# jurgisp/pydreamer

Hardware: AMD Instinct MI355X
Metric: grad-steps/sec (world-model+AC) at B=50,T=50,H=15, 64×64 obs, 1/2/4/8 GPU (higher is better)
Workload: dtype f32; 1 GPU; atari-literal: defaults+atari, batch_size 50, batch_length 50, imag_horizon 15, deter_dim 600, stoch 32x32, hidden 1000, cnn_depth 48, action_dim 18, fp32; fwd + 4 bwd + clip + 4 AdamW per step; replay resident in HBM; global_batch=50, batch_length=50, imag_horizon=15, parallelism=dp1 (batch-sharded [50])

## Files before the change

### include/dreamer_hip.h

```cpp
#ifndef DREAMER_HIP_H
#define DREAMER_HIP_H

#include <stddef.h>
#include <stdint.h>

#ifdef __cplusplus
extern "C" {
#endif

#define DM_OK 0
#define DM_E_SHAPE (-1)
#define DM_E_WORKSPACE (-2)
#define DM_E_HIP (-3)
#define DM_E_DEVICE (-4)
#define DM_E_NULL (-5)

#define DM_MAX_MLP_LAYERS 8

typedef struct dm_shape {
  int32_t T, B, I;
  int32_t H;
  int32_t D, Hd;
  int32_t S, C;
  int32_t E;
  int32_t A;
  int32_t mlp_hidden;
  int32_t mlp_layers;
  int32_t cnn_depth;
  int32_t img, img_ch;
  int32_t flags;
} dm_shape;
#define DM_FLAG_IMAGE_U8 16
#define DM_FLAG_GRU_SHIFT 5
#define DM_FLAG_BF16 128
#define DM_FLAG_GRU_LAYERS_SHIFT 8
#define DM_FLAG_GRU_LAYERS_MASK (3 << DM_FLAG_GRU_LAYERS_SHIFT)
#define DM_FLAG_GRU_MASK (3 << DM_FLAG_GRU_SHIFT)

int dm_version(void);
const char* dm_last_error(void);
int dm_device_check(void);
size_t dm_workspace_bytes(const dm_shape* shp);
int dm_stream_create_cu_mask(const uint32_t* mask, int words, void** stream);
int dm_stream_destroy(void* stream);
int dm_wgrad_side_arm(int on);
int dm_wgrad_side_touch(void);
int dm_wgrad_side_join(void* stream);

#define DM_GEMM_ACCUM 1
#define DM_GEMM_ELU 2
#define DM_GEMM_BF16 256
int dm_gemm_f32(int a_layout, int b_layout, int M, int N, int K,
                const float* A, int lda, const float* B, int ldb, float* C, int ldc,
                const float* bias, const float* add, int ldadd, int flags,
                void* ws, size_t ws_bytes, void* stream);
int dm_gemm_bf16h(int a_layout, int b_layout, int M, int N, int K, const uint16_t* A, int lda, const uint16_t* B, int ldb,
                  float* C, int ldc, uint16_t* C_h, const float* bias, int flags, void* ws, size_t ws_bytes, void* stream);
int dm_bf16_twins_enable(int on);
int dm_gemm_dma_enable(int on);
int dm_dec_l4_bwd_direct_enable(int on);
int dm_rssm_lds_enable(int on);
int dm_bptt_fold_enable(int on);
int dm_rssm_lds_status(void);
int dm_rssm_lds_status_ack(void);
int dm_rssm_lds_gave_up(void);
int dm_rssm_lds_prof(unsigned long long* out16, int reset);

int dm_ln_elu_fwd(int rows, int n, const float* x, int ldx, const float* gamma, const float* beta, float eps,
                  float* y, int ldy, float* stats, void* stream);
int dm_ln_elu_bwd(int rows, int n, const float* x, int ldx, const float* y, int ldy, const float* stats,
                  const float* gamma, const float* dy, int lddy, float* dx, int lddx,
                  float* dgamma, float* dbeta, void* ws, size_t ws_bytes, void* stream);
int dm_colsum(int rows, int n, const float* x, int ld, float* out, void* ws, size_t ws_bytes, void* stream);

int dm_gru_gates_fwd(int rows, int D, const float* gi, const float* gh, const float* h_in, int ldh,
                     float* h_out, int ldo, void* stream);
int dm_gru_gates_bwd(int rows, int D, const float* gi, const float* gh, const float* h_in, int ldh,
                     const float* dh_out, int lddh, float* dgi, float* dgh, float* dh_in, int lddi, void* stream);

int dm_sample_onehot(int rows, int groups, int C, const float* logits, int ldl, const float* u,
                     const int32_t* forced_idx, float* onehot, int ldo, int32_t* idx, void* stream);

int dm_kl_balance_fwd(int rows, int S, int C, const float* post, const float* prior,
                      float* kl, float* ent_post, float* ent_prior, void* stream);
int dm_kl_balance_bwd(int rows, int S, int C, const float* post, const float* prior,
                      float scale_post, float scale_prior, float* dpost, float* dprior, void* stream);
int dm_st_softmax_bwd(int rows, int groups, int C, const float* logits, int ldl, const float* dz, int lddz,
                      float* dlogits, int lddl, int accum, void* stream);

int dm_kl_sampled_fwd(int rows, int S, int C, const float* post, const float* prior, const int32_t* idx, float* out, void* stream);
int dm_kl_sampled_bwd(int rows, int S, int C, const float* post, const float* prior, const int32_t* idx, float scale,
                      const float* row_w, float* dpost, float* dprior, void* stream);
int dm_kl_sampled_gauss_fwd(int rows, int S, const float* post, const float* prior, const float* z, int ldz, float* out,
                            void* stream);
int dm_kl_sampled_gauss_bwd(int rows, int S, const float* post, const float* prior, const float* z, int ldz, float scale,
                            const float* row_w, float* dpost, float* dprior, float* dz, int lddz, void* stream);
int dm_reduce_i(int TB, int I, int W, const float* x, int mode, float* out, float* w_out, void* stream);
int dm_combine_rows(int count, int64_t n, const float* const* x, const float* w, float* out, void* stream);
int dm_scale_rows(int64_t rows, int n, float* x, int ldx, const float* w, float scale, void* stream);

int dm_mask_rows(int rows, int n, const float* x, int ldx, const uint8_t* reset, float* y, int ldy, void* stream);

int dm_im2col_s2(int n, int hb, int wb, int c, int k, const float* big, int big_nchw, float* col, void* stream);
#define DM_C2I_ELU 1
int dm_col2im_s2(int n, int hb, int wb, int c, int k, const float* col, const float* bias, int flags,
                 const float* elu_ref, float* big, void* stream);

typedef struct dm_mlp_params {
  const float* w[DM_MAX_MLP_LAYERS + 1];
  const float* b[DM_MAX_MLP_LAYERS + 1];
  const float* ln_g[DM_MAX_MLP_LAYERS];
  const float* ln_b[DM_MAX_MLP_LAYERS];
  int32_t precision;
  int32_t reserved_;
} dm_mlp_params;
typedef struct dm_mlp_grads {
  float* w[DM_MAX_MLP_LAYERS + 1];
  float* b[DM_MAX_MLP_LAYERS + 1];
  float* ln_g[DM_MAX_MLP_LAYERS];
  float* ln_b[DM_MAX_MLP_LAYERS];
} dm_mlp_grads;
size_t dm_mlp_acts_floats(int rows, int hidden, int layers);
size_t dm_mlp_ws_floats(int rows, int hidden, int layers);
int dm_mlp_head_fwd(int rows, int in_dim, int hidden, int layers, int out_dim,
                    const float* x, int ldx, const dm_mlp_params* p, float* acts, float* out,
                    void* ws, size_t ws_bytes, void* stream);
int dm_mlp_head_fwd_sparse(int rows, int in_dim, int sparse_cols, int hidden, int layers, int out_dim,
                           const float* x, int ldx, const dm_mlp_params* p, float* acts, float* out,
                           void* ws, size_t ws_bytes, void* stream);
int dm_mlp_head_fwd_rows(int rows_total, int row0, int rows, int in_dim, int sparse_cols, int hidden, int layers, int out_dim,
                         const float* x, int ldx, const dm_mlp_params* p, float* acts, float* out,
                         void* ws, size_t ws_bytes, void* stream);

int dm_mlp_head_bwd(int rows, int in_dim, int hidden, int layers, int out_dim,
                    const float* x, int ldx, const dm_mlp_params* p, const float* acts, const float* dout,
                    const dm_mlp_grads* g, float* dx, int lddx, int dx_accum,
                    void* ws, size_t ws_bytes, void* stream);

int dm_head_loss(int kind, int rows, const float* out, const float* target, float scale, float loss_const,
                 float* loss, float* dout, float* mean_out, void* stream);

int dm_head_loss_normal_nd(int rows, int V, const float* out, const float* target, float scale, float loss_const,
                           float* loss, float* dout, float* mean_out, void* stream);

int dm_cat_target_index(int rows, int C, int cells, const float* onehot, int32_t* idx, void* stream);
int dm_cat_image_loss(int rows, int I, int C, int cells, const float* logits, int ld, const int32_t* target, float* loss,
                      float* dlogits, void* stream);
int dm_cat_image_pred(int groups, int I, int C, int cells, const float* logits, int ld, const int32_t* target,
                      const int32_t* seen, float* logp, float* acc, float* acc_seen, void* stream);
int dm_cat_concat_rows(int rows, int I, int F, int E, const float* x, int ldx, const float* extra, float* out, void* stream);

int dm_dense_image_rows(int rows, int C, int cells, const float* image_f32, const int32_t* class_i32, const float* reward,
                        const float* terminal, float* out, int ldo, void* stream);
int dm_elu_rows_fwd(int rows, int n, const float* x, int ldx, float* y, int ldy, void* stream);
int dm_elu_rows_bwd(int rows, int n, const float* y, int ldy, const float* dy, int lddy, float* dx, int lddx, void* stream);
int dm_cat_image_loss_mix(int rows, int I, int C, int cells, const float* logits, int ld, const int32_t* target, float min_prob,
                          float* loss, float* dlogits, void* stream);

size_t dm_goals_stats_ws_floats(int rows, int G);
int dm_goals_stats(int rows, int G, const float* goals, const float* pred, const float* visage, float* out, void* ws,
                   size_t ws_bytes, void* stream);

int dm_preprocess_image_u8(int64_t n, int hw, int c, const uint8_t* src, float* dst, void* stream);

typedef struct dm_conv_params { const float* w[5]; const float* b[5]; } dm_conv_params;
typedef struct dm_conv_grads { float* w[5]; float* b[5]; } dm_conv_grads;
size_t dm_conv_encoder_acts_floats(const dm_shape* shp);
int dm_conv_encoder_fwd(const dm_shape* shp, const float* image , const dm_conv_params* p,
                        float* acts, float* embed , void* ws, size_t ws_bytes, void* stream);
int dm_conv_encoder_bwd(const dm_shape* shp, const float* image, const dm_conv_params* p, const float* acts,
                        const float* dembed, const dm_conv_grads* g, void* ws, size_t ws_bytes, void* stream);
int dm_conv_encoder_fwd_planes(const dm_shape* shp, const float* image, const dm_conv_params* p, const float* reward,
                               const float* terminal, float* acts, float* embed, int ld_embed, void* ws, size_t ws_bytes,
                               void* stream);
int dm_conv_encoder_bwd_planes(const dm_shape* shp, const float* image, const dm_conv_params* p, const float* reward,
                               const float* terminal, const float* acts, const float* dembed, int ld_dembed,
                               const dm_conv_grads* g, void* ws, size_t ws_bytes, void* stream);

size_t dm_conv_decoder_acts_floats(const dm_shape* shp);
size_t dm_conv_decoder_pred_offset(const dm_shape* shp);
int dm_conv_decoder_mse_fwd(const dm_shape* shp, const float* feat, int ldf, const float* target,
                            const dm_conv_params* p, float* acts, float* loss_image, float* image_rec ,
                            void* ws, size_t ws_bytes, void* stream);
int dm_conv_decoder_mse_bwd_rows(const dm_shape* shp, const float* feat, int ldf, const float* target,
                                 const dm_conv_params* p, const float* acts, float scale, const float* row_scale,
                                 const dm_conv_grads* g, float* dfeat, int lddf, void* ws, size_t ws_bytes, void* stream);
int dm_conv_decoder_mse_bwd(const dm_shape* shp, const float* feat, int ldf, const float* target,
                            const dm_conv_params* p, const float* acts, float scale,
                            const dm_conv_grads* g, float* dfeat, int lddf, void* ws, size_t ws_bytes, void* stream);

enum {
  DM_RSSM_Z_W = 0, DM_RSSM_Z_B, DM_RSSM_A_W, DM_RSSM_IN_G, DM_RSSM_IN_B,
  DM_RSSM_GRU_WIH, DM_RSSM_GRU_WHH, DM_RSSM_GRU_BIH, DM_RSSM_GRU_BHH,
  DM_RSSM_PRIOR_H_W, DM_RSSM_PRIOR_H_B, DM_RSSM_PRIOR_G, DM_RSSM_PRIOR_B, DM_RSSM_PRIOR_W, DM_RSSM_PRIOR_OB,
  DM_RSSM_POST_H_W, DM_RSSM_POST_H_B, DM_RSSM_POST_E_W, DM_RSSM_POST_G, DM_RSSM_POST_B, DM_RSSM_POST_W, DM_RSSM_POST_OB,
  DM_RSSM_GRU_LN_G0, DM_RSSM_GRU_LN_B0, DM_RSSM_GRU_LN_G1, DM_RSSM_GRU_LN_B1, DM_RSSM_GRU_LN_G2, DM_RSSM_GRU_LN_B2,
  DM_RSSM_GRU_L1_WIH, DM_RSSM_GRU_L1_WHH, DM_RSSM_GRU_L1_BIH, DM_RSSM_GRU_L1_BHH,
  DM_RSSM_GRU_L2_WIH, DM_RSSM_GRU_L2_WHH, DM_RSSM_GRU_L2_BIH, DM_RSSM_GRU_L2_BHH,
  DM_RSSM_GRU_L3_WIH, DM_RSSM_GRU_L3_WHH, DM_RSSM_GRU_L3_BIH, DM_RSSM_GRU_L3_BHH,
  DM_RSSM_GRU_L1_LN_G0, DM_RSSM_GRU_L1_LN_B0, DM_RSSM_GRU_L1_LN_G1, DM_RSSM_GRU_L1_LN_B1, DM_RSSM_GRU_L1_LN_G2, DM_RSSM_GRU_L1_LN_B2,
  DM_RSSM_GRU_L2_LN_G0, DM_RSSM_GRU_L2_LN_B0, DM_RSSM_GRU_L2_LN_G1, DM_RSSM_GRU_L2_LN_B1, DM_RSSM_GRU_L2_LN_G2, DM_RSSM_GRU_L2_LN_B2,
  DM_RSSM_GRU_L3_LN_G0, DM_RSSM_GRU_L3_LN_B0, DM_RSSM_GRU_L3_LN_G1, DM_RSSM_GRU_L3_LN_B1, DM_RSSM_GRU_L3_LN_G2, DM_RSSM_GRU_L3_LN_B2,
  DM_RSSM_NPARAMS
};
typedef struct dm_rssm_params { const float* p[DM_RSSM_NPARAMS]; } dm_rssm_params;
typedef struct dm_rssm_grads { float* p[DM_RSSM_NPARAMS]; } dm_rssm_grads;
size_t dm_rssm_acts_floats(const dm_shape* shp);
int dm_rssm_sequence_fwd(const dm_shape* shp, const float* embed, const float* action, const uint8_t* reset,
                         const float* h0, const float* z0, const float* u, const int32_t* forced_idx,
                         const dm_rssm_params* p, float* acts, float* feat, float* post, float* prior, int32_t* idx,
                         void* ws, size_t ws_bytes, void* stream);
int dm_rssm_sequence_bwd(const dm_shape* shp, const float* embed, const float* action, const uint8_t* reset,
                         const dm_rssm_params* p, const float* acts, const float* feat, const float* post,
                         float* dfeat, float* dpost, float* dprior,
                         const dm_rssm_grads* g, float* dembed, void* ws, size_t ws_bytes, void* stream);

#define DM_SCHED_FWD_FUSE_LN 1
#define DM_SCHED_FWD_FUSE_SAMPLE 2
#define DM_SCHED_FWD_FRAG 4
#define DM_SCHED_FWD_WZT 8
#define DM_SCHED_FWD_PSYNC 16
#define DM_SCHED_BWD_FUSE_B 1
#define DM_SCHED_BWD_FOLD 2
#define DM_SCHED_BWD_FOLD_SM 4
#define DM_SCHED_BWD_FRAG 8
#define DM_SCHED_BWD_NCHUNK_SHIFT 8
#define DM_SCHED_BWD_NCHUNK_MASK (15 << DM_SCHED_BWD_NCHUNK_SHIFT)
#define DM_SCHED_ROLL_WZT 1
#define DM_SCHED_ROLL_WAT 2
#define DM_SCHED_ROLL_ACTOR_WPACK 4
#define DM_SCHED_ROLL_ACTOR_ADD0 8
#define DM_SCHED_ROLL_FUSE_ACT 16
#define DM_SCHED_ROLL_TW_ON 32
int dm_rssm_last_schedule(int which);

typedef struct dm_gru_params { const float* w_ih; const float* w_hh; const float* b_ih; const float* b_hh; } dm_gru_params;
typedef struct dm_gru_grads { float* w_ih; float* w_hh; float* b_ih; float* b_hh; } dm_gru_grads;
size_t dm_gru_sequence_acts_floats(int T, int B, int In, int D);
size_t dm_gru_sequence_ws_bytes(int T, int B, int In, int D);
// ... 60 lines not shown
```

### pydreamer_amd/csrc/common.h

```cpp
#pragma once
#include <hip/hip_runtime.h>
#include <stdint.h>
#include <stddef.h>
#include "dreamer_hip.h"

int dm_fail(int code, const char* fmt, ...);

#define DM_MAX_DEVICES 16

#define DM_LAUNCH_CHECK()                                                                      \
  do {                                                                                         \
    hipError_t e__ = hipGetLastError();                                                        \
    if (e__ != hipSuccess) return dm_fail(DM_E_HIP, "%s:%d: %s", __FILE__, __LINE__, hipGetErrorString(e__)); \
  } while (0)

#define DM_TRY(expr)                 \
  do {                               \
    int rc__ = (expr);               \
    if (rc__ != DM_OK) return rc__;  \
  } while (0)

#define DM_REQUIRE(cond, code, ...)                     \
  do {                                                  \
    if (!(cond)) return dm_fail(code, __VA_ARGS__);     \
  } while (0)

static inline int dm_cdiv(int64_t a, int64_t b) { return (int)((a + b - 1) / b); }
static inline size_t dm_align_up(size_t x, size_t a) { return (x + a - 1) / a * a; }

struct DmArena {
  float* base;
  size_t cap;
  size_t off;
  bool ok;
  DmArena(void* p, size_t bytes) : base((float*)p), cap(bytes / sizeof(float)), off(0), ok(true) {}
  float* take(size_t nfloats) {
    size_t n = dm_align_up(nfloats, 64);
    if (base == nullptr || off + n > cap) { ok = false; off += n; return nullptr; }
    float* r = base + off;
    off += n;
    return r;
  }
};

hipStream_t dm_wgrad_side_stream(hipStream_t st);
int dm_wgrad_side_fork(hipStream_t st, hipStream_t sw);
int dm_wgrad_side_mark(hipStream_t sw, hipStream_t st);

int dm_cur_precision();
struct DmPrecisionScope {
  int prev;
  explicit DmPrecisionScope(int p);
  ~DmPrecisionScope();
};

struct DmTwinScope {
  bool active, opened;
  explicit DmTwinScope(bool bf16_mode);
  ~DmTwinScope();
};
bool dm_twins_on();
void dm_twin_add(const float* base, size_t n, unsigned short* twin, bool valid);
void dm_twin_mark(const float* p);
unsigned short* dm_twin_of(const float* p, bool need_valid);
void dm_twin_arena_note(const void* acts, bool written);
bool dm_twin_arena_valid(const void* acts);
struct DmCvtSeg { const float* src; unsigned short* dst; size_t n; };
int dm_to_bf16_multi_launch(const DmCvtSeg* segs, int count, hipStream_t st);
static inline size_t dm_half_floats(size_t elems) { return (elems + 1) / 2; }
constexpr int DM_HSTORE_MIN_K = 1024;
constexpr int DM_HSTORE_MIN_K_DENSE = 400;

struct DmGatesBwd;
struct DmGemm {
  int bf16 = dm_cur_precision();
  int a_layout = 0, b_layout = 0;
  int M = 0, N = 0, K = 0;
  const float* A = nullptr; int lda = 0;
  const float* B = nullptr; int ldb = 0;
  float* C = nullptr; int ldc = 0;
  const float* bias = nullptr;
  const float* add = nullptr; int ldadd = 0;
  const float* mulref = nullptr; int ldmul = 0;
  const uint8_t* row_zero = nullptr;
  const int* a_maj = nullptr; const int* a_min = nullptr; int a_tab_vec = 0;
  const int* b_maj = nullptr; const int* b_min = nullptr; int b_tab_vec = 0;
  int a_tab_vec8 = 0, b_tab_vec8 = 0;
  int flags = 0;
  const int2* c_tab = nullptr; int sc_cout = 0, sc_wpitch = 0;
  int bias_mod = 0;
  const float* ln_g = nullptr; const float* ln_b = nullptr; float ln_eps = 1e-3f;
  const float* lnb_x = nullptr; int lnb_ldx = 0; const float* lnb_stats = nullptr;
  const float* eg_x = nullptr; int eg_ldx = 0; const float* eg_stats = nullptr; const float* eg_gamma = nullptr; const float* eg_beta = nullptr;
  float* eg_G = nullptr; int eg_ldg = 0; float* eg_Gf = nullptr; float* eg_ps = nullptr;
  const float* lnf_ps = nullptr; int lnf_nps = 0; const float* lnf_stats = nullptr;
  const float* lnf_xw = nullptr; int lnf_ldxw = 0; const float* lnf_cs = nullptr;
  const float* sm_logits = nullptr; int sm_ld = 0; float* sm_dlogits = nullptr; int sm_ldd = 0;
  const struct DmGatesBwd* gates = nullptr;
  const float* A_frag = nullptr;
  float* C_frag = nullptr;
  const unsigned short* A_h = nullptr;
  const unsigned short* B_h = nullptr;
  unsigned short* C_h = nullptr;
  bool no_twin = false;
};
__host__ __device__ __forceinline__ size_t dm_frag_off(int row, int k) {
  return ((((size_t)(k >> 4) * 4 + (row >> 4)) * 4 + ((k >> 2) & 3)) * 16 + (row & 15)) * 4 + (k & 3);
}
static inline size_t dm_frag_floats(int K) { return (size_t)dm_cdiv(K, 16) * 1024; }
int dm_frag_pack_launch(int rows, int K, const float* X, int ldx, float* Xf, hipStream_t st);
struct DmRssmLds {
  int B, D, Hd, S, C, F, t_begin, t_end;
  const float *wzt, *zb, *wih, *bih, *whh, *bhh, *wph, *bph, *wpo, *bpo, *in_g, *in_b, *post_g, *post_b, *ea, *ee;
  const uint8_t* reset; const float* u; const int32_t* forced;
  float *x1, *gi, *gh, *hin, *zin, *feat, *x2, *post; int32_t* idx;
  float* ws; size_t ws_floats;
};
bool dm_rssm_lds_ok(int B, int D, int Hd, int S, int C);
size_t dm_rssm_lds_ws_floats(int B, int D, int Hd, int S, int C, int steps);
int dm_rssm_lds_launch(const DmRssmLds& q, hipStream_t st);
extern "C" int dm_rssm_lds_enable(int on);
bool dm_z_embed_ok(int n);
int dm_sparse_rows_launch(int rows, int n, int Zc, const float* z, int ldz, const float* Wt, float* x, int ldx,
                          hipStream_t st);
int dm_z_embed_launch(int rows, int n, int S, int C, const int32_t* idx, const uint8_t* row_zero, const float* Wt,
                      const float* bias, const float* add, int ldadd, const int32_t* idx2, const float* Wt2, float* x, int ldx,
                      float* x_frag, const float* gamma, const float* beta, float eps, float* y, int ldy, hipStream_t st,
                      float* y_frag = nullptr, float* stats = nullptr);
struct DmGatesBwd {
  const float* gi; const float* gh; const float* h_in; int ldh, D;
  float* dgi; float* dgh; float* dprev; int ldp; const uint8_t* row_zero;
  float* dgi_frag = nullptr; float* dgh_frag = nullptr;
};
struct DmSample {
  const float* u = nullptr; const int32_t* forced = nullptr;
  float* onehot = nullptr; int ldo = 0;
  int32_t* idx = nullptr;
  float* z_next = nullptr; const uint8_t* next_reset = nullptr;
  float* z_next_frag = nullptr;
};
bool dm_skinny_ln_ok(int M, int N, int K);
int dm_gemm_sample_launch(const DmGemm& q, const DmSample& sm, hipStream_t stream);
int dm_gemm_launch(const DmGemm& g, void* ws, size_t ws_bytes, hipStream_t stream);
int dm_gemm_skinny_try(const DmGemm& g, hipStream_t stream);
int dm_gemm_pair_launch(const DmGemm& g0, const DmGemm& g1, void* ws, size_t ws_bytes, hipStream_t stream);

int dm_colsum_launch(int rows, int n, const float* x, int ld, float* out, void* ws, size_t ws_bytes, hipStream_t st);
int dm_elu_fwd_launch(int rows, int n, const float* x, int ldx, float* y, int ldy, hipStream_t st);
int dm_elu_bwd_launch(int rows, int n, const float* y, int ldy, const float* dy, int lddy, float* dx, int lddx,
                      hipStream_t st);
int dm_ln_elu_fwd_launch(int rows, int n, const float* x, int ldx, const float* gamma, const float* beta, float eps,
                         float* y, int ldy, float* stats, hipStream_t st);
int dm_ln_elu_bwd_dx_launch(int rows, int n, const float* x, int ldx, const float* y, int ldy, const float* stats,
                            const float* gamma, const float* dy, int lddy, float* dx, int lddx, hipStream_t st);
int dm_ln_elu_bwd_params_launch(int rows, int n, const float* x, int ldx, const float* y, int ldy, const float* stats,
                                const float* dy, int lddy, float* dgamma, float* dbeta, void* ws, size_t ws_bytes,
                                hipStream_t st);
int dm_gru_norm_fwd_launch(int kind, int rows, int D, const float* gi, const float* gh, const float* h_in, int ldh,
                           const float* const* ln_g, const float* const* ln_b, float* h_out, int ldo, float* gs, float* gst,
                           float* h_next, const uint8_t* next_reset, hipStream_t st, int ldg = 0, int ldst = 0, int ldn = 0);
int dm_gru_norm_bwd_launch(int kind, int rows, int D, const float* gh, const float* h_in, int ldh, const float* gs,
                           const float* gst, const float* const* ln_g, const float* const* ln_b, const float* dh_out, int lddh,
                           float* dgi, float* dgh, float* dg, float* dh_in, int lddi, const uint8_t* row_zero, hipStream_t st,
                           int ldg = 0, int ldst = 0);
int dm_gru_norm_param_grads_launch(int kind, int rows, int D, const float* gs, const float* gst, const float* dg, float* dgam,
                                   float* dbet, hipStream_t st, int ldg = 0, int ldst = 0);
int dm_gru_gates_fwd_launch(int rows, int D, const float* gi, const float* gh, const float* h_in, int ldh, float* h_out,
                            int ldo, float* h_next, const uint8_t* next_reset, float* h_frag, float* h_next_frag,
                            hipStream_t st, int ldg = 0, int ldn = 0);
int dm_gru_gates_bwd_launch(int rows, int D, const float* gi, const float* gh, const float* h_in, int ldh,
                            const float* dh_out, int lddh, float* dgi, float* dgh, float* dh_in, int lddi, int accum,
                            const uint8_t* row_zero, hipStream_t st, int ldg = 0);
int dm_sample_onehot_launch(int rows, int groups, int C, const float* logits, int ldl, const float* u,
                            const int32_t* forced, float* onehot, int ldo, int32_t* idx, float* z_next,
                            const uint8_t* next_reset, hipStream_t st);
int dm_gauss_sample_bwd_launch(int rows, int S, const float* par, int ldp, const float* z, int ldz, const float* dz,
                               int lddz, float* dpar, int lddp, int accum, hipStream_t st);
int dm_kl_fwd_launch(int rows, int S, int C, const float* post, const float* prior, float* kl, float* ep, float* eq,
                     hipStream_t st);
int dm_kl_bwd_launch(int rows, int S, int C, const float* post, const float* prior, float sp, float sq, float* dpost,
                     float* dprior, hipStream_t st);
int dm_st_softmax_bwd_launch(int rows, int groups, int C, const float* logits, int ldl, const float* dz, int lddz,
                             float* dlogits, int lddl, int accum, hipStream_t st);
int dm_mask_rows_launch(int rows, int n, const float* x, int ldx, const uint8_t* reset, float* y, int ldy, hipStream_t st);
int dm_mask_rows2_launch(int rows, int n1, const float* x1, int ldx1, float* y1, int ldy1, int n2, const float* x2,
                         int ldx2, float* y2, int ldy2, const uint8_t* reset, hipStream_t st);
int dm_sample_continuous_launch(int kind, int rows, int A, const float* params, const float* eps, float* action,
                                hipStream_t st);
int dm_mul_elu_grad_launch(size_t n, const float* dy, const float* yact, float* out, hipStream_t st);

int dm_im2col_s2_launch(int n, int hb, int wb, int c, int k, const float* big, int big_nchw, float* col, hipStream_t st);
int dm_col2im_s2_launch(int n, int hb, int wb, int c, int k, const float* col, const float* bias, int flags,
                        const float* elu_ref, float* big, hipStream_t st);
int dm_permute4_launch(const float* src, float* dst, int d0, int d1, int d2, int d3, int p0, int p1, int p2, int p3,
                       hipStream_t st);

bool dm_enc_l1_direct_ok(int ch, int d, int img);
int dm_enc_l1_fwd_launch(int frames, int d, int u8, const void* image, const float* w, const float* bias, float* wt, float* y,
                         unsigned short* y_h, hipStream_t st);
size_t dm_enc_l1_wgrad_part_floats(int frames, int d);
int dm_enc_l1_wgrad_launch(int frames, int d, int u8, const void* image, const float* G, float* part, float* dW, void* ws,
                           size_t ws_bytes, hipStream_t st);
int dm_enc_l1_fwd_planes_launch(int frames, int d, int u8, const void* image, const float* w5, const float* bias,
                                const float* reward, const float* terminal, float* wt, float* fb, float* y,
                                unsigned short* y_h, hipStream_t st);
size_t dm_enc_l1_planes_part_floats(int frames, int d);
int dm_enc_l1_planes_bwd_launch(int frames, int d, const float* G, const float* reward, const float* terminal,
                                const float* dw3, float* part, float* db, float* dW5, hipStream_t st);
bool dm_dec_l4_direct_ok(int ch, int d, int hs, int k);
size_t dm_dec_l4_w4_floats(int d);
int dm_dec_l4_fwd_launch(int frames, int d, const float* x, const float* w, const float* bias, float* w4, float* out,
                         hipStream_t st);
bool dm_dec_l4_bwd_direct_ok(int ch, int d, int hs, int k);
size_t dm_dec_l4_wp_floats(int d);
size_t dm_dec_l4_wgrad_part_floats(int frames, int d);
int dm_dec_l4_dgrad_launch(int frames, int d, const float* G4, const float* w, float* wp, const float* x3, float* dx,
                           unsigned short* dx_h, hipStream_t st);
int dm_dec_l4_wgrad_launch(int frames, int d, const float* G4, const float* x3, float* part, float* dW, void* ws,
                           size_t ws_bytes, hipStream_t st);

struct DmChainSample {
  const float* u;
  float* onehot;
  int ldo;
  int32_t* idx;
};
int dm_mlp_fwd_launch(int rows, int in_dim, int hidden, int layers, int out_dim, const float* x, int ldx,
                      const dm_mlp_params* p, float* acts, int acts_total_rows, int acts_row_off, float* out, int ldout,
                      void* ws, size_t ws_bytes, hipStream_t st, const float* chain_wpack = nullptr, int sparse_cols = 0,
                      const float* chain_add0 = nullptr, const DmChainSample* chain_sample = nullptr);

bool dm_panel_ok(int rows, int hidden);
int dm_panel_count(int rows);
int dm_panel_ln_fwd_launch(int rows, int hidden, int kin, const float* x, int ldx, const float* W, const float* b,
                           const float* gamma, const float* beta, float eps, float* xpre, float* stats, float* y,
                           const float* wout, const float* bout, float* out, int out_dim, int ldout, hipStream_t st,
                           const unsigned short* Wh = nullptr, int ldw = 0, const float* addm = nullptr);
int dm_panel_bf16_weights_launch(int count, const float* const* w, unsigned short* const* dst, const int* rows, const int* cols,
                                 int transpose, hipStream_t st);
int dm_panel_ln_bwd_launch(int rows, int hidden, int kup, const float* dup, int lddup, const float* W, const float* xpre,
                           const float* stats, const float* gamma, const float* beta, float* dx, float* colpart, float* wt,
                           hipStream_t st, const unsigned short* Wth = nullptr);
int dm_panel_colsum_final_launch(int count, const float* const* part, float* const* out, int n, int npanels, int pstride,
                                 hipStream_t st);

bool dm_mlp_chain_ok(int rows, int in_dim, int hidden, int layers, int out_dim, const float* x, int ldx,
                     const dm_mlp_params* p);
size_t dm_mlp_chain_pack_floats(int in_dim, int layers);
int dm_mlp_chain_pack_launch(int in_dim, int layers, const dm_mlp_params* p, float* wpack, hipStream_t st, int k0 = 0);
int dm_mlp_chain_fwd_launch(int rows, int in_dim, int layers, int out_dim, const float* x, int ldx, const dm_mlp_params* p,
                            float* const* xpre, float* const* stats, float* const* y, float* out, int ldout, const float* wpack,
                            hipStream_t st, int k0 = 0, const float* add0 = nullptr, const DmChainSample* sample = nullptr);
bool dm_mlp_chain_sparse_ok(int in_dim, int sparse_cols);

int dm_prof_slot_begin(int kind, double flops, double bytes, hipStream_t st);
void dm_prof_slot_end(int slot, hipStream_t st);
extern "C" int dm_mlp_chain_min_rows(int rows);
bool dm_prof_active();

static const size_t DM_SPLITK_FLOATS = (size_t)16 * 1024 * 1024;

typedef __bf16 bf16x8 __attribute__((ext_vector_type(8)));
typedef __bf16 bf16x2 __attribute__((ext_vector_type(2)));
typedef float dm_f32x2 __attribute__((ext_vector_type(2)));
__device__ __forceinline__ unsigned dm_pack_bf16x2(float lo, float hi) {
  const dm_f32x2 v = {lo, hi};
  return __builtin_bit_cast(unsigned, __builtin_convertvector(v, bf16x2));
}
__device__ __forceinline__ unsigned dm_f2bf(float x) { return dm_pack_bf16x2(x, 0.f) & 0xFFFFu; }
__device__ __forceinline__ uint2 dm_pack_bf16x4(float4 v) {
  return make_uint2(dm_pack_bf16x2(v.x, v.y), dm_pack_bf16x2(v.z, v.w));
}

__device__ __forceinline__ float dm_elu(float v) { return v > 0.f ? v : expm1f(v); }
__device__ __forceinline__ float dm_elu_grad_from_y(float y) { return y > 0.f ? 1.f : y + 1.f; }

__device__ __forceinline__ float dm_wave_sum(float v) {
#pragma unroll
  for (int off = 32; off > 0; off >>= 1) v += __shfl_xor(v, off, 64);
  return v;
}
__device__ __forceinline__ float dm_wave_max(float v) {
#pragma unroll
  for (int off = 32; off > 0; off >>= 1) v = fmaxf(v, __shfl_xor(v, off, 64));
  return v;
}
```

### pydreamer_amd/csrc/elementwise.hip

```cpp
#include "common.h"

template <bool CACHE>
__global__ void __launch_bounds__(256) ln_elu_fwd_kernel(int rows, int n, const float* __restrict__ x, int ldx,
                                                         const float* __restrict__ gamma, const float* __restrict__ beta,
                                                         float eps, float* __restrict__ y, int ldy, float* __restrict__ stats,
                                                         unsigned short* __restrict__ y_h) {
  const int row = blockIdx.x * 4 + (threadIdx.x >> 6);
  const int lane = threadIdx.x & 63;
  if (row >= rows) return;
  const float* xr = x + (size_t)row * ldx;
  unsigned short* yh = y_h ? y_h + (size_t)row * ldy : nullptr;
  float xc[16];
  float s = 0.f;
  if (CACHE) {
#pragma unroll
    for (int j = 0; j < 16; ++j) {
      const int c = lane + 64 * j;
      xc[j] = c < n ? xr[c] : 0.f;
      s += xc[j];
    }
  } else {
    for (int c = lane; c < n; c += 64) s += xr[c];
  }
  const float mean = dm_wave_sum(s) / (float)n;
  float v = 0.f;
  if (CACHE) {
#pragma unroll
    for (int j = 0; j < 16; ++j) {
      const float d = (lane + 64 * j < n) ? xc[j] - mean : 0.f;
      v += d * d;
    }
  } else {
    for (int c = lane; c < n; c += 64) {
      const float d = xr[c] - mean;
      v += d * d;
    }
  }
  const float var = dm_wave_sum(v) / (float)n;
  const float rstd = 1.0f / sqrtf(var + eps);
  float* yr = y + (size_t)row * ldy;
  if (CACHE) {
#pragma unroll
    for (int j = 0; j < 16; ++j) {
      const int c = lane + 64 * j;
      if (c < n) {
        const float o = dm_elu((xc[j] - mean) * rstd * gamma[c] + beta[c]);
        yr[c] = o;
        if (yh) yh[c] = (unsigned short)dm_f2bf(o);
      }
    }
  } else {
    for (int c = lane; c < n; c += 64) {
      const float o = dm_elu((xr[c] - mean) * rstd * gamma[c] + beta[c]);
      yr[c] = o;
      if (yh) yh[c] = (unsigned short)dm_f2bf(o);
    }
  }
  if (lane == 0) {
    stats[2 * row] = mean;
    stats[2 * row + 1] = rstd;
  }
}

template <bool CACHE>
__global__ void __launch_bounds__(256) ln_elu_bwd_dx_kernel(int rows, int n, const float* __restrict__ x, int ldx,
                                                            const float* __restrict__ y, int ldy,
                                                            const float* __restrict__ stats, const float* __restrict__ gamma,
                                                            const float* __restrict__ dy, int lddy,
                                                            float* __restrict__ dx, int lddx) {
  const int row = blockIdx.x * 4 + (threadIdx.x >> 6);
  const int lane = threadIdx.x & 63;
  if (row >= rows) return;
  const float mean = stats[2 * row], rstd = stats[2 * row + 1];
  const float* xr = x + (size_t)row * ldx;
  const float* yr = y + (size_t)row * ldy;
  const float* dyr = dy + (size_t)row * lddy;
  float gc[16], hc[16];
  float sg = 0.f, sgx = 0.f;
  if (CACHE) {
#pragma unroll
    for (int j = 0; j < 16; ++j) {
      const int c = lane + 64 * j;
      gc[j] = 0.f; hc[j] = 0.f;
      if (c < n) {
        gc[j] = dyr[c] * dm_elu_grad_from_y(yr[c]) * gamma[c];
        hc[j] = (xr[c] - mean) * rstd;
      }
      sg += gc[j];
      sgx += gc[j] * hc[j];
    }
  } else {
    for (int c = lane; c < n; c += 64) {
      const float g = dyr[c] * dm_elu_grad_from_y(yr[c]) * gamma[c];
      const float xh = (xr[c] - mean) * rstd;
      sg += g;
      sgx += g * xh;
    }
  }
  sg = dm_wave_sum(sg) / (float)n;
  sgx = dm_wave_sum(sgx) / (float)n;
  float* dxr = dx + (size_t)row * lddx;
  if (CACHE) {
#pragma unroll
    for (int j = 0; j < 16; ++j) {
      const int c = lane + 64 * j;
      if (c < n) dxr[c] = rstd * (gc[j] - sg - hc[j] * sgx);
    }
  } else {
    for (int c = lane; c < n; c += 64) {
      const float g = dyr[c] * dm_elu_grad_from_y(yr[c]) * gamma[c];
      const float xh = (xr[c] - mean) * rstd;
      dxr[c] = rstd * (g - sg - xh * sgx);
    }
  }
}

template <int MODE>
__global__ void __launch_bounds__(256) colsum_partial_kernel(int rows, int n, int rows_per_chunk,
                                                             const float* __restrict__ x, int ldx,
                                                             const float* __restrict__ y, int ldy,
                                                             const float* __restrict__ stats,
                                                             const float* __restrict__ dy, int lddy,
                                                             float* __restrict__ partial) {
  __shared__ float red[2][4][64];
  const int cx = threadIdx.x & 63, ry = threadIdx.x >> 6;
  const int col = blockIdx.x * 64 + cx;
  const int chunk = blockIdx.y;
  const int r0 = chunk * rows_per_chunk;
  const int r1 = min(rows, r0 + rows_per_chunk);
  float a0 = 0.f, a1 = 0.f;
  if (col < n) {
    if (MODE == 0) {
      float b0 = 0.f, b1 = 0.f, b2 = 0.f, b3 = 0.f;
      int r = r0 + ry;
      for (; r + 12 < r1; r += 16) {
        b0 += x[(size_t)r * ldx + col];
        b1 += x[(size_t)(r + 4) * ldx + col];
        b2 += x[(size_t)(r + 8) * ldx + col];
        b3 += x[(size_t)(r + 12) * ldx + col];
      }
      for (; r < r1; r += 4) b0 += x[(size_t)r * ldx + col];
      a0 = (b0 + b1) + (b2 + b3);
    } else {
      for (int r = r0 + ry; r < r1; r += 4) {
        const float dl = dy[(size_t)r * lddy + col] * dm_elu_grad_from_y(y[(size_t)r * ldy + col]);
        const float xh = (x[(size_t)r * ldx + col] - stats[2 * r]) * stats[2 * r + 1];
        a0 += dl * xh;
        a1 += dl;
      }
    }
  }
  red[0][ry][cx] = a0;
  red[1][ry][cx] = a1;
  __syncthreads();
  if (ry == 0 && col < n) {
    const int nq = (MODE == 0) ? 1 : 2;
    float s0 = red[0][0][cx] + red[0][1][cx] + red[0][2][cx] + red[0][3][cx];
    partial[((size_t)chunk * nq + 0) * n + col] = s0;
    if (MODE == 1) {
      float s1 = red[1][0][cx] + red[1][1][cx] + red[1][2][cx] + red[1][3][cx];
      partial[((size_t)chunk * nq + 1) * n + col] = s1;
    }
  }
}

__global__ void __launch_bounds__(256) colsum_flat_kernel(long long total, int n, int W, long long chunk_elems,
                                                          const float* __restrict__ x, float* __restrict__ partial) {
  __shared__ float sh[256];
  const long long base = (long long)blockIdx.x * chunk_elems;
  const long long end = min(total, base + chunk_elems);
  float b0 = 0.f, b1 = 0.f, b2 = 0.f, b3 = 0.f;
  if ((int)threadIdx.x < W) {
    long long i = base + threadIdx.x;
    for (; i + 3LL * W < end; i += 4LL * W) {
      b0 += x[i];
      b1 += x[i + W];
      b2 += x[i + 2LL * W];
      b3 += x[i + 3LL * W];
    }
    for (; i < end; i += W) b0 += x[i];
  }
  sh[threadIdx.x] = (b0 + b1) + (b2 + b3);
  __syncthreads();
  if ((int)threadIdx.x < n) {
    float s = 0.f;
    for (int t = threadIdx.x; t < W; t += n) s += sh[t];
    partial[(size_t)blockIdx.x * n + threadIdx.x] = s;
  }
}

__global__ void __launch_bounds__(256) colsum_final_kernel(int n, int chunks, int nq, const float* __restrict__ partial,
                                                           float* __restrict__ out0, float* __restrict__ out1) {
  __shared__ float red[8][32];
  const int cx = threadIdx.x & 31, cy = threadIdx.x >> 5;
  const int col = blockIdx.x * 32 + cx;
  for (int q = 0; q < nq; ++q) {
    float s = 0.f;
    if (col < n) {
      const float* p = partial + (size_t)q * n + col;
      const size_t st = (size_t)nq * n;
      int c = cy;
      for (; c + 24 < chunks; c += 32) {
        const float v0 = p[(size_t)c * st], v1 = p[(size_t)(c + 8) * st], v2 = p[(size_t)(c + 16) * st], v3 = p[(size_t)(c + 24) * st];
        s += v0; s += v1; s += v2; s += v3;
      }
      for (; c < chunks; c += 8) s += p[(size_t)c * st];
    }
    red[cy][cx] = s;
    __syncthreads();
    if (cy == 0 && col < n) {
      float t = 0.f;
#pragma unroll
      for (int k = 0; k < 8; ++k) t += red[k][cx];
      (q == 0 ? out0 : out1)[col] = t;
    }
    __syncthreads();
  }
}

static int colsum_plan(int rows, size_t budget_floats, int n, int nq, int* rows_per_chunk) {
  int chunks = dm_cdiv(rows, 64);
  if (chunks > 1024) chunks = 1024;
  const size_t per = (size_t)n * nq;
  if (per > 0 && (size_t)chunks * per > budget_floats) chunks = (int)(budget_floats / per);
  if (chunks < 1) chunks = 1;
  *rows_per_chunk = dm_cdiv(rows, chunks);
  return dm_cdiv(rows, *rows_per_chunk);
}

int dm_colsum_launch(int rows, int n, const float* x, int ld, float* out, void* ws, size_t ws_bytes, hipStream_t st) {
  if (n <= 0) return DM_OK;
  if (rows <= 0) {
    (void)hipMemsetAsync(out, 0, (size_t)n * sizeof(float), st);
    return DM_OK;
  }
  DM_REQUIRE(ws && ws_bytes >= (size_t)n * sizeof(float), DM_E_WORKSPACE, "colsum: workspace too small");
  const size_t budget = ws_bytes / sizeof(float);
  int chunks;
  if (n <= 64 && ld == n && (long long)rows * n >= (1 << 16)) {
    const long long total = (long long)rows * n;
    const int W = 256 - 256 % n;
    long long want = total / ((long long)W * 16);
    if (want > 2048) want = 2048;
    if (want < 1) want = 1;
    if ((size_t)want * n > budget) want = (long long)(budget / n);
    long long chunk_elems = (total + want - 1) / want;
    chunk_elems = (chunk_elems + W - 1) / W * W;
    chunks = (int)((total + chunk_elems - 1) / chunk_elems);
    hipLaunchKernelGGL(colsum_flat_kernel, dim3(chunks), dim3(256), 0, st, total, n, W, chunk_elems, x, (float*)ws);
  } else {
    int rpc;
    chunks = colsum_plan(rows, budget, n, 1, &rpc);
    hipLaunchKernelGGL((colsum_partial_kernel<0>), dim3(dm_cdiv(n, 64), chunks), dim3(256), 0, st, rows, n, rpc, x, ld,
                       nullptr, 0, nullptr, nullptr, 0, (float*)ws);
  }
  DM_LAUNCH_CHECK();
  hipLaunchKernelGGL(colsum_final_kernel, dim3(dm_cdiv(n, 32)), dim3(256), 0, st, n, chunks, 1, (const float*)ws, out,
                     nullptr);
  DM_LAUNCH_CHECK();
  return DM_OK;
}

int dm_ln_elu_fwd_launch(int rows, int n, const float* x, int ldx, const float* gamma, const float* beta, float eps,
                         float* y, int ldy, float* stats, hipStream_t st) {
  if (rows <= 0) return DM_OK;
  unsigned short* y_h = dm_twin_of(y, false);
  if (y_h) dm_twin_mark(y);
  if (n <= 1024)
    hipLaunchKernelGGL((ln_elu_fwd_kernel<true>), dim3(dm_cdiv(rows, 4)), dim3(256), 0, st, rows, n, x, ldx, gamma, beta,
                       eps, y, ldy, stats, y_h);
  else
    hipLaunchKernelGGL((ln_elu_fwd_kernel<false>), dim3(dm_cdiv(rows, 4)), dim3(256), 0, st, rows, n, x, ldx, gamma, beta,
                       eps, y, ldy, stats, y_h);
  DM_LAUNCH_CHECK();
  return DM_OK;
}

__global__ void __launch_bounds__(256) elu_fwd_kernel(int rows, int n, const float* __restrict__ x, int ldx,
                                                      float* __restrict__ y, int ldy) {
  const size_t total = (size_t)rows * n;
  for (size_t i = (size_t)blockIdx.x * 256 + threadIdx.x; i < total; i += (size_t)gridDim.x * 256) {
    const size_t r = i / n, c = i % n;
    y[r * ldy + c] = dm_elu(x[r * ldx + c]);
  }
}
__global__ void __launch_bounds__(256) elu_bwd_kernel(int rows, int n, const float* __restrict__ y, int ldy,
                                                      const float* __restrict__ dy, int lddy, float* __restrict__ dx,
                                                      int lddx) {
  const size_t total = (size_t)rows * n;
  for (size_t i = (size_t)blockIdx.x * 256 + threadIdx.x; i < total; i += (size_t)gridDim.x * 256) {
    const size_t r = i / n, c = i % n;
    dx[r * lddx + c] = dy[r * lddy + c] * dm_elu_grad_from_y(y[r * ldy + c]);
  }
}
int dm_elu_fwd_launch(int rows, int n, const float* x, int ldx, float* y, int ldy, hipStream_t st) {
  if (rows <= 0) return DM_OK;
  const size_t total = (size_t)rows * n;
  hipLaunchKernelGGL(elu_fwd_kernel, dim3((unsigned)((total + 255) / 256 < 65536 ? (total + 255) / 256 : 65536)), dim3(256), 0,
                     st, rows, n, x, ldx, y, ldy);
  DM_LAUNCH_CHECK();
  return DM_OK;
}
int dm_elu_bwd_launch(int rows, int n, const float* y, int ldy, const float* dy, int lddy, float* dx, int lddx,
                      hipStream_t st) {
  if (rows <= 0) return DM_OK;
  const size_t total = (size_t)rows * n;
  hipLaunchKernelGGL(elu_bwd_kernel, dim3((unsigned)((total + 255) / 256 < 65536 ? (total + 255) / 256 : 65536)), dim3(256), 0,
                     st, rows, n, y, ldy, dy, lddy, dx, lddx);
  DM_LAUNCH_CHECK();
  return DM_OK;
}

int dm_ln_elu_bwd_dx_launch(int rows, int n, const float* x, int ldx, const float* y, int ldy, const float* stats,
                            const float* gamma, const float* dy, int lddy, float* dx, int lddx, hipStream_t st) {
  if (rows <= 0) return DM_OK;
  if (n <= 1024)
    hipLaunchKernelGGL((ln_elu_bwd_dx_kernel<true>), dim3(dm_cdiv(rows, 4)), dim3(256), 0, st, rows, n, x, ldx, y, ldy,
                       stats, gamma, dy, lddy, dx, lddx);
  else
    hipLaunchKernelGGL((ln_elu_bwd_dx_kernel<false>), dim3(dm_cdiv(rows, 4)), dim3(256), 0, st, rows, n, x, ldx, y, ldy,
                       stats, gamma, dy, lddy, dx, lddx);
  DM_LAUNCH_CHECK();
  return DM_OK;
}

int dm_ln_elu_bwd_params_launch(int rows, int n, const float* x, int ldx, const float* y, int ldy, const float* stats,
                                const float* dy, int lddy, float* dgamma, float* dbeta, void* ws, size_t ws_bytes,
                                hipStream_t st) {
  int rpc;
  DM_REQUIRE(ws && ws_bytes >= (size_t)2 * n * sizeof(float), DM_E_WORKSPACE, "ln_bwd: workspace too small");
  const int chunks = colsum_plan(rows, ws_bytes / sizeof(float), n, 2, &rpc);
  hipLaunchKernelGGL((colsum_partial_kernel<1>), dim3(dm_cdiv(n, 64), chunks), dim3(256), 0, st, rows, n, rpc, x, ldx, y,
                     ldy, stats, dy, lddy, (float*)ws);
  DM_LAUNCH_CHECK();
  hipLaunchKernelGGL(colsum_final_kernel, dim3(dm_cdiv(n, 32)), dim3(256), 0, st, n, chunks, 2, (const float*)ws, dgamma,
                     dbeta);
  DM_LAUNCH_CHECK();
  return DM_OK;
}

extern "C" int dm_ln_elu_fwd(int rows, int n, const float* x, int ldx, const float* gamma, const float* beta, float eps,
                             float* y, int ldy, float* stats, void* stream) {
  DM_REQUIRE(x && gamma && beta && y && stats, DM_E_NULL, "ln_elu_fwd: null pointer");
  return dm_ln_elu_fwd_launch(rows, n, x, ldx, gamma, beta, eps, y, ldy, stats, (hipStream_t)stream);
}

extern "C" int dm_ln_elu_bwd(int rows, int n, const float* x, int ldx, const float* y, int ldy, const float* stats,
                             const float* gamma, const float* dy, int lddy, float* dx, int lddx, float* dgamma,
                             float* dbeta, void* ws, size_t ws_bytes, void* stream) {
  DM_REQUIRE(x && y && stats && gamma && dy && dx && dgamma && dbeta, DM_E_NULL, "ln_elu_bwd: null pointer");
  DM_TRY(dm_ln_elu_bwd_dx_launch(rows, n, x, ldx, y, ldy, stats, gamma, dy, lddy, dx, lddx, (hipStream_t)stream));
  return dm_ln_elu_bwd_params_launch(rows, n, x, ldx, y, ldy, stats, dy, lddy, dgamma, dbeta, ws, ws_bytes,
                                     (hipStream_t)stream);
}

extern "C" int dm_colsum(int rows, int n, const float* x, int ld, float* out, void* ws, size_t ws_bytes, void* stream) {
  DM_REQUIRE(x && out, DM_E_NULL, "colsum: null pointer");
  return dm_colsum_launch(rows, n, x, ld, out, ws, ws_bytes, (hipStream_t)stream);
}

__device__ __forceinline__ float dm_sigmoid(float v) { return 1.0f / (1.0f + expf(-v)); }

__global__ void __launch_bounds__(256) gru_gates_fwd_kernel(int rows, int D, const float* __restrict__ gi,
                                                            const float* __restrict__ gh, const float* __restrict__ h_in,
                                                            int ldh, float* __restrict__ h_out, int ldo,
                                                            float* __restrict__ h_next,
                                                            const uint8_t* __restrict__ next_reset,
                                                            float* __restrict__ h_frag, float* __restrict__ h_next_frag,
                                                            int ldg, int ldn, unsigned short* __restrict__ h_out_h) {
  const size_t total = (size_t)rows * D;
  for (size_t i = (size_t)blockIdx.x * 256 + threadIdx.x; i < total; i += (size_t)gridDim.x * 256) {
    const int r = (int)(i / D), d = (int)(i % D);
    const float* gir = gi + (size_t)r * ldg;
    const float* ghr = gh + (size_t)r * ldg;
    const float rg = dm_sigmoid(gir[d] + ghr[d]);
    const float ug = dm_sigmoid(gir[D + d] + ghr[D + d]);
    const float ng = tanhf(gir[2 * D + d] + rg * ghr[2 * D + d]);
    const float h = h_in[(size_t)r * ldh + d];
    const float ho = (h - ng) * ug + ng;
    h_out[(size_t)r * ldo + d] = ho;
    if (h_out_h) h_out_h[(size_t)r * ldo + d] = (unsigned short)dm_f2bf(ho);
    const float hn = (next_reset && next_reset[r]) ? 0.f : ho;
    if (h_next) h_next[(size_t)r * ldn + d] = hn;
    if (h_frag) h_frag[dm_frag_off(r, d)] = ho;
    if (h_next_frag) h_next_frag[dm_frag_off(r, d)] = hn;
  }
}
__global__ void __launch_bounds__(256) frag_pack_kernel(int rows, int K, const float* __restrict__ X, int ldx,
                                                        float* __restrict__ Xf) {
  const int total = rows * K;
  for (int i = blockIdx.x * 256 + threadIdx.x; i < total; i += gridDim.x * 256) {
    const int r = i / K, k = i % K;
    Xf[dm_frag_off(r, k)] = X[(size_t)r * ldx + k];
  }
}

__global__ void __launch_bounds__(256) gru_gates_bwd_kernel(int rows, int D, const float* __restrict__ gi,
                                                            const float* __restrict__ gh, const float* __restrict__ h_in,
                                                            int ldh, const float* __restrict__ dh_out, int lddh,
                                                            float* __restrict__ dgi, float* __restrict__ dgh,
                                                            float* __restrict__ dh_in, int lddi, int accum,
                                                            const uint8_t* __restrict__ row_zero, int ldg) {
  const size_t total = (size_t)rows * D;
  for (size_t i = (size_t)blockIdx.x * 256 + threadIdx.x; i < total; i += (size_t)gridDim.x * 256) {
    const int r = (int)(i / D), d = (int)(i % D);
    const size_t g0 = (size_t)r * ldg;
    const float ghn = gh[g0 + 2 * D + d];
    const float rg = dm_sigmoid(gi[g0 + d] + gh[g0 + d]);
    const float ug = dm_sigmoid(gi[g0 + D + d] + gh[g0 + D + d]);
    const float ng = tanhf(gi[g0 + 2 * D + d] + rg * ghn);
    const float h = h_in[(size_t)r * ldh + d];
    const float dh = dh_out[(size_t)r * lddh + d];
    const float dn = dh * (1.f - ug);
    const float du = dh * (h - ng);
    const float dpn = dn * (1.f - ng * ng);
    const float dpr = dpn * ghn * rg * (1.f - rg);
    const float dpu = du * ug * (1.f - ug);
    dgi[g0 + d] = dpr;
    dgi[g0 + D + d] = dpu;
    dgi[g0 + 2 * D + d] = dpn;
    dgh[g0 + d] = dpr;
    dgh[g0 + D + d] = dpu;
    dgh[g0 + 2 * D + d] = dpn * rg;
    if (dh_in) {
      const float v = (row_zero && row_zero[r]) ? 0.f : dh * ug;
      float* o = dh_in + (size_t)r * lddi + d;
      *o = accum ? *o + v : v;
    }
  }
}

struct GruLnParams { const float* g[3]; const float* b[3]; };

template <int KIND>
__global__ void __launch_bounds__(256) gru_norm_fwd_kernel(int rows, int D, const float* __restrict__ gi,
                                                           const float* __restrict__ gh, const float* __restrict__ h_in,
                                                           int ldh, const GruLnParams lp, float* __restrict__ h_out, int ldo,
                                                           float* __restrict__ gs, float* __restrict__ gst,
                                                           float* __restrict__ h_next, const uint8_t* __restrict__ next_reset,
                                                           int ldg, int ldst, int ldn) {
  const int row = blockIdx.x * 4 + (threadIdx.x >> 6);
  const int lane = threadIdx.x & 63;
  if (row >= rows) return;
  const float eps = 1e-3f;
  const float* gir = gi + (size_t)row * ldg;
  const float* ghr = gh + (size_t)row * ldg;
  float* sr = gs + (size_t)row * ldg;
  const float* hr = h_in + (size_t)row * ldh;
  float st[6] = {0.f, 0.f, 0.f, 0.f, 0.f, 0.f};
  if (KIND == 2) {
    float sum = 0.f;
    for (int j = lane; j < 3 * D; j += 64) { const float v = gir[j] + ghr[j]; sr[j] = v; sum += v; }
    const float mean = dm_wave_sum(sum) / (float)(3 * D);
    float var = 0.f;
    for (int j = lane; j < 3 * D; j += 64) { const float d = (gir[j] + ghr[j]) - mean; var += d * d; }
    const float rstd = 1.0f / sqrtf(dm_wave_sum(var) / (float)(3 * D) + eps);
    st[0] = mean; st[1] = rstd;
    for (int d = lane; d < D; d += 64) {
      const float g_r = ((gir[d] + ghr[d]) - mean) * rstd * lp.g[0][d] + lp.b[0][d];
      const float g_u = ((gir[D + d] + ghr[D + d]) - mean) * rstd * lp.g[0][D + d] + lp.b[0][D + d];
      const float g_n = ((gir[2 * D + d] + ghr[2 * D + d]) - mean) * rstd * lp.g[0][2 * D + d] + lp.b[0][2 * D + d];
      const float r = dm_sigmoid(g_r), u = dm_sigmoid(g_u - 1.0f), n = tanhf(r * g_n);
      const float ho = u * n + (1.f - u) * hr[d];
      h_out[(size_t)row * ldo + d] = ho;
      if (h_next) h_next[(size_t)row * ldn + d] = (next_reset && next_reset[row]) ? 0.f : ho;
    }
  } else {
    float s0 = 0.f, s1 = 0.f;
    for (int d = lane; d < D; d += 64) {
      const float a = gir[d] + ghr[d], b = gir[D + d] + ghr[D + d];
      sr[d] = a; sr[D + d] = b;
      s0 += a; s1 += b;
    }
    const float m0 = dm_wave_sum(s0) / (float)D, m1 = dm_wave_sum(s1) / (float)D;
    float v0 = 0.f, v1 = 0.f;
    for (int d = lane; d < D; d += 64) {
      const float a = (gir[d] + ghr[d]) - m0, b = (gir[D + d] + ghr[D + d]) - m1;
      v0 += a * a; v1 += b * b;
    }
    const float r0 = 1.0f / sqrtf(dm_wave_sum(v0) / (float)D + eps), r1 = 1.0f / sqrtf(dm_wave_sum(v1) / (float)D + eps);
    float s2 = 0.f;
    for (int d = lane; d < D; d += 64) {
      const float r = dm_sigmoid(((gir[d] + ghr[d]) - m0) * r0 * lp.g[0][d] + lp.b[0][d]);
      const float c = gir[2 * D + d] + r * ghr[2 * D + d];
      sr[2 * D + d] = c;
      s2 += c;
    }
    const float m2 = dm_wave_sum(s2) / (float)D;
    float v2 = 0.f;
    for (int d = lane; d < D; d += 64) { const float c = sr[2 * D + d] - m2; v2 += c * c; }
    const float r2 = 1.0f / sqrtf(dm_wave_sum(v2) / (float)D + eps);
    st[0] = m0; st[1] = r0; st[2] = m1; st[3] = r1; st[4] = m2; st[5] = r2;
    for (int d = lane; d < D; d += 64) {
      const float u = dm_sigmoid(((gir[D + d] + ghr[D + d]) - m1) * r1 * lp.g[1][d] + lp.b[1][d]);
      const float n = tanhf((sr[2 * D + d] - m2) * r2 * lp.g[2][d] + lp.b[2][d]);
      const float ho = u * n + (1.f - u) * hr[d];
      h_out[(size_t)row * ldo + d] = ho;
      if (h_next) h_next[(size_t)row * ldn + d] = (next_reset && next_reset[row]) ? 0.f : ho;
    }
  }
  if (lane < 6) gst[(size_t)row * ldst + lane] = st[lane];
}

template <int KIND>
__global__ void __launch_bounds__(256) gru_norm_bwd_kernel(int rows, int D, const float* __restrict__ gh,
                                                           const float* __restrict__ h_in, int ldh,
// ... 673 lines not shown
}
int dm_gauss_sample_bwd_launch(int rows, int S, const float* par, int ldp, const float* z, int ldz, const float* dz,
                               int lddz, float* dpar, int lddp, int accum, hipStream_t st) {
  if (rows <= 0) return DM_OK;
  hipLaunchKernelGGL(gauss_sample_bwd_kernel, dim3(ew_blocks((size_t)rows * S)), dim3(256), 0, st, rows, S, par, ldp, z, ldz,
                     dz, lddz, dpar, lddp, accum);
  DM_LAUNCH_CHECK();
  return DM_OK;
}
__global__ void __launch_bounds__(256) gauss_kl_fwd_kernel(int rows, int S, const float* __restrict__ post,
                                                           const float* __restrict__ prior, float* __restrict__ kl,
                                                           float* __restrict__ ent_post, float* __restrict__ ent_prior) {
  const int row = blockIdx.x * 4 + (threadIdx.x >> 6);
  const int lane = threadIdx.x & 63;
  if (row >= rows) return;
  const float* a = post + (size_t)row * 2 * S;
  const float* b = prior + (size_t)row * 2 * S;
  float akl = 0.f, aep = 0.f, aeq = 0.f;
  for (int s = lane; s < S; s += 64) {
    const float s1 = dm_gauss_std(a[S + s]), s2 = dm_gauss_std(b[S + s]);
    const float d = a[s] - b[s];
    akl += logf(s2 / s1) + (s1 * s1 + d * d) / (2.0f * s2 * s2) - 0.5f;
    aep += 1.4189385332046727f + logf(s1);
    aeq += 1.4189385332046727f + logf(s2);
  }
  akl = dm_wave_sum(akl); aep = dm_wave_sum(aep); aeq = dm_wave_sum(aeq);
  if (lane == 0) {
    kl[row] = akl;
    if (ent_post) ent_post[row] = aep;
    if (ent_prior) ent_prior[row] = aeq;
  }
}
__global__ void __launch_bounds__(256) gauss_kl_bwd_kernel(int rows, int S, const float* __restrict__ post,
                                                           const float* __restrict__ prior, float sp, float sq,
                                                           float* __restrict__ dpost, float* __restrict__ dprior) {
  const int total = rows * S;
  for (int i = blockIdx.x * 256 + threadIdx.x; i < total; i += gridDim.x * 256) {
    const int r = i / S, s = i % S;
    const size_t o = (size_t)r * 2 * S;
    const float g1 = dm_sigmoid(post[o + S + s]), g2 = dm_sigmoid(prior[o + S + s]);
    const float s1 = 2.0f * g1 + 0.1f, s2 = 2.0f * g2 + 0.1f;
    const float d = post[o + s] - prior[o + s];
    const float i22 = 1.0f / (s2 * s2);
    dpost[o + s] = sp * d * i22;
    dpost[o + S + s] = sp * (s1 * i22 - 1.0f / s1) * 2.0f * g1 * (1.0f - g1);
    dprior[o + s] = -sq * d * i22;
    dprior[o + S + s] = sq * (1.0f / s2 - (s1 * s1 + d * d) * i22 / s2) * 2.0f * g2 * (1.0f - g2);
  }
}

int dm_sample_onehot_launch(int rows, int groups, int C, const float* logits, int ldl, const float* u,
                            const int32_t* forced, float* onehot, int ldo, int32_t* idx, float* z_next,
                            const uint8_t* next_reset, hipStream_t st) {
  if (rows <= 0) return DM_OK;
  if (C == 0) {
    DM_REQUIRE(u && !forced, DM_E_NULL, "sample: Gaussian latents need their noise (and cannot be index-forced)");
    hipLaunchKernelGGL(gauss_sample_kernel, dim3(ew_blocks((size_t)rows * groups)), dim3(256), 0, st, rows, groups, logits,
                       ldl, u, onehot, ldo, z_next, next_reset);
    DM_LAUNCH_CHECK();
    if (idx && hipMemsetAsync(idx, 0, (size_t)rows * groups * sizeof(int32_t), st) != hipSuccess)
      return dm_fail(DM_E_HIP, "sample: memset failed");
    return DM_OK;
  }
  const size_t tg = (size_t)rows * groups;
  if (C == 32 && (ldl & 3) == 0 && (ldo & 3) == 0 &&
      (((uintptr_t)logits | (uintptr_t)onehot | (uintptr_t)z_next) & 15) == 0) {
    hipLaunchKernelGGL(sample_onehot_lane32_kernel, dim3((unsigned)dm_cdiv(tg, 256)), dim3(256), 0, st, rows, groups,
                       logits, ldl, u, forced, onehot, ldo, idx, z_next, next_reset);
    DM_LAUNCH_CHECK();
    return DM_OK;
  }
#define DM_SAMPLE_WAVE(L)                                                                                              \
  hipLaunchKernelGGL((sample_onehot_wave_kernel<L>), dim3(ew_blocks(tg * L)), dim3(256), 0, st, rows, groups, C, logits, \
                     ldl, u, forced, onehot, ldo, idx)
  if (C <= 8) DM_SAMPLE_WAVE(8);
  else if (C <= 16) DM_SAMPLE_WAVE(16);
  else if (C <= 32) DM_SAMPLE_WAVE(32);
  else if (C <= 64) DM_SAMPLE_WAVE(64);
  else
    hipLaunchKernelGGL(sample_onehot_kernel, dim3(ew_blocks(tg)), dim3(256), 0, st, rows, groups, C, logits, ldl, u, forced,
                       onehot, ldo, idx);
#undef DM_SAMPLE_WAVE
  DM_LAUNCH_CHECK();
  if (z_next) DM_TRY(dm_mask_rows_launch(rows, groups * C, onehot, ldo, next_reset, z_next, groups * C, st));
  return DM_OK;
}
extern "C" int dm_sample_onehot(int rows, int groups, int C, const float* logits, int ldl, const float* u,
                                const int32_t* forced_idx, float* onehot, int ldo, int32_t* idx, void* stream) {
  DM_REQUIRE(logits && onehot && (u || forced_idx), DM_E_NULL, "sample_onehot: null pointer");
  DM_REQUIRE(C >= 0 && groups >= 1, DM_E_SHAPE, "sample_onehot: bad groups/C");
  return dm_sample_onehot_launch(rows, groups, C, logits, ldl, u, forced_idx, onehot, ldo, idx, nullptr, nullptr,
                                 (hipStream_t)stream);
}

__device__ __forceinline__ float dm_group_lse(const float* x, int C) {
  float mx = x[0];
  for (int k = 1; k < C; ++k) mx = fmaxf(mx, x[k]);
  float s = 0.f;
  for (int k = 0; k < C; ++k) s += expf(x[k] - mx);
  return mx + logf(s);
}

__global__ void __launch_bounds__(256) kl_fwd_kernel(int rows, int S, int C, const float* __restrict__ post,
                                                     const float* __restrict__ prior, float* __restrict__ kl,
                                                     float* __restrict__ ent_post, float* __restrict__ ent_prior) {
  const int row = blockIdx.x * 4 + (threadIdx.x >> 6);
  const int lane = threadIdx.x & 63;
  if (row >= rows) return;
  float akl = 0.f, aep = 0.f, aeq = 0.f;
  for (int s = lane; s < S; s += 64) {
    const float* a = post + ((size_t)row * S + s) * C;
    const float* b = prior + ((size_t)row * S + s) * C;
    const float la = dm_group_lse(a, C), lb = dm_group_lse(b, C);
    float gk = 0.f, ep = 0.f, eq = 0.f;
    for (int k = 0; k < C; ++k) {
      const float lp = a[k] - la, lq = b[k] - lb;
      const float p = expf(lp), q = expf(lq);
      gk += p * (lp - lq);
      ep -= p * lp;
      eq -= q * lq;
    }
    akl += gk; aep += ep; aeq += eq;
  }
  akl = dm_wave_sum(akl); aep = dm_wave_sum(aep); aeq = dm_wave_sum(aeq);
  if (lane == 0) {
    kl[row] = akl;
    if (ent_post) ent_post[row] = aep;
    if (ent_prior) ent_prior[row] = aeq;
  }
}

__global__ void __launch_bounds__(256) kl_bwd_kernel(int rows, int S, int C, const float* __restrict__ post,
                                                     const float* __restrict__ prior, float sp, float sq,
                                                     float* __restrict__ dpost, float* __restrict__ dprior) {
  const int total = rows * S;
  for (int i = blockIdx.x * 256 + threadIdx.x; i < total; i += gridDim.x * 256) {
    const float* a = post + (size_t)i * C;
    const float* b = prior + (size_t)i * C;
    const float la = dm_group_lse(a, C), lb = dm_group_lse(b, C);
    float gk = 0.f;
    for (int k = 0; k < C; ++k) {
      const float lp = a[k] - la, lq = b[k] - lb;
      gk += expf(lp) * (lp - lq);
    }
    for (int k = 0; k < C; ++k) {
      const float lp = a[k] - la, lq = b[k] - lb;
      const float p = expf(lp), q = expf(lq);
      dpost[(size_t)i * C + k] = sp * p * ((lp - lq) - gk);
      dprior[(size_t)i * C + k] = sq * (q - p);
    }
  }
}

__global__ void __launch_bounds__(256) kl_sampled_fwd_kernel(int rows, int S, int C, const float* __restrict__ post,
                                                             const float* __restrict__ prior, const int32_t* __restrict__ idx,
                                                             float* __restrict__ out) {
  const int row = blockIdx.x * 4 + (threadIdx.x >> 6);
  const int lane = threadIdx.x & 63;
  if (row >= rows) return;
  float acc = 0.f;
  for (int s = lane; s < S; s += 64) {
    const float* a = post + ((size_t)row * S + s) * C;
    const float* b = prior + ((size_t)row * S + s) * C;
    const int k = idx[(size_t)row * S + s];
    acc += (a[k] - dm_group_lse(a, C)) - (b[k] - dm_group_lse(b, C));
  }
  acc = dm_wave_sum(acc);
  if (lane == 0) out[row] = acc;
}
__global__ void __launch_bounds__(256) kl_sampled_bwd_kernel(int rows, int S, int C, const float* __restrict__ post,
                                                             const float* __restrict__ prior, const int32_t* __restrict__ idx,
                                                             float scale, const float* __restrict__ row_w,
                                                             float* __restrict__ dpost, float* __restrict__ dprior) {
  const int total = rows * S;
  for (int i = blockIdx.x * 256 + threadIdx.x; i < total; i += gridDim.x * 256) {
    const float* a = post + (size_t)i * C;
    const float* b = prior + (size_t)i * C;
    const float la = dm_group_lse(a, C), lb = dm_group_lse(b, C);
    const float w = scale * (row_w ? row_w[i / S] : 1.f);
    const int kk = idx[i];
    for (int k = 0; k < C; ++k) {
      const float hot = k == kk ? 1.f : 0.f;
      dpost[(size_t)i * C + k] = w * (hot - expf(a[k] - la));
      dprior[(size_t)i * C + k] = -w * (hot - expf(b[k] - lb));
    }
  }
}
extern "C" int dm_kl_sampled_fwd(int rows, int S, int C, const float* post, const float* prior, const int32_t* idx,
                                 float* out, void* stream) {
  DM_REQUIRE(post && prior && idx && out, DM_E_NULL, "kl_sampled_fwd: null pointer");
  if (rows <= 0) return DM_OK;
  hipLaunchKernelGGL(kl_sampled_fwd_kernel, dim3(dm_cdiv(rows, 4)), dim3(256), 0, (hipStream_t)stream, rows, S, C, post, prior,
                     idx, out);
  DM_LAUNCH_CHECK();
  return DM_OK;
}
extern "C" int dm_kl_sampled_bwd(int rows, int S, int C, const float* post, const float* prior, const int32_t* idx,
                                 float scale, const float* row_w, float* dpost, float* dprior, void* stream) {
  DM_REQUIRE(post && prior && idx && dpost && dprior, DM_E_NULL, "kl_sampled_bwd: null pointer");
  if (rows <= 0) return DM_OK;
  int blocks = dm_cdiv((size_t)rows * S, 256);
  if (blocks > 4096) blocks = 4096;
  hipLaunchKernelGGL(kl_sampled_bwd_kernel, dim3(blocks), dim3(256), 0, (hipStream_t)stream, rows, S, C, post, prior, idx,
                     scale, row_w, dpost, dprior);
  DM_LAUNCH_CHECK();
  return DM_OK;
}

__global__ void __launch_bounds__(256) gauss_kl_sampled_fwd_kernel(int rows, int S, const float* __restrict__ post,
                                                                   const float* __restrict__ prior, const float* __restrict__ z,
                                                                   int ldz, float* __restrict__ out) {
  const int row = blockIdx.x * 4 + (threadIdx.x >> 6);
  const int lane = threadIdx.x & 63;
  if (row >= rows) return;
  const float* a = post + (size_t)row * 2 * S;
  const float* b = prior + (size_t)row * 2 * S;
  float acc = 0.f;
  for (int s = lane; s < S; s += 64) {
    const float s1 = dm_gauss_std(a[S + s]), s2 = dm_gauss_std(b[S + s]);
    const float zz = z[(size_t)row * ldz + s];
    const float d1 = (zz - a[s]) / s1, d2 = (zz - b[s]) / s2;
    acc += (-logf(s1) - 0.5f * d1 * d1) - (-logf(s2) - 0.5f * d2 * d2);
  }
  acc = dm_wave_sum(acc);
  if (lane == 0) out[row] = acc;
}
__global__ void __launch_bounds__(256) gauss_kl_sampled_bwd_kernel(int rows, int S, const float* __restrict__ post,
                                                                   const float* __restrict__ prior, const float* __restrict__ z,
                                                                   int ldz, float scale, const float* __restrict__ row_w,
                                                                   float* __restrict__ dpost, float* __restrict__ dprior,
                                                                   float* __restrict__ dz, int lddz) {
  const int total = rows * S;
  for (int i = blockIdx.x * 256 + threadIdx.x; i < total; i += gridDim.x * 256) {
    const int r = i / S, s = i % S;
    const size_t o = (size_t)r * 2 * S;
    const float g1 = dm_sigmoid(post[o + S + s]), g2 = dm_sigmoid(prior[o + S + s]);
    const float s1 = 2.0f * g1 + 0.1f, s2 = 2.0f * g2 + 0.1f;
    const float zz = z[(size_t)r * ldz + s];
    const float e1 = zz - post[o + s], e2 = zz - prior[o + s];
    const float w = scale * (row_w ? row_w[r] : 1.f);
    const float i11 = 1.0f / (s1 * s1), i22 = 1.0f / (s2 * s2);
    dpost[o + s] = w * e1 * i11;
    dpost[o + S + s] = w * (-1.0f / s1 + e1 * e1 * i11 / s1) * 2.0f * g1 * (1.0f - g1);
    dprior[o + s] = -w * e2 * i22;
    dprior[o + S + s] = w * (1.0f / s2 - e2 * e2 * i22 / s2) * 2.0f * g2 * (1.0f - g2);
    dz[(size_t)r * lddz + s] += w * (-e1 * i11 + e2 * i22);
  }
}
extern "C" int dm_kl_sampled_gauss_fwd(int rows, int S, const float* post, const float* prior, const float* z, int ldz,
                                       float* out, void* stream) {
  DM_REQUIRE(post && prior && z && out, DM_E_NULL, "kl_sampled_gauss_fwd: null pointer");
  if (rows <= 0) return DM_OK;
  hipLaunchKernelGGL(gauss_kl_sampled_fwd_kernel, dim3(dm_cdiv(rows, 4)), dim3(256), 0, (hipStream_t)stream, rows, S, post, prior,
                     z, ldz, out);
  DM_LAUNCH_CHECK();
  return DM_OK;
}
extern "C" int dm_kl_sampled_gauss_bwd(int rows, int S, const float* post, const float* prior, const float* z, int ldz,
                                       float scale, const float* row_w, float* dpost, float* dprior, float* dz, int lddz,
                                       void* stream) {
  DM_REQUIRE(post && prior && z && dpost && dprior && dz, DM_E_NULL, "kl_sampled_gauss_bwd: null pointer");
  if (rows <= 0) return DM_OK;
  int blocks = dm_cdiv((size_t)rows * S, 256);
  if (blocks > 4096) blocks = 4096;
  hipLaunchKernelGGL(gauss_kl_sampled_bwd_kernel, dim3(blocks), dim3(256), 0, (hipStream_t)stream, rows, S, post, prior, z, ldz,
                     scale, row_w, dpost, dprior, dz, lddz);
  DM_LAUNCH_CHECK();
  return DM_OK;
}

__global__ void __launch_bounds__(256) reduce_i_kernel(int TB, int I, int W, const float* __restrict__ x, int mode,
                                                       float* __restrict__ out, float* __restrict__ w_out) {
  const size_t total = (size_t)TB * W;
  for (size_t e = (size_t)blockIdx.x * 256 + threadIdx.x; e < total; e += (size_t)gridDim.x * 256) {
    const size_t tb = e / W;
    const int c = (int)(e % W);
    const float* p = x + (tb * I) * W + c;
    if (mode == 1) {
      float mx = -p[0];
      for (int i = 1; i < I; ++i) mx = fmaxf(mx, -p[(size_t)i * W]);
      float s = 0.f;
      for (int i = 0; i < I; ++i) s += expf(-p[(size_t)i * W] - mx);
      out[e] = -(mx + logf(s) - logf((float)I));
      if (w_out)
        for (int i = 0; i < I; ++i) w_out[tb * I + i] = expf(-p[(size_t)i * W] - mx) / s;
    } else {
      float s = 0.f;
      for (int i = 0; i < I; ++i) s += p[(size_t)i * W];
      out[e] = mode == 0 ? s / (float)I : s;
    }
  }
}
extern "C" int dm_reduce_i(int TB, int I, int W, const float* x, int mode, float* out, float* w_out, void* stream) {
  DM_REQUIRE(x && out, DM_E_NULL, "reduce_i: null pointer");
  DM_REQUIRE(I >= 1 && W >= 1 && (unsigned)mode <= 2 && (mode != 1 || W == 1), DM_E_SHAPE, "reduce_i: I=%d W=%d mode=%d", I, W, mode);
  if (TB <= 0) return DM_OK;
  int blocks = dm_cdiv((size_t)TB * W, 256);
  if (blocks > 4096) blocks = 4096;
  hipLaunchKernelGGL(reduce_i_kernel, dim3(blocks), dim3(256), 0, (hipStream_t)stream, TB, I, W, x, mode, out, w_out);
  DM_LAUNCH_CHECK();
  return DM_OK;
}

struct RowCombineArgs { const float* x[8]; float w[8]; };
__global__ void __launch_bounds__(256) combine_rows_kernel(int count, long long n, const RowCombineArgs a, float* __restrict__ out) {
  for (long long i = (long long)blockIdx.x * 256 + threadIdx.x; i < n; i += (long long)gridDim.x * 256) {
    float s = 0.f;
    for (int j = 0; j < count; ++j) s += a.w[j] * a.x[j][i];
    out[i] = s;
  }
}
extern "C" int dm_combine_rows(int count, int64_t n, const float* const* x, const float* w, float* out, void* stream) {
  DM_REQUIRE(x && w && out, DM_E_NULL, "combine_rows: null pointer");
  DM_REQUIRE(count >= 1 && count <= 8, DM_E_SHAPE, "combine_rows: count %d not in [1,8]", count);
  if (n <= 0) return DM_OK;
  RowCombineArgs a;
  for (int j = 0; j < count; ++j) { a.x[j] = x[j]; a.w[j] = w[j]; }
  int blocks = dm_cdiv(n, 256);
  if (blocks > 2048) blocks = 2048;
  hipLaunchKernelGGL(combine_rows_kernel, dim3(blocks), dim3(256), 0, (hipStream_t)stream, count, (long long)n, a, out);
  DM_LAUNCH_CHECK();
  return DM_OK;
}

__global__ void __launch_bounds__(256) scale_rows_kernel(long long rows, int n, float* __restrict__ x, int ldx,
                                                         const float* __restrict__ w, float scale) {
  const long long total = rows * n;
  for (long long e = (long long)blockIdx.x * 256 + threadIdx.x; e < total; e += (long long)gridDim.x * 256) {
    const long long r = e / n;
    x[r * ldx + e % n] *= w[r] * scale;
  }
}
extern "C" int dm_scale_rows(int64_t rows, int n, float* x, int ldx, const float* w, float scale, void* stream) {
  DM_REQUIRE(x && w, DM_E_NULL, "scale_rows: null pointer");
  if (rows <= 0 || n <= 0) return DM_OK;
  int blocks = dm_cdiv(rows * n, 256);
  if (blocks > 4096) blocks = 4096;
  hipLaunchKernelGGL(scale_rows_kernel, dim3(blocks), dim3(256), 0, (hipStream_t)stream, (long long)rows, n, x, ldx, w, scale);
  DM_LAUNCH_CHECK();
  return DM_OK;
}

template <int LPG>
__global__ void __launch_bounds__(256) st_softmax_bwd_kernel(int rows, int groups, int C, const float* __restrict__ logits,
                                                             int ldl, const float* __restrict__ dz, int lddz,
                                                             float* __restrict__ dlogits, int lddl, int accum) {
  constexpr int GPB = 256 / LPG;
  const int k = threadIdx.x % LPG;
  const int total = rows * groups;
  for (int i0 = blockIdx.x * GPB; i0 < total; i0 += gridDim.x * GPB) {
    const int i = i0 + threadIdx.x / LPG;
    const bool live = i < total && k < C;
    const int r = live ? i / groups : 0, gq = live ? i % groups : 0;
    const size_t off = (size_t)gq * C + k;
    const float x = live ? logits[(size_t)r * ldl + off] : -INFINITY;
    const float g = live ? dz[(size_t)r * lddz + off] : 0.f;
    float mx = x;
#pragma unroll
    for (int o = LPG / 2; o > 0; o >>= 1) mx = fmaxf(mx, __shfl_xor(mx, o, 64));
    const float e = live ? expf(x - mx) : 0.f;
    float se = e, sg = e * g;
#pragma unroll
    for (int o = LPG / 2; o > 0; o >>= 1) {
      se += __shfl_xor(se, o, 64);
      sg += __shfl_xor(sg, o, 64);
    }
    if (live) {
      const float p = e / se;
      const float v = p * (g - sg / se);
      float* o = dlogits + (size_t)r * lddl + off;
      *o = accum ? *o + v : v;
    }
  }
}

int dm_kl_fwd_launch(int rows, int S, int C, const float* post, const float* prior, float* kl, float* ep, float* eq,
                     hipStream_t st) {
  if (rows <= 0) return DM_OK;
  if (C == 0) {
    hipLaunchKernelGGL(gauss_kl_fwd_kernel, dim3(dm_cdiv(rows, 4)), dim3(256), 0, st, rows, S, post, prior, kl, ep, eq);
    DM_LAUNCH_CHECK();
    return DM_OK;
  }
  hipLaunchKernelGGL(kl_fwd_kernel, dim3(dm_cdiv(rows, 4)), dim3(256), 0, st, rows, S, C, post, prior, kl, ep, eq);
  DM_LAUNCH_CHECK();
  return DM_OK;
}
int dm_kl_bwd_launch(int rows, int S, int C, const float* post, const float* prior, float sp, float sq, float* dpost,
                     float* dprior, hipStream_t st) {
  if (rows <= 0) return DM_OK;
  if (C == 0) {
    hipLaunchKernelGGL(gauss_kl_bwd_kernel, dim3(ew_blocks((size_t)rows * S)), dim3(256), 0, st, rows, S, post, prior, sp, sq,
                       dpost, dprior);
    DM_LAUNCH_CHECK();
    return DM_OK;
  }
  hipLaunchKernelGGL(kl_bwd_kernel, dim3(ew_blocks((size_t)rows * S)), dim3(256), 0, st, rows, S, C, post, prior, sp, sq,
                     dpost, dprior);
  DM_LAUNCH_CHECK();
  return DM_OK;
}
int dm_st_softmax_bwd_launch(int rows, int groups, int C, const float* logits, int ldl, const float* dz, int lddz,
                             float* dlogits, int lddl, int accum, hipStream_t st) {
  if (rows <= 0) return DM_OK;
  DM_REQUIRE(C >= 1 && C <= 64, DM_E_SHAPE, "st_softmax_bwd: C=%d not in [1,64]", C);
  const size_t tg = (size_t)rows * groups;
  if (C <= 8) hipLaunchKernelGGL((st_softmax_bwd_kernel<8>), dim3(ew_blocks(tg * 8)), dim3(256), 0, st, rows, groups, C, logits, ldl, dz, lddz, dlogits, lddl, accum);
  else if (C <= 16) hipLaunchKernelGGL((st_softmax_bwd_kernel<16>), dim3(ew_blocks(tg * 16)), dim3(256), 0, st, rows, groups, C, logits, ldl, dz, lddz, dlogits, lddl, accum);
  else if (C <= 32) hipLaunchKernelGGL((st_softmax_bwd_kernel<32>), dim3(ew_blocks(tg * 32)), dim3(256), 0, st, rows, groups, C, logits, ldl, dz, lddz, dlogits, lddl, accum);
  else hipLaunchKernelGGL((st_softmax_bwd_kernel<64>), dim3(ew_blocks(tg * 64)), dim3(256), 0, st, rows, groups, C, logits, ldl, dz, lddz, dlogits, lddl, accum);
  DM_LAUNCH_CHECK();
  return DM_OK;
}
extern "C" int dm_kl_balance_fwd(int rows, int S, int C, const float* post, const float* prior, float* kl,
                                 float* ent_post, float* ent_prior, void* stream) {
  DM_REQUIRE(post && prior && kl, DM_E_NULL, "kl_fwd: null pointer");
  return dm_kl_fwd_launch(rows, S, C, post, prior, kl, ent_post, ent_prior, (hipStream_t)stream);
}
extern "C" int dm_kl_balance_bwd(int rows, int S, int C, const float* post, const float* prior, float scale_post,
                                 float scale_prior, float* dpost, float* dprior, void* stream) {
  DM_REQUIRE(post && prior && dpost && dprior, DM_E_NULL, "kl_bwd: null pointer");
  return dm_kl_bwd_launch(rows, S, C, post, prior, scale_post, scale_prior, dpost, dprior, (hipStream_t)stream);
}
extern "C" int dm_st_softmax_bwd(int rows, int groups, int C, const float* logits, int ldl, const float* dz, int lddz,
                                 float* dlogits, int lddl, int accum, void* stream) {
  DM_REQUIRE(logits && dz && dlogits, DM_E_NULL, "st_softmax_bwd: null pointer");
  return dm_st_softmax_bwd_launch(rows, groups, C, logits, ldl, dz, lddz, dlogits, lddl, accum, (hipStream_t)stream);
}

__global__ void __launch_bounds__(256) mask_rows_kernel(int rows, int n, const float* __restrict__ x, int ldx,
                                                        const uint8_t* __restrict__ reset, float* __restrict__ y, int ldy) {
  const size_t total = (size_t)rows * n;
  for (size_t i = (size_t)blockIdx.x * 256 + threadIdx.x; i < total; i += (size_t)gridDim.x * 256) {
    const int r = (int)(i / n), c = (int)(i % n);
    const float m = reset[r] ? 0.f : 1.f;
    y[(size_t)r * ldy + c] = x[(size_t)r * ldx + c] * m;
  }
}
__global__ void __launch_bounds__(256) mask_rows2_kernel(int rows, int n1, const float* __restrict__ x1, int ldx1,
                                                         float* __restrict__ y1, int ldy1, int n2,
                                                         const float* __restrict__ x2, int ldx2, float* __restrict__ y2,
                                                         int ldy2, const uint8_t* __restrict__ reset) {
  const int n = n1 + n2;
  const size_t total = (size_t)rows * n;
  for (size_t i = (size_t)blockIdx.x * 256 + threadIdx.x; i < total; i += (size_t)gridDim.x * 256) {
    const int r = (int)(i / n), c = (int)(i % n);
    const float m = reset[r] ? 0.f : 1.f;
    if (c < n1) y1[(size_t)r * ldy1 + c] = x1[(size_t)r * ldx1 + c] * m;
    else y2[(size_t)r * ldy2 + (c - n1)] = x2[(size_t)r * ldx2 + (c - n1)] * m;
  }
}
int dm_mask_rows2_launch(int rows, int n1, const float* x1, int ldx1, float* y1, int ldy1, int n2, const float* x2,
                         int ldx2, float* y2, int ldy2, const uint8_t* reset, hipStream_t st) {
  if (rows <= 0) return DM_OK;
  hipLaunchKernelGGL(mask_rows2_kernel, dim3(ew_blocks((size_t)rows * (n1 + n2))), dim3(256), 0, st, rows, n1, x1, ldx1, y1,
                     ldy1, n2, x2, ldx2, y2, ldy2, reset);
  DM_LAUNCH_CHECK();
  return DM_OK;
}
int dm_mask_rows_launch(int rows, int n, const float* x, int ldx, const uint8_t* reset, float* y, int ldy, hipStream_t st) {
  if (rows <= 0 || n <= 0) return DM_OK;
  hipLaunchKernelGGL(mask_rows_kernel, dim3(ew_blocks((size_t)rows * n)), dim3(256), 0, st, rows, n, x, ldx, reset, y, ldy);
  DM_LAUNCH_CHECK();
  return DM_OK;
}
extern "C" int dm_mask_rows(int rows, int n, const float* x, int ldx, const uint8_t* reset, float* y, int ldy,
                            void* stream) {
  DM_REQUIRE(x && reset && y, DM_E_NULL, "mask_rows: null pointer");
  return dm_mask_rows_launch(rows, n, x, ldx, reset, y, ldy, (hipStream_t)stream);
}

__global__ void __launch_bounds__(256) mul_elu_grad_kernel(size_t n, const float* __restrict__ dy,
                                                           const float* __restrict__ yact, float* __restrict__ out) {
  for (size_t i = (size_t)blockIdx.x * 256 + threadIdx.x; i < n; i += (size_t)gridDim.x * 256)
    out[i] = dy[i] * dm_elu_grad_from_y(yact[i]);
}
int dm_mul_elu_grad_launch(size_t n, const float* dy, const float* yact, float* out, hipStream_t st) {
  if (n == 0) return DM_OK;
  hipLaunchKernelGGL(mul_elu_grad_kernel, dim3(ew_blocks(n)), dim3(256), 0, st, n, dy, yact, out);
  DM_LAUNCH_CHECK();
  return DM_OK;
}

__global__ void __launch_bounds__(256) head_loss_kernel(int kind, int rows, const float* __restrict__ out,
                                                        const float* __restrict__ target, float scale, float loss_const,
                                                        float* __restrict__ loss, float* __restrict__ dout,
                                                        float* __restrict__ mean_out) {
  for (int i = blockIdx.x * 256 + threadIdx.x; i < rows; i += gridDim.x * 256) {
    const float o = out[i];
    const float y = target ? target[i] : 0.f;
    if (kind == 0) {
      const float d = o - y;
      if (loss) loss[i] = 0.5f * d * d + loss_const;
      if (dout) dout[i] = scale * d;
      if (mean_out) mean_out[i] = o;
    } else {
      const float sg = dm_sigmoid(o);
      if (loss) loss[i] = fmaxf(o, 0.f) - o * y + log1pf(expf(-fabsf(o)));
      if (dout) dout[i] = scale * (sg - y);
      if (mean_out) mean_out[i] = sg;
    }
  }
}
extern "C" int dm_head_loss(int kind, int rows, const float* out, const float* target, float scale, float loss_const,
                            float* loss, float* dout, float* mean_out, void* stream) {
  DM_REQUIRE(out, DM_E_NULL, "head_loss: null pointer");
  DM_REQUIRE(kind == 0 || kind == 1, DM_E_SHAPE, "head_loss: kind %d", kind);
  if (rows <= 0) return DM_OK;
  hipLaunchKernelGGL(head_loss_kernel, dim3(ew_blocks(rows)), dim3(256), 0, (hipStream_t)stream, kind, rows, out, target,
                     scale, loss_const, loss, dout, mean_out);
  DM_LAUNCH_CHECK();
  return DM_OK;
}

__global__ void __launch_bounds__(256) head_loss_nd_kernel(int rows, int V, const float* __restrict__ out,
                                                           const float* __restrict__ target, float scale, float row_const,
                                                           float* __restrict__ loss, float* __restrict__ dout,
                                                           float* __restrict__ mean_out) {
  const int sub = threadIdx.x & 7;
  for (int r = blockIdx.x * 32 + (threadIdx.x >> 3); r < rows; r += gridDim.x * 32) {
    const size_t base = (size_t)r * V;
    float s = 0.f;
    for (int v = sub; v < V; v += 8) {
      const float o = out[base + v];
      const float d = o - (target ? target[base + v] : 0.f);
      s = fmaf(d, d, s);
      if (dout) dout[base + v] = scale * d;
      if (mean_out) mean_out[base + v] = o;
    }
    s += __shfl_xor(s, 1, 8);
    s += __shfl_xor(s, 2, 8);
    s += __shfl_xor(s, 4, 8);
    if (sub == 0 && loss) loss[r] = 0.5f * s + row_const;
  }
}
extern "C" int dm_head_loss_normal_nd(int rows, int V, const float* out, const float* target, float scale, float loss_const,
                                      float* loss, float* dout, float* mean_out, void* stream) {
  DM_REQUIRE(out, DM_E_NULL, "head_loss_normal_nd: null pointer");
  DM_REQUIRE(V >= 1, DM_E_SHAPE, "head_loss_normal_nd: V %d", V);
  if (rows <= 0) return DM_OK;
  int blocks = dm_cdiv(rows, 32);
  if (blocks > 4096) blocks = 4096;
  hipLaunchKernelGGL(head_loss_nd_kernel, dim3(blocks), dim3(256), 0, (hipStream_t)stream, rows, V, out, target, scale,
                     (float)V * loss_const, loss, dout, mean_out);
  DM_LAUNCH_CHECK();
  return DM_OK;
}

__global__ void __launch_bounds__(256) gae_kernel(int H, int M, float gamma, float lambda, const float* __restrict__ reward,
                                                  const float* __restrict__ terminal, const float* __restrict__ value_t,
                                                  float* __restrict__ advantage, float* __restrict__ advantage_gae,
// ... 288 lines not shown
```

### pydreamer_amd/csrc/mlp.hip

```cpp
#include "common.h"

struct MlpActs {
  float* xpre[DM_MAX_MLP_LAYERS];
  float* stats[DM_MAX_MLP_LAYERS];
  float* y[DM_MAX_MLP_LAYERS];
};
static size_t mlp_carve(int rows, int hidden, int layers, float* base, MlpActs* a) {
  DmArena ar(base, (size_t)1 << 62);
  for (int l = 0; l < layers; ++l) {
    float* xp = ar.take((size_t)rows * hidden);
    float* st = ar.take((size_t)rows * 2);
    float* yy = ar.take((size_t)rows * hidden);
    if (a) { a->xpre[l] = xp; a->stats[l] = st; a->y[l] = yy; }
  }
  return ar.off;
}
extern "C" size_t dm_mlp_acts_floats(int rows, int hidden, int layers) {
  if (rows < 0 || hidden < 0 || layers < 0 || layers > DM_MAX_MLP_LAYERS) return 0;
  return mlp_carve(rows, hidden, layers, nullptr, nullptr);
}

static size_t mlp_ws_floats(int rows, int hidden, int layers) {
  const size_t rh = dm_align_up((size_t)rows * hidden, 64);
  return DM_SPLITK_FLOATS + 3 * rh + dm_align_up((size_t)layers * dm_panel_count(rows) * 3 * hidden, 64) +
// ... 114 lines not shown
                                    l == 0 ? addm : nullptr));
      in = a.y[l]; ldin = hidden; kin = hidden;
    }
    if (fuse_out) return DM_OK;
  } else {
    for (int l = 0; l < layers; ++l) {
      DmGemm q;
      q.M = rows; q.N = hidden; q.K = kin;
      q.A = in; q.lda = ldin;
      q.B = p->w[l]; q.ldb = kin;
      q.C = a.xpre[l]; q.ldc = hidden;
      q.bias = p->b[l];
      DM_TRY(dm_gemm_launch(q, ws, skb, st));
      if (normed)
        DM_TRY(dm_ln_elu_fwd_launch(rows, hidden, a.xpre[l], hidden, p->ln_g[l], p->ln_b[l], 1e-3f, a.y[l], hidden,
                                    a.stats[l], st));
      else DM_TRY(dm_elu_fwd_launch(rows, hidden, a.xpre[l], hidden, a.y[l], hidden, st));
      in = a.y[l]; ldin = hidden; kin = hidden;
    }
  }
  DmGemm q;
  q.M = rows; q.N = out_dim; q.K = hidden;
  q.A = in; q.lda = hidden;
  q.B = p->w[layers]; q.ldb = hidden;
  q.C = out; q.ldc = ldout;
  q.bias = p->b[layers];
  return dm_gemm_launch(q, ws, skb, st);
}

extern "C" int dm_mlp_head_fwd(int rows, int in_dim, int hidden, int layers, int out_dim, const float* x, int ldx,
                               const dm_mlp_params* p, float* acts, float* out, void* ws, size_t ws_bytes, void* stream) {
  DM_REQUIRE(x && p && out && ws, DM_E_NULL, "mlp_head_fwd: null pointer");
  DmPrecisionScope prec(p->precision);
  return dm_mlp_fwd_launch(rows, in_dim, hidden, layers, out_dim, x, ldx, p, acts, rows, 0, out, out_dim, ws, ws_bytes,
                           (hipStream_t)stream);
}

extern "C" int dm_mlp_head_fwd_sparse(int rows, int in_dim, int sparse_cols, int hidden, int layers, int out_dim,
                                      const float* x, int ldx, const dm_mlp_params* p, float* acts, float* out, void* ws,
                                      size_t ws_bytes, void* stream) {
  DM_REQUIRE(x && p && out && ws, DM_E_NULL, "mlp_head_fwd_sparse: null pointer");
  DmPrecisionScope prec(p->precision);
  return dm_mlp_fwd_launch(rows, in_dim, hidden, layers, out_dim, x, ldx, p, acts, rows, 0, out, out_dim, ws, ws_bytes,
                           (hipStream_t)stream, nullptr, sparse_cols);
}

extern "C" int dm_mlp_head_fwd_rows(int rows_total, int row0, int rows, int in_dim, int sparse_cols, int hidden, int layers,
                                    int out_dim, const float* x, int ldx, const dm_mlp_params* p, float* acts, float* out,
                                    void* ws, size_t ws_bytes, void* stream) {
  DM_REQUIRE(x && p && out && ws, DM_E_NULL, "mlp_head_fwd_rows: null pointer");
  DM_REQUIRE(row0 >= 0 && rows >= 1 && row0 + rows <= rows_total, DM_E_SHAPE, "mlp_head_fwd_rows: window [%d, %d) of %d rows", row0,
             row0 + rows, rows_total);
  DmPrecisionScope prec(p->precision);
  return dm_mlp_fwd_launch(rows, in_dim, hidden, layers, out_dim, x + (size_t)row0 * ldx, ldx, p, acts, rows_total, row0,
                           out + (size_t)row0 * out_dim, out_dim, ws, ws_bytes, (hipStream_t)stream, nullptr, sparse_cols);
}

extern "C" int dm_mlp_head_bwd(int rows, int in_dim, int hidden, int layers, int out_dim, const float* x, int ldx,
                               const dm_mlp_params* p, const float* acts, const float* dout, const dm_mlp_grads* g,
                               float* dx, int lddx, int dx_accum, void* ws, size_t ws_bytes, void* stream) {
  DM_REQUIRE(x && p && acts && dout && g && ws, DM_E_NULL, "mlp_head_bwd: null pointer");
  DmPrecisionScope prec(p->precision);
  DM_REQUIRE(layers >= 1 && layers <= DM_MAX_MLP_LAYERS, DM_E_SHAPE, "mlp: layers=%d", layers);
  hipStream_t st = (hipStream_t)stream;
  MlpActs a;
  mlp_carve(rows, hidden, layers, const_cast<float*>(acts), &a);
  DmArena ar(ws, ws_bytes);
  float* splitk = ar.take(DM_SPLITK_FLOATS);
  float* dy = ar.take((size_t)rows * hidden);
  float* dxp = ar.take((size_t)rows * hidden);
  const bool normed = p->ln_g[0] != nullptr;
  const bool panel = normed && dm_panel_ok(rows, hidden) && ((uintptr_t)p->w[layers] & 15) == 0;
  const int npanels = dm_panel_count(rows);
  float* colpart = ar.take(panel ? (size_t)layers * npanels * 3 * hidden : 0);
  float* wt = (panel && dm_cur_precision()) ? ar.take((size_t)hidden * hidden) : nullptr;
  DM_REQUIRE(ar.ok, DM_E_WORKSPACE, "mlp_head_bwd: workspace too small (need %zu floats)", ar.off);
  const unsigned short* wth[DM_MAX_MLP_LAYERS] = {};
  if (panel && dm_cur_precision() && (hidden & 7) == 0 && layers > 1) {
    const float* src[DM_MAX_MLP_LAYERS];
    unsigned short* dst[DM_MAX_MLP_LAYERS];
    int rws[DM_MAX_MLP_LAYERS], cls[DM_MAX_MLP_LAYERS];
    for (int l = 1; l < layers; ++l) {
      src[l - 1] = p->w[l]; rws[l - 1] = hidden; cls[l - 1] = hidden;
      dst[l - 1] = (unsigned short*)ar.take(((size_t)hidden * hidden + 1) / 2);
    }
    if (ar.ok) {
      DM_TRY(dm_panel_bf16_weights_launch(layers - 1, src, dst, rws, cls, 1, st));
      for (int l = 1; l < layers; ++l) wth[l] = dst[l - 1];
    }
  }
  const size_t skb = DM_SPLITK_FLOATS * sizeof(float);

  if (panel) {
    {
      DmGemm q;
      q.a_layout = 1; q.b_layout = 1;
      q.M = out_dim; q.N = hidden; q.K = rows;
      q.A = dout; q.lda = out_dim;
      q.B = a.y[layers - 1]; q.ldb = hidden;
      q.C = g->w[layers]; q.ldc = hidden;
      DM_TRY(dm_gemm_launch(q, splitk, skb, st));
      DM_TRY(dm_colsum_launch(rows, out_dim, dout, out_dim, g->b[layers], splitk, skb, st));
    }
    float* cur = dxp;
    float* other = dy;
    DM_TRY(dm_panel_ln_bwd_launch(rows, hidden, out_dim, dout, out_dim, p->w[layers], a.xpre[layers - 1],
                                  a.stats[layers - 1], p->ln_g[layers - 1], p->ln_b[layers - 1], cur,
                                  colpart + (size_t)(layers - 1) * npanels * 3 * hidden, nullptr, st));
    for (int l = layers - 1; l >= 0; --l) {
      const float* in = l == 0 ? x : a.y[l - 1];
      const int ldin = l == 0 ? ldx : hidden;
      const int kin = l == 0 ? in_dim : hidden;
      DmGemm q;
      q.a_layout = 1; q.b_layout = 1;
      q.M = hidden; q.N = kin; q.K = rows;
      q.A = cur; q.lda = hidden;
      q.B = in; q.ldb = ldin;
      q.C = g->w[l]; q.ldc = kin;
      DM_TRY(dm_gemm_launch(q, splitk, skb, st));
      if (l > 0) {
        DM_TRY(dm_panel_ln_bwd_launch(rows, hidden, hidden, cur, hidden, p->w[l], a.xpre[l - 1], a.stats[l - 1],
                                      p->ln_g[l - 1], p->ln_b[l - 1], other, colpart + (size_t)(l - 1) * npanels * 3 * hidden,
                                      wt, st, wth[l]));
        float* t = cur; cur = other; other = t;
      } else if (dx) {
        DmGemm d;
        d.a_layout = 0; d.b_layout = 1;
        d.M = rows; d.N = kin; d.K = hidden;
        d.A = cur; d.lda = hidden;
        d.B = p->w[0]; d.ldb = kin;
        d.C = dx; d.ldc = lddx; d.flags = dx_accum ? DM_GEMM_ACCUM : 0;
        DM_TRY(dm_gemm_launch(d, splitk, skb, st));
      }
    }
    const float* parts[3 * DM_MAX_MLP_LAYERS];
    float* outs[3 * DM_MAX_MLP_LAYERS];
    for (int l = 0; l < layers; ++l) {
      const float* base = colpart + (size_t)l * npanels * 3 * hidden;
      parts[3 * l + 0] = base;              outs[3 * l + 0] = g->b[l];
      parts[3 * l + 1] = base + hidden;     outs[3 * l + 1] = g->ln_g[l];
      parts[3 * l + 2] = base + 2 * hidden; outs[3 * l + 2] = g->ln_b[l];
    }
    return dm_panel_colsum_final_launch(3 * layers, parts, outs, hidden, npanels, 3 * hidden, st);
  }

  {
    DmGemm q;
    q.a_layout = 1; q.b_layout = 1;
    q.M = out_dim; q.N = hidden; q.K = rows;
    q.A = dout; q.lda = out_dim;
    q.B = a.y[layers - 1]; q.ldb = hidden;
    q.C = g->w[layers]; q.ldc = hidden;
    DM_TRY(dm_gemm_launch(q, splitk, skb, st));
    DM_TRY(dm_colsum_launch(rows, out_dim, dout, out_dim, g->b[layers], splitk, skb, st));
    DmGemm d;
    d.a_layout = 0; d.b_layout = 1;
    d.M = rows; d.N = hidden; d.K = out_dim;
    d.A = dout; d.lda = out_dim;
    d.B = p->w[layers]; d.ldb = hidden;
    d.C = dy; d.ldc = hidden;
    DM_TRY(dm_gemm_launch(d, splitk, skb, st));
  }
  for (int l = layers - 1; l >= 0; --l) {
    const float* in = l == 0 ? x : a.y[l - 1];
    const int ldin = l == 0 ? ldx : hidden;
    const int kin = l == 0 ? in_dim : hidden;
    if (normed) {
      DM_TRY(dm_ln_elu_bwd_dx_launch(rows, hidden, a.xpre[l], hidden, a.y[l], hidden, a.stats[l], p->ln_g[l], dy, hidden,
                                     dxp, hidden, st));
      DM_TRY(dm_ln_elu_bwd_params_launch(rows, hidden, a.xpre[l], hidden, a.y[l], hidden, a.stats[l], dy, hidden,
                                         g->ln_g[l], g->ln_b[l], splitk, skb, st));
    } else {
      DM_TRY(dm_elu_bwd_launch(rows, hidden, a.y[l], hidden, dy, hidden, dxp, hidden, st));
    }
    DmGemm q;
    q.a_layout = 1; q.b_layout = 1;
    q.M = hidden; q.N = kin; q.K = rows;
    q.A = dxp; q.lda = hidden;
    q.B = in; q.ldb = ldin;
    q.C = g->w[l]; q.ldc = kin;
    DM_TRY(dm_gemm_launch(q, splitk, skb, st));
    DM_TRY(dm_colsum_launch(rows, hidden, dxp, hidden, g->b[l], splitk, skb, st));
    if (l > 0 || dx) {
      DmGemm d;
      d.a_layout = 0; d.b_layout = 1;
      d.M = rows; d.N = kin; d.K = hidden;
      d.A = dxp; d.lda = hidden;
      d.B = p->w[l]; d.ldb = kin;
      if (l > 0) { d.C = dy; d.ldc = hidden; }
      else { d.C = dx; d.ldc = lddx; d.flags = dx_accum ? DM_GEMM_ACCUM : 0; }
      DM_TRY(dm_gemm_launch(d, splitk, skb, st));
    }
  }
  return DM_OK;
}
```

### pydreamer_amd/csrc/rssm.hip

```cpp
#include "common.h"

static inline int rssm_gru_kind(const dm_shape* s) { return (s->flags & DM_FLAG_GRU_MASK) >> DM_FLAG_GRU_SHIFT; }
static inline int rssm_gru_layers(const dm_shape* s) {
  return 1 + ((s->flags & DM_FLAG_GRU_LAYERS_MASK) >> DM_FLAG_GRU_LAYERS_SHIFT);
}
struct RssmDims {
  int T, B, N, D, Hd, S, C, Z, ZP, F, E, A, kind, layers;
  bool gauss;
};
static void rssm_dims(const dm_shape* s, RssmDims* d) {
  d->T = s->T; d->B = s->B; d->N = s->T * s->B; d->D = s->D; d->Hd = s->Hd; d->S = s->S; d->C = s->C;
  d->Z = s->S * (s->C ? s->C : 1); d->ZP = s->S * (s->C ? s->C : 2); d->F = d->D + d->Z; d->E = s->E; d->A = s->A;
  d->gauss = s->C == 0; d->kind = rssm_gru_kind(s); d->layers = rssm_gru_layers(s);
}

struct RssmActs {
  float *ea, *ee, *hin, *zin, *x1, *st1, *za, *gi, *gh, *x2, *st2, *pin, *x3, *st3, *prin;
  float *gs, *gst;
};
static size_t rssm_carve(const RssmDims& d, float* base, RssmActs* a) {
  const size_t N = (size_t)d.T * d.B, Hd = d.Hd, D = d.D, Z = d.Z;
  DmArena ar(base, (size_t)1 << 62);
  RssmActs t;
  t.ea = ar.take(N * Hd); t.ee = ar.take(N * Hd);
  t.hin = ar.take(N * D); t.zin = ar.take(N * Z);
  t.x1 = ar.take(N * Hd); t.st1 = ar.take(N * 2); t.za = ar.take(N * Hd);
  t.gi = ar.take(N * 3 * D); t.gh = ar.take(N * 3 * D);
  t.x2 = ar.take(N * Hd); t.st2 = ar.take(N * 2); t.pin = ar.take(N * Hd);
  t.x3 = ar.take(N * Hd); t.st3 = ar.take(N * 2); t.prin = ar.take(N * Hd);
  t.gs = ar.take(d.kind ? N * 3 * D : 0); t.gst = ar.take(d.kind ? N * 6 * d.layers : 0);
  if (a) *a = t;
  return ar.off;
}
extern "C" size_t dm_rssm_acts_floats(const dm_shape* shp) {
  if (!shp) return 0;
  RssmDims d;
  rssm_dims(shp, &d);
  return rssm_carve(d, nullptr, nullptr);
}

static int rssm_check(const dm_shape* s) {
  DM_REQUIRE(s->I == 1, DM_E_SHAPE, "rssm: iwae_samples=%d unsupported (only 1)", s->I);
  DM_REQUIRE(s->T >= 1 && s->B >= 1 && s->D >= 4 && s->Hd >= 4 && s->S >= 1 && (s->C >= 2 || s->C == 0) && s->A >= 1 && s->E >= 1,
             DM_E_SHAPE, "rssm: bad shape");
  DM_REQUIRE((s->D & 3) == 0, DM_E_SHAPE, "rssm: deter_dim must be a multiple of 4 (got %d)", s->D);
  DM_REQUIRE(rssm_gru_kind(s) <= 2, DM_E_SHAPE, "rssm: unknown recurrent cell kind %d", rssm_gru_kind(s));
  const int GL = rssm_gru_layers(s);
  DM_REQUIRE(s->D % (4 * GL) == 0, DM_E_SHAPE, "rssm: deter_dim=%d must be a multiple of 4*gru_layers (%d)", s->D, 4 * GL);
  return DM_OK;
}

struct GruStack {
  int L, ls, kind;
  const float *wih[4], *whh[4], *bih[4], *bhh[4];
  float *g_wih[4], *g_whh[4], *g_bih[4], *g_bhh[4];
  const float *lng[4][3], *lnb[4][3];
  float *g_lng[4][3], *g_lnb[4][3];
};
static int gru_stack(const dm_shape* s, const float* const* p, float* const* g, GruStack* k) {
  k->L = rssm_gru_layers(s);
  k->ls = s->D / k->L;
  k->kind = rssm_gru_kind(s);
  for (int i = 0; i < k->L; ++i) {
    const int lb = i == 0 ? DM_RSSM_GRU_LN_G0 : DM_RSSM_GRU_L1_LN_G0 + 6 * (i - 1);
    for (int q = 0; q < 3; ++q) {
      k->lng[i][q] = p[lb + 2 * q]; k->lnb[i][q] = p[lb + 2 * q + 1];
      k->g_lng[i][q] = g ? g[lb + 2 * q] : nullptr; k->g_lnb[i][q] = g ? g[lb + 2 * q + 1] : nullptr;
      const bool need = k->kind == 1 || (k->kind == 2 && q == 0);
      DM_REQUIRE(!need || (k->lng[i][q] && k->lnb[i][q]), DM_E_NULL, "rssm: LayerNorm GRU layer %d without LayerNorm parameter %d",
                 i, q);
      DM_REQUIRE(!need || !g || (k->g_lng[i][q] && k->g_lnb[i][q]), DM_E_NULL,
                 "rssm: LayerNorm GRU layer %d without LayerNorm gradient slot %d", i, q);
    }
    const int b = i == 0 ? DM_RSSM_GRU_WIH : DM_RSSM_GRU_L1_WIH + 4 * (i - 1);
    k->wih[i] = p[b]; k->whh[i] = p[b + 1]; k->bih[i] = p[b + 2]; k->bhh[i] = p[b + 3];
    const bool biased = rssm_gru_kind(s) == 0;
    DM_REQUIRE(k->wih[i] && k->whh[i] && (!biased || (k->bih[i] && k->bhh[i])), DM_E_NULL,
               "rssm: GRU layer %d has a null parameter", i);
    if (g) {
      k->g_wih[i] = g[b]; k->g_whh[i] = g[b + 1]; k->g_bih[i] = g[b + 2]; k->g_bhh[i] = g[b + 3];
      DM_REQUIRE(k->g_wih[i] && k->g_whh[i] && (!biased || (k->g_bih[i] && k->g_bhh[i])), DM_E_NULL,
                 "rssm: GRU layer %d has a null gradient slot", i);
    }
  }
  return DM_OK;
}

static int norm_elu_fwd(int rows, int n, const float* x, int ldx, const float* gamma, const float* beta, float eps, float* y,
                        int ldy, float* stats, hipStream_t st) {
  if (gamma) return dm_ln_elu_fwd_launch(rows, n, x, ldx, gamma, beta, eps, y, ldy, stats, st);
  return dm_elu_fwd_launch(rows, n, x, ldx, y, ldy, st);
}
static int norm_elu_bwd_dx(int rows, int n, const float* x, int ldx, const float* y, int ldy, const float* stats,
                           const float* gamma, const float* dy, int lddy, float* dx, int lddx, hipStream_t st) {
  if (gamma) return dm_ln_elu_bwd_dx_launch(rows, n, x, ldx, y, ldy, stats, gamma, dy, lddy, dx, lddx, st);
  return dm_elu_bwd_launch(rows, n, y, ldy, dy, lddy, dx, lddx, st);
}
static int norm_elu_bwd_params(int rows, int n, const float* x, int ldx, const float* y, int ldy, const float* stats,
                               const float* dy, int lddy, float* dgamma, float* dbeta, void* ws, size_t ws_bytes,
                               hipStream_t st) {
  if (!dgamma && !dbeta) return DM_OK;
  return dm_ln_elu_bwd_params_launch(rows, n, x, ldx, y, ldy, stats, dy, lddy, dgamma, dbeta, ws, ws_bytes, st);
}

static DmGemm linear_q(int rows, int nout, int kin, const float* x, int ldx, const float* W, const float* bias,
                       const float* add, int ldadd, float* y, int ldy) {
  DmGemm q;
  q.M = rows; q.N = nout; q.K = kin;
  q.A = x; q.lda = ldx;
  q.B = W; q.ldb = kin;
  q.C = y; q.ldc = ldy;
  q.bias = bias; q.add = add; q.ldadd = ldadd;
  return q;
}
static int linear(hipStream_t st, void* sk, size_t skb, int rows, int nout, int kin, const float* x, int ldx,
                  const float* W, const float* bias, const float* add, int ldadd, float* y, int ldy) {
  return dm_gemm_launch(linear_q(rows, nout, kin, x, ldx, W, bias, add, ldadd, y, ldy), sk, skb, st);
}
static int wgrad(hipStream_t st, void* sk, size_t skb, int rows, int nout, int kin, const float* dy, int lddy,
                 const float* x, int ldx, float* dW, int accum = 0) {
  DmGemm q;
  q.a_layout = 1; q.b_layout = 1;
  q.M = nout; q.N = kin; q.K = rows;
  q.A = dy; q.lda = lddy;
  q.B = x; q.ldb = ldx;
  q.C = dW; q.ldc = kin;
  q.flags = accum ? DM_GEMM_ACCUM : 0;
  return dm_gemm_launch(q, sk, skb, st);
}
static int dgrad(hipStream_t st, void* sk, size_t skb, int rows, int nout, int kin, const float* dy, int lddy,
                 const float* W, float* dx, int lddx, int accum, const uint8_t* row_zero) {
  DmGemm q;
  q.a_layout = 0; q.b_layout = 1;
  q.M = rows; q.N = kin; q.K = nout;
  q.A = dy; q.lda = lddy;
  q.B = W; q.ldb = kin;
  q.C = dx; q.ldc = lddx;
  q.flags = accum ? DM_GEMM_ACCUM : 0;
  q.row_zero = row_zero;
  return dm_gemm_launch(q, sk, skb, st);
}

static DmGemm dgrad_t_q(int rows, int nout, int kin, const float* dy, int lddy, const float* Wt, float* dx, int lddx,
                        int accum, const uint8_t* row_zero) {
  DmGemm q;
  q.M = rows; q.N = kin; q.K = nout;
  q.A = dy; q.lda = lddy;
  q.B = Wt; q.ldb = nout;
  q.C = dx; q.ldc = lddx;
  q.flags = accum ? DM_GEMM_ACCUM : 0;
  q.row_zero = row_zero;
  return q;
}
static int dgrad_t(hipStream_t st, void* sk, size_t skb, int rows, int nout, int kin, const float* dy, int lddy,
                   const float* Wt, float* dx, int lddx, int accum, const uint8_t* row_zero) {
  return dm_gemm_launch(dgrad_t_q(rows, nout, kin, dy, lddy, Wt, dx, lddx, accum, row_zero), sk, skb, st);
}
static int transpose(hipStream_t st, const float* W, float* Wt, int rows, int cols) {
  return dm_permute4_launch(W, Wt, 1, 1, rows, cols, 0, 1, 3, 2, st);
}

static int gru_stack_fwd(hipStream_t st, void* sk, size_t skb, const GruStack& k, int rows, int Hd, int D, const float* x0,
                         const float* hin, int ldh, float* gi, float* gh, float* hout, int ldo, float* h_next,
                         const uint8_t* next_reset, float* gs, float* gst) {
  const int ls = k.ls;
  for (int i = 0; i < k.L; ++i) {
    const float* x = i == 0 ? x0 : hout + (size_t)(i - 1) * ls;
    const int ldx = i == 0 ? Hd : ldo, kin = i == 0 ? Hd : ls;
    DM_TRY(linear(st, sk, skb, rows, 3 * ls, kin, x, ldx, k.wih[i], k.bih[i], nullptr, 0, gi + 3 * ls * i, 3 * D));
    DM_TRY(linear(st, sk, skb, rows, 3 * ls, ls, hin + i * ls, ldh, k.whh[i], k.bhh[i], nullptr, 0, gh + 3 * ls * i, 3 * D));
    if (k.kind == 0)
      DM_TRY(dm_gru_gates_fwd_launch(rows, ls, gi + 3 * ls * i, gh + 3 * ls * i, hin + i * ls, ldh, hout + i * ls, ldo,
                                     h_next ? h_next + i * ls : nullptr, next_reset, nullptr, nullptr, st, 3 * D, D));
    else
      DM_TRY(dm_gru_norm_fwd_launch(k.kind, rows, ls, gi + 3 * ls * i, gh + 3 * ls * i, hin + i * ls, ldh, k.lng[i], k.lnb[i],
                                    hout + i * ls, ldo, gs + 3 * ls * i, gst + 6 * i, h_next ? h_next + i * ls : nullptr,
                                    next_reset, st, 3 * D, 6 * k.L, D));
  }
  return DM_OK;
}

static thread_local int tl_last_schedule[3] = {0, 0, 0};
extern "C" int dm_rssm_last_schedule(int which) { return which >= 0 && which < 3 ? tl_last_schedule[which] : -1; }

struct PostCtx : RssmDims {
  RssmActs a; GruStack gk;
  const float* const* p; hipStream_t st; void* ws; size_t skb;
  const uint8_t* reset; const float* u; const int32_t* forced; float *feat, *post; int32_t* idx;
  bool fuse_ln, fuse_sample;
  float* wzt;
  float *zinf, *x1f, *hinf, *hf, *x2f;
  float* psync; size_t psync_floats;

  int plan(size_t ws_bytes) {
    const bool stacked = gk.L > 1;
    const bool normed = p[DM_RSSM_IN_G] != nullptr;
    DM_REQUIRE((p[DM_RSSM_POST_G] != nullptr) == normed && (p[DM_RSSM_PRIOR_G] != nullptr) == normed, DM_E_NULL,
               "rssm: the cell's three norms must be all LayerNorm or all NoNorm");
    fuse_ln = normed && !stacked && !gauss && dm_skinny_ln_ok(B, 3 * D, Hd) && dm_skinny_ln_ok(B, ZP, Hd) &&
              (ZP >= 64 * 1024 / Hd);
    fuse_sample = fuse_ln && C == 32 && (Z & 31) == 0 && (F & 3) == 0 && (D & 3) == 0 &&
                  (((uintptr_t)feat | (uintptr_t)a.zin) & 15) == 0;
    DmArena ar(ws, ws_bytes);
    ar.take(DM_SPLITK_FLOATS);
    if (!gauss && idx && T > 1 && dm_z_embed_ok(Hd)) {
      const size_t mark = ar.off;
      float* w = ar.take((size_t)Z * Hd);
      if (ar.ok) wzt = w;
      else { ar.off = mark; ar.ok = true; }
    }
    if (fuse_sample && kind == 0 && B <= 64) {
      float* f0 = ar.take(dm_frag_floats(Z)); float* f1 = ar.take(dm_frag_floats(Hd)); float* f2 = ar.take(dm_frag_floats(D));
      float* f3 = ar.take(dm_frag_floats(D)); float* f4 = ar.take(dm_frag_floats(Hd));
      if (ar.ok) { zinf = f0; x1f = f1; hinf = f2; hf = f3; x2f = f4; }
    }
    if (normed && !stacked && !gauss && kind == 0 && wzt && idx && (F & 3) == 0 && T >= 3 && dm_rssm_lds_ok(B, D, Hd, S, C)) {
      psync_floats = dm_rssm_lds_ws_floats(B, D, Hd, S, C, T - 1);
      float* sy = ar.take(psync_floats);
      if (ar.ok) psync = sy;
      else ar.ok = true;
    }
    return DM_OK;
  }

  float* hin_next(int t) const { return t + 1 < T ? a.hin + (size_t)(t + 1) * B * D : nullptr; }
  float* zin_next(int t) const { return t + 1 < T ? a.zin + (size_t)(t + 1) * B * Z : nullptr; }
  const uint8_t* reset_next(int t) const { return t + 1 < T ? reset + (size_t)(t + 1) * B : nullptr; }

  int post_x1(int t, bool ln_z) const {
    const size_t r0 = (size_t)t * B;
    if (ln_z)
      return dm_z_embed_launch(B, Hd, S, C, idx + (r0 - B) * S, reset + r0, wzt, p[DM_RSSM_Z_B], a.ea + r0 * Hd, Hd, nullptr,
                               nullptr, a.x1 + r0 * Hd, Hd, nullptr, p[DM_RSSM_IN_G], p[DM_RSSM_IN_B], 1e-3f, a.za + r0 * Hd, Hd,
                               st, x1f, a.st1 + r0 * 2);
    if (wzt && t > 0)
      return dm_z_embed_launch(B, Hd, S, C, idx + (r0 - B) * S, reset + r0, wzt, p[DM_RSSM_Z_B], a.ea + r0 * Hd, Hd, nullptr,
                               nullptr, a.x1 + r0 * Hd, Hd, x1f, nullptr, nullptr, 0.f, nullptr, 0, st);
    DmGemm q = linear_q(B, Hd, Z, a.zin + r0 * Z, Z, p[DM_RSSM_Z_W], p[DM_RSSM_Z_B], a.ea + r0 * Hd, Hd, a.x1 + r0 * Hd, Hd);
    q.A_frag = zinf; q.C_frag = x1f;
    return dm_gemm_launch(q, ws, skb, st);
  }
  int post_cell(int t, bool prologue) const {
    const size_t r0 = (size_t)t * B;
    const float* hin = a.hin + r0 * D;
    DmGemm gi_q = linear_q(B, 3 * D, Hd, (prologue ? a.x1 : a.za) + r0 * Hd, Hd, p[DM_RSSM_GRU_WIH], p[DM_RSSM_GRU_BIH], nullptr, 0,
                           a.gi + r0 * 3 * D, 3 * D);
    if (prologue) { gi_q.ln_g = p[DM_RSSM_IN_G]; gi_q.ln_b = p[DM_RSSM_IN_B]; gi_q.ln_eps = 1e-3f; }
    gi_q.A_frag = x1f;
    DmGemm gh_q = linear_q(B, 3 * D, D, hin, D, p[DM_RSSM_GRU_WHH], p[DM_RSSM_GRU_BHH], nullptr, 0, a.gh + r0 * 3 * D, 3 * D);
    gh_q.A_frag = hinf;
    DM_TRY(dm_gemm_pair_launch(gi_q, gh_q, ws, skb, st));
    if (kind == 0)
      return dm_gru_gates_fwd_launch(B, D, a.gi + r0 * 3 * D, a.gh + r0 * 3 * D, hin, D, feat + r0 * F, F, hin_next(t),
                                     reset_next(t), hf, t + 1 < T ? hinf : nullptr, st);
    return dm_gru_norm_fwd_launch(kind, B, D, a.gi + r0 * 3 * D, a.gh + r0 * 3 * D, hin, D, gk.lng[0], gk.lnb[0], feat + r0 * F, F,
// ... 167 lines not shown
    dx1s = fuse_b ? dx1_w : dx1;
    const int ls = gk.ls;
    int n = 0;
    wg[n++] = {dpost, ZP, ZP, a.pin, Hd, Hd, g[DM_RSSM_POST_W]};
    wg[n++] = {dx2s, Hd, Hd, feat, F, D, g[DM_RSSM_POST_H_W]};
    wg[n++] = {dx2s, Hd, Hd, embed, E, E, g[DM_RSSM_POST_E_W]};
    for (int i = 0; i < gk.L; ++i) {
      wg[n++] = {dgi + 3 * ls * i, 3 * D, 3 * ls, i == 0 ? a.za : feat + (size_t)(i - 1) * ls, i == 0 ? Hd : F, i == 0 ? Hd : ls,
                 gk.g_wih[i]};
      wg[n++] = {dgh + 3 * ls * i, 3 * D, 3 * ls, a.hin + i * ls, D, ls, gk.g_whh[i]};
    }
    wg[n++] = {dx1s, Hd, Hd, a.zin, Z, Z, g[DM_RSSM_Z_W]};
    wg[n++] = {dx1s, Hd, Hd, action, A, A, g[DM_RSSM_A_W]};
    nwg = n;
    return DM_OK;
  }
  int wgrads(int first, int count, size_t c0, int rows, int accum) const {
    for (const Wgrad* w = wg + first; w < wg + first + count; ++w)
      DM_TRY(wgrad(sw, sk_w, skb, rows, w->nout, w->kin, w->dy + c0 * w->lddy, w->lddy, w->x + c0 * w->ldx, w->ldx, w->dW, accum));
    return DM_OK;
  }
  int side_chunk(int t) {
    if (gk.L > 1 || next_chunk < 0 || t != (int)((long long)T * next_chunk / nchunk)) return DM_OK;
    const int k = next_chunk--;
    const int t0 = (int)((long long)T * k / nchunk), t1 = (int)((long long)T * (k + 1) / nchunk);
    const size_t c0 = (size_t)t0 * B;
    const int rows = (t1 - t0) * B;
    DM_TRY(dm_wgrad_side_fork(st, sw));
    if (fuse_b) {
      DM_TRY(post_norm_bwd(c0, rows, dx2_w, sw));
      DM_TRY(in_norm_bwd(c0, rows, dx1_w, sw));
    }
    return wgrads(0, nwg, c0, rows, k != nchunk - 1);
  }
  int post_norm_bwd(size_t c0, int rows, float* dx, hipStream_t s) const {
    return norm_elu_bwd_dx(rows, Hd, a.x2 + c0 * Hd, Hd, a.pin + c0 * Hd, Hd, a.st2 + c0 * 2, p[DM_RSSM_POST_G], dpin + c0 * Hd, Hd,
                           dx + c0 * Hd, Hd, s);
  }
  int in_norm_bwd(size_t c0, int rows, float* dx, hipStream_t s) const {
    return norm_elu_bwd_dx(rows, Hd, a.x1 + c0 * Hd, Hd, a.za + c0 * Hd, Hd, a.st1 + c0 * 2, p[DM_RSSM_IN_G], dza + c0 * Hd, Hd,
                           dx + c0 * Hd, Hd, s);
  }

  struct Rows { size_t r0; float *dft, *dpt, *dprev; const uint8_t* rz; };
  Rows rows_of(int t) const {
    const size_t r0 = (size_t)t * B;
    return {r0, dfeat + r0 * F, dpost + r0 * ZP, t > 0 ? dfeat + (r0 - B) * F : nullptr, reset + r0};
  }
  DmGemm dprev_h(const Rows& r) const {
    DmGemm q = dgrad_t_q(B, 3 * D, D, dgh + r.r0 * 3 * D, 3 * D, wt_hh, r.dprev, F, 1, r.rz);
    q.A_frag = dghf;
    return q;
  }
  struct Ln {
    const float *x, *stats, *gamma, *beta;
    float *dy, *gx, *frag, *ps;
    const float *xw, *cs; int ldxw;
  };
  DmGemm make_dy(const Ln& n, bool folded, int K, const float* A_, const float* A_frag, const float* Wt) const {
    DmGemm q = dgrad_t_q(B, K, Hd, A_, K, Wt, n.dy, Hd, 0, nullptr);
    q.A_frag = A_frag;
    if (folded) {
      q.eg_x = n.x; q.eg_ldx = Hd; q.eg_stats = n.stats; q.eg_gamma = n.gamma; q.eg_beta = n.beta;
      q.eg_G = n.gx; q.eg_ldg = Hd; q.eg_Gf = n.frag; q.eg_ps = n.ps;
    } else {
      q.C_frag = n.frag;
    }
    return q;
  }
  DmGemm use_dx(const Ln& n, bool folded, int N_, const float* Wt, float* C_, const uint8_t* rz) const {
    DmGemm q = dgrad_t_q(B, Hd, N_, folded ? n.gx : n.dy, Hd, Wt, C_, F, 1, rz);
    q.A_frag = n.frag;
    if (folded) {
      q.lnf_ps = n.ps; q.lnf_nps = nstrip; q.lnf_stats = n.stats; q.lnf_xw = n.xw; q.lnf_ldxw = n.ldxw; q.lnf_cs = n.cs;
    } else {
      q.ln_g = n.gamma; q.ln_b = n.beta; q.lnb_x = n.x; q.lnb_ldx = Hd; q.lnb_stats = n.stats;
    }
    return q;
  }

  int bptt_step_fused(int t) const {
    const Rows r = rows_of(t);
    const size_t r0 = r.r0;
    const Ln post_n = {a.x2 + r0 * Hd, a.st2 + r0 * 2, p[DM_RSSM_POST_G], p[DM_RSSM_POST_B], dpin + r0 * Hd, dx2 + r0 * Hd, dpinf,
                       eps2, fold ? xw2 + r0 * D : nullptr, cs2, D};
    const Ln in_n = {a.x1 + r0 * Hd, a.st1 + r0 * 2, p[DM_RSSM_IN_G], p[DM_RSSM_IN_B], dza + r0 * Hd, dx1 + r0 * Hd, dzaf,
                     eps1, fold ? xwz + r0 * Z : nullptr, csz, Z};
    if (!(fold_sm && t < T - 1)) DM_TRY(dm_st_softmax_bwd_launch(B, S, C, post + r0 * ZP, ZP, r.dft + D, F, r.dpt, ZP, 1, st));
    DM_TRY(dm_gemm_launch(make_dy(post_n, fold, ZP, r.dpt, nullptr, wt_post), sk, skb, st));
    DmGatesBwd gb;
    gb.gi = a.gi + r0 * 3 * D; gb.gh = a.gh + r0 * 3 * D; gb.h_in = a.hin + r0 * D; gb.ldh = D; gb.D = D;
    gb.dgi = dgi + r0 * 3 * D; gb.dgh = dgh + r0 * 3 * D; gb.dprev = r.dprev; gb.ldp = F; gb.row_zero = r.rz;
    gb.dgi_frag = dgif; gb.dgh_frag = dghf;
    DmGemm q4 = use_dx(post_n, fold, D, wt_post_h, r.dft, nullptr);
    q4.gates = &gb;
    DM_TRY(dm_gemm_launch(q4, sk, skb, st));
    DM_TRY(dm_gemm_launch(make_dy(in_n, fold, 3 * D, dgi + r0 * 3 * D, dgif, wt_ih), sk, skb, st));
    if (t == 0) return DM_OK;
    DmGemm qz = use_dx(in_n, fold, Z, wt_z, r.dprev + D, r.rz);
    if (fold_sm) { qz.sm_logits = post + (r0 - B) * ZP; qz.sm_ld = ZP; qz.sm_dlogits = dpost + (r0 - B) * ZP; qz.sm_ldd = ZP; }
    return dm_gemm_pair_launch(dprev_h(r), qz, sk, skb, st);
  }

  int post_branch(const Rows& r) const {
    const size_t r0 = r.r0;
    if (gauss) DM_TRY(dm_gauss_sample_bwd_launch(B, S, post + r0 * ZP, ZP, feat + r0 * F + D, F, r.dft + D, F, r.dpt, ZP, 1, st));
    else DM_TRY(dm_st_softmax_bwd_launch(B, S, C, post + r0 * ZP, ZP, r.dft + D, F, r.dpt, ZP, 1, st));
    DM_TRY(dgrad_t(st, sk, skb, B, ZP, Hd, r.dpt, ZP, wt_post, dpin + r0 * Hd, Hd, 0, nullptr));
    DM_TRY(post_norm_bwd(r0, B, dx2, st));
    return dgrad_t(st, sk, skb, B, Hd, D, dx2 + r0 * Hd, Hd, wt_post_h, r.dft, F, 1, nullptr);
  }
  int bptt_step_single(int t) const {
    const Rows r = rows_of(t);
    const size_t r0 = r.r0;
    DM_TRY(post_branch(r));
    if (kind == 0)
      DM_TRY(dm_gru_gates_bwd_launch(B, D, a.gi + r0 * 3 * D, a.gh + r0 * 3 * D, a.hin + r0 * D, D, r.dft, F, dgi + r0 * 3 * D,
                                     dgh + r0 * 3 * D, r.dprev, F, 1, r.rz, st));
    else
      DM_TRY(dm_gru_norm_bwd_launch(kind, B, D, a.gh + r0 * 3 * D, a.hin + r0 * D, D, a.gs + r0 * 3 * D, a.gst + r0 * 6, gk.lng[0],
                                    gk.lnb[0], r.dft, F, dgi + r0 * 3 * D, dgh + r0 * 3 * D, dgl + r0 * 3 * D, r.dprev, F, r.rz, st));
    DM_TRY(dgrad_t(st, sk, skb, B, 3 * D, Hd, dgi + r0 * 3 * D, 3 * D, wt_ih, dza + r0 * Hd, Hd, 0, nullptr));
    DM_TRY(in_norm_bwd(r0, B, dx1, st));
    if (t == 0) return DM_OK;
    return dm_gemm_pair_launch(dprev_h(r), dgrad_t_q(B, Hd, Z, dx1 + r0 * Hd, Hd, wt_z, r.dprev + D, F, 1, r.rz), sk, skb, st);
  }
  int bptt_step_stacked(int t) const {
    const Rows r = rows_of(t);
    const size_t r0 = r.r0;
    const int ls = gk.ls;
    float* dprev = r.dprev;
    DM_TRY(post_branch(r));
    for (int i = gk.L - 1; i >= 0; --i) {
      float* dgi_i = dgi + r0 * 3 * D + 3 * ls * i;
      float* dgh_i = dgh + r0 * 3 * D + 3 * ls * i;
      if (kind == 0)
        DM_TRY(dm_gru_gates_bwd_launch(B, ls, a.gi + r0 * 3 * D + 3 * ls * i, a.gh + r0 * 3 * D + 3 * ls * i,
                                       a.hin + r0 * D + i * ls, D, r.dft + i * ls, F, dgi_i, dgh_i,
                                       dprev ? dprev + i * ls : nullptr, F, 1, r.rz, st, 3 * D));
      else
        DM_TRY(dm_gru_norm_bwd_launch(kind, B, ls, a.gh + r0 * 3 * D + 3 * ls * i, a.hin + r0 * D + i * ls, D,
                                      a.gs + r0 * 3 * D + 3 * ls * i, a.gst + r0 * 6 * gk.L + 6 * i, gk.lng[i], gk.lnb[i],
                                      r.dft + i * ls, F, dgi_i, dgh_i, dgl + r0 * 3 * D + 3 * ls * i,
                                      dprev ? dprev + i * ls : nullptr, F, r.rz, st, 3 * D, 6 * gk.L));
      if (i > 0) DM_TRY(dgrad(st, sk, skb, B, 3 * ls, ls, dgi_i, 3 * D, gk.wih[i], r.dft + (i - 1) * ls, F, 1, nullptr));
      else DM_TRY(dgrad(st, sk, skb, B, 3 * ls, Hd, dgi_i, 3 * D, gk.wih[0], dza + r0 * Hd, Hd, 0, nullptr));
      if (dprev) DM_TRY(dgrad(st, sk, skb, B, 3 * ls, ls, dgh_i, 3 * D, gk.whh[i], dprev + i * ls, F, 1, r.rz));
    }
    DM_TRY(in_norm_bwd(r0, B, dx1, st));
    if (dprev) DM_TRY(dgrad_t(st, sk, skb, B, Hd, Z, dx1 + r0 * Hd, Hd, wt_z, dprev + D, F, 1, r.rz));
    return DM_OK;
  }

  int cell_param_grads(int i) const {
    const int ls = gk.ls;
    if (kind == 0) {
      DM_TRY(dm_colsum_launch(N, 3 * ls, dgi + 3 * ls * i, 3 * D, gk.g_bih[i], sk_w, skb, sw));
      return dm_colsum_launch(N, 3 * ls, dgh + 3 * ls * i, 3 * D, gk.g_bhh[i], sk_w, skb, sw);
    }
    DM_TRY(dm_gru_norm_param_grads_launch(kind, N, ls, a.gs + 3 * ls * i, a.gst + 6 * i, dgl + 3 * ls * i, lnpg, lnpb, sw, 3 * D,
                                          6 * gk.L));
    const int parts = kind == 1 ? 3 : 1;
    const size_t len = (size_t)(kind == 1 ? ls : 3 * ls) * sizeof(float);
    for (int q = 0; q < parts; ++q)
      if (hipMemcpyAsync(gk.g_lng[i][q], lnpg + (size_t)q * ls, len, hipMemcpyDeviceToDevice, sw) != hipSuccess ||
          hipMemcpyAsync(gk.g_lnb[i][q], lnpb + (size_t)q * ls, len, hipMemcpyDeviceToDevice, sw) != hipSuccess)
        return dm_fail(DM_E_HIP, "rssm_sequence_bwd: gradient copy failed");
    return DM_OK;
  }
  int param_tail() const {
    const int L = gk.L;
    const bool stacked = L > 1;
    if (stacked) DM_TRY(dm_wgrad_side_fork(st, sw));
    DM_TRY(dm_colsum_launch(N, ZP, dpost, ZP, g[DM_RSSM_POST_OB], sk_w, skb, sw));
    DM_TRY(norm_elu_bwd_params(N, Hd, a.x2, Hd, a.pin, Hd, a.st2, dpin, Hd, g[DM_RSSM_POST_G], g[DM_RSSM_POST_B], sk_w, skb, sw));
    DM_TRY(dm_colsum_launch(N, Hd, dx2s, Hd, g[DM_RSSM_POST_H_B], sk_w, skb, sw));
    if (stacked) DM_TRY(wgrads(0, 3, 0, N, 0));
    for (int i = 0; i < L; ++i) {
      if (stacked) DM_TRY(wgrads(3 + 2 * i, 2, 0, N, 0));
      DM_TRY(cell_param_grads(i));
    }
    DM_TRY(norm_elu_bwd_params(N, Hd, a.x1, Hd, a.za, Hd, a.st1, dza, Hd, g[DM_RSSM_IN_G], g[DM_RSSM_IN_B], sk_w, skb, sw));
    DM_TRY(dm_colsum_launch(N, Hd, dx1s, Hd, g[DM_RSSM_Z_B], sk_w, skb, sw));
    if (stacked) DM_TRY(wgrads(3 + 2 * L, 2, 0, N, 0));
    return dm_wgrad_side_mark(sw, st);
  }
};

extern "C" int dm_rssm_sequence_bwd(const dm_shape* s, const float* embed, const float* action, const uint8_t* reset,
                                    const dm_rssm_params* P, const float* acts, const float* feat, const float* post,
                                    float* dfeat, float* dpost, float* dprior, const dm_rssm_grads* G, float* dembed,
                                    void* ws, size_t ws_bytes, void* stream) {
  DM_REQUIRE(s && embed && action && reset && P && acts && feat && post && dfeat && dpost && dprior && G && ws, DM_E_NULL,
             "rssm_sequence_bwd: null pointer");
  DmPrecisionScope prec(s->flags & DM_FLAG_BF16);
  DM_TRY(rssm_check(s));
  BpttCtx c = {};
  rssm_dims(s, &c);
  rssm_carve(c, const_cast<float*>(acts), &c.a);
  c.p = P->p; c.g = G->p; c.st = (hipStream_t)stream; c.sw = dm_wgrad_side_stream(c.st);
  c.embed = embed; c.action = action; c.feat = feat; c.post = post; c.reset = reset; c.dfeat = dfeat; c.dpost = dpost;
  DM_TRY(gru_stack(s, c.p, c.g, &c.gk));
  DM_TRY(c.plan(ws, ws_bytes));
  tl_last_schedule[1] = (c.fuse_b ? DM_SCHED_BWD_FUSE_B : 0) | (c.fold ? DM_SCHED_BWD_FOLD : 0) | (c.fold_sm ? DM_SCHED_BWD_FOLD_SM : 0) |
                        (c.dgif ? DM_SCHED_BWD_FRAG : 0) | (c.nchunk << DM_SCHED_BWD_NCHUNK_SHIFT);
  const RssmActs& a = c.a;
  const float* const* p = c.p;
  float* const* g = c.g;
  const int N = c.N, D = c.D, Hd = c.Hd, Z = c.Z, ZP = c.ZP, F = c.F;
  hipStream_t st = c.st, sw = c.sw;
  float *sk = c.sk, *sk_w = c.sk_w;
  const size_t skb = c.skb;

  DM_TRY(dgrad(st, sk, skb, N, ZP, Hd, dprior, ZP, p[DM_RSSM_PRIOR_W], c.dprin, Hd, 0, nullptr));
  DM_TRY(norm_elu_bwd_dx(N, Hd, a.x3, Hd, a.prin, Hd, a.st3, p[DM_RSSM_PRIOR_G], c.dprin, Hd, c.dx3, Hd, st));
  DM_TRY(dgrad(st, sk, skb, N, Hd, D, c.dx3, Hd, p[DM_RSSM_PRIOR_H_W], dfeat, F, 1, nullptr));
  DM_TRY(dm_wgrad_side_fork(st, sw));
  DM_TRY(wgrad(sw, sk_w, skb, N, ZP, Hd, dprior, ZP, a.prin, Hd, g[DM_RSSM_PRIOR_W]));
  DM_TRY(dm_colsum_launch(N, ZP, dprior, ZP, g[DM_RSSM_PRIOR_OB], sk_w, skb, sw));
  DM_TRY(norm_elu_bwd_params(N, Hd, a.x3, Hd, a.prin, Hd, a.st3, c.dprin, Hd, g[DM_RSSM_PRIOR_G], g[DM_RSSM_PRIOR_B], sk_w, skb, sw));
  DM_TRY(wgrad(sw, sk_w, skb, N, Hd, D, c.dx3, Hd, feat, F, g[DM_RSSM_PRIOR_H_W]));
  DM_TRY(dm_colsum_launch(N, Hd, c.dx3, Hd, g[DM_RSSM_PRIOR_H_B], sk_w, skb, sw));

  DM_TRY(transpose(st, p[DM_RSSM_POST_W], c.wt_post, ZP, Hd));
  DM_TRY(transpose(st, p[DM_RSSM_POST_H_W], c.wt_post_h, Hd, D));
  if (c.gk.L == 1) {
    DM_TRY(transpose(st, p[DM_RSSM_GRU_WIH], c.wt_ih, 3 * D, Hd));
    DM_TRY(transpose(st, p[DM_RSSM_GRU_WHH], c.wt_hh, 3 * D, D));
  }
  DM_TRY(transpose(st, p[DM_RSSM_Z_W], c.wt_z, Hd, Z));
  if (c.fold) {
    DM_TRY(dgrad(st, sk, skb, N, Hd, D, a.x2, Hd, p[DM_RSSM_POST_H_W], c.xw2, D, 0, nullptr));
    DM_TRY(dgrad(st, sk, skb, N, Hd, Z, a.x1, Hd, p[DM_RSSM_Z_W], c.xwz, Z, 0, nullptr));
    DM_TRY(dm_colsum_launch(Hd, D, p[DM_RSSM_POST_H_W], D, c.cs2, sk, skb, st));
    DM_TRY(dm_colsum_launch(Hd, Z, p[DM_RSSM_Z_W], Z, c.csz, sk, skb, st));
  }
  for (int t = c.T - 1; t >= 0; --t) {
    DM_TRY(c.fuse_b ? c.bptt_step_fused(t) : c.gk.L > 1 ? c.bptt_step_stacked(t) : c.bptt_step_single(t));
    DM_TRY(c.side_chunk(t));
  }
  if (c.fuse_b) DM_TRY(c.post_norm_bwd(0, N, c.dx2, st));
  if (dembed) DM_TRY(dgrad(st, sk, skb, N, Hd, c.E, c.dx2, Hd, p[DM_RSSM_POST_E_W], dembed, c.E, 0, nullptr));
  return c.param_tail();
}

static thread_local int tl_marks_n = 0;
static thread_local int tl_mark_step[4];
static thread_local hipEvent_t tl_mark_ev[4];
extern "C" int dm_dream_rollout_marks(int n, const int* steps, void* const* events) {
  DM_REQUIRE(n >= 0 && n <= 4 && (n == 0 || (steps && events)), DM_E_SHAPE, "dream_rollout_marks: n=%d (0..4)", n);
  for (int i = 0; i < n; ++i) {
    DM_REQUIRE(events[i], DM_E_NULL, "dream_rollout_marks: null event %d", i);
    tl_mark_step[i] = steps[i];
    tl_mark_ev[i] = (hipEvent_t)events[i];
  }
  tl_marks_n = n;
  return DM_OK;
}
struct DmRolloutMarks {
  int n;
  bool done[4] = {false, false, false, false};
  hipStream_t caller;
  explicit DmRolloutMarks(hipStream_t st) : n(tl_marks_n), caller(st) { tl_marks_n = 0; }
  void at_step(int i, hipStream_t st, bool eager) {
    if (!eager) return;
    for (int k = 0; k < n; ++k)
      if (!done[k] && tl_mark_step[k] == i) { (void)hipEventRecord(tl_mark_ev[k], st); done[k] = true; }
  }
  ~DmRolloutMarks() {
    for (int k = 0; k < n; ++k)
      if (!done[k]) (void)hipEventRecord(tl_mark_ev[k], caller);
  }
};

static int g_rollout_fuse_act = 1;
extern "C" int dm_rollout_fuse_act_enable(int on) {
  if (on >= 0) g_rollout_fuse_act = on ? 1 : 0;
  return g_rollout_fuse_act;
}

struct RolloutCtx : RssmDims {
  GruStack gk;
  int M, H, Hm, L, adist, AO;
  const float* const* p; const dm_mlp_params* actor; hipStream_t st; float* sk; size_t skb;
  const float *u_act, *u_prior; float *feats, *actions; int32_t* act_idx; float *actor_acts, *actor_logits;
  float *macts, *logits_ws, *ea, *x1, *za, *stats, *gi, *gh, *prior, *gsw, *gstw;
  bool tw_on;
  unsigned short *wih_h, *whh_h, *wph_h, *wp_h, *za_h, *feats_h;
  float *wzt, *wat; int32_t *pidx, *aidx;
  float *actor_wpack, *actor_w0t, *actor_add0;
  bool fuse_act;

  int plan(void* ws, size_t ws_bytes) {
    DmArena ar(ws, ws_bytes);
    sk = ar.take(DM_SPLITK_FLOATS);
    macts = ar.take(actor_acts ? 0 : dm_mlp_acts_floats(M, Hm, L)); logits_ws = ar.take(actor_acts ? 0 : (size_t)M * AO);
    ea = ar.take((size_t)M * Hd); x1 = ar.take((size_t)M * Hd); za = ar.take((size_t)M * Hd); stats = ar.take((size_t)M * 2);
    gi = ar.take((size_t)M * 3 * D); gh = ar.take((size_t)M * 3 * D); prior = ar.take((size_t)M * ZP);
    gsw = ar.take(kind ? (size_t)M * 3 * D : 0); gstw = ar.take(kind ? (size_t)M * 6 * layers : 0);
    tw_on = dm_twins_on() && kind == 0 && layers == 1 && p[DM_RSSM_IN_G] && p[DM_RSSM_PRIOR_G] && (F & 7) == 0;
    wih_h = (unsigned short*)ar.take(tw_on ? dm_half_floats((size_t)3 * D * Hd) : 0);
    whh_h = (unsigned short*)ar.take(tw_on ? dm_half_floats((size_t)3 * D * D) : 0);
    wph_h = (unsigned short*)ar.take(tw_on ? dm_half_floats((size_t)Hd * D) : 0);
    wp_h = (unsigned short*)ar.take(tw_on ? dm_half_floats((size_t)ZP * Hd) : 0);
    za_h = (unsigned short*)ar.take(tw_on ? dm_half_floats((size_t)M * Hd) : 0);
    feats_h = (unsigned short*)ar.take(tw_on ? dm_half_floats((size_t)(H + 1) * M * F) : 0);
    DM_REQUIRE(ar.ok, DM_E_WORKSPACE, "dream_rollout: workspace too small (need %zu floats)", ar.off);
    skb = DM_SPLITK_FLOATS * sizeof(float);
    if (C != 0 && H > 1 && dm_z_embed_ok(Hd)) {
      const size_t mark = ar.off;
      float* w = ar.take((size_t)Z * Hd);
      float* w2 = ar.take((size_t)A * Hd);
      int32_t* ix = reinterpret_cast<int32_t*>(ar.take((size_t)M * S));
      int32_t* ax = reinterpret_cast<int32_t*>(ar.take((size_t)M));
      if (ar.ok) {
        wzt = w; pidx = ix;
        if (adist == 0) { wat = w2; aidx = ax; }
      } else {
        ar.off = mark; ar.ok = true;
      }
    }
    if (dm_mlp_chain_ok(M, F, Hm, L, AO, feats, F, actor) && !dm_panel_ok(M, Hm)) {
      float* wpk = ar.take(dm_mlp_chain_pack_floats(F, L));
      if (ar.ok) {
        actor_wpack = wpk;
        if (C != 0 && pidx && dm_mlp_chain_sparse_ok(F, Z) && dm_z_embed_ok(Hm)) {
          const size_t mark = ar.off;
          float* wt = ar.take((size_t)F * Hm);
          float* ad = ar.take((size_t)M * Hm);
          if (ar.ok) { actor_w0t = wt; actor_add0 = ad; }
          else { ar.off = mark; ar.ok = true; }
        }
      }
    }
    fuse_act = adist == 0 && actor_wpack && g_rollout_fuse_act;
    return DM_OK;
  }

  int32_t* act_idx_of(int i) const { return act_idx ? act_idx + (size_t)i * M : aidx; }

  int rollout_actor(int i) const {
    const float* cur = feats + (size_t)i * M * F;
    float* act = actions + (size_t)i * M * A;
    const bool keep = actor_acts != nullptr;
    float* logits = keep ? actor_logits + (size_t)i * M * AO : logits_ws;
    if (actor_add0) {
      if (i == 0) DM_TRY(dm_sparse_rows_launch(M, Hm, Z, cur + D, F, actor_w0t + (size_t)D * Hm, actor_add0, Hm, st));
      else DM_TRY(dm_z_embed_launch(M, Hm, S, C, pidx, nullptr, actor_w0t + (size_t)D * Hm, nullptr, nullptr, 0, nullptr, nullptr,
                                    actor_add0, Hm, nullptr, nullptr, nullptr, 0.f, nullptr, 0, st));
    }
    int32_t* ai = act_idx_of(i);
    const DmChainSample samp = {u_act + (size_t)i * M, act, A, ai};
    DM_TRY(dm_mlp_fwd_launch(M, F, Hm, L, AO, cur, F, actor, keep ? actor_acts : macts, keep ? H * M : M, keep ? i * M : 0, logits,
                             AO, sk, skb, st, actor_wpack, actor_add0 ? Z : 0, actor_add0, fuse_act ? &samp : nullptr));
    if (fuse_act) return DM_OK;
    if (adist == 0)
      return dm_sample_onehot_launch(M, 1, A, logits, A, u_act + (size_t)i * M, nullptr, act, A, ai, nullptr, nullptr, st);
    return dm_sample_continuous_launch(adist, M, A, logits, u_act + (size_t)i * M * A, act, st);
  }
  int rollout_cell(int i) const {
    const float* cur = feats + (size_t)i * M * F;
    float* nxt = feats + (size_t)(i + 1) * M * F;
    const float* act = actions + (size_t)i * M * A;
    const int32_t* ai = act_idx_of(i);
    const bool embed = wzt && i > 0, embed_a = embed && wat && ai;
    if (!embed_a) DM_TRY(linear(st, sk, skb, M, Hd, A, act, A, p[DM_RSSM_A_W], nullptr, nullptr, 0, ea, Hd));
    if (embed) {
      DM_TRY(dm_z_embed_launch(M, Hd, S, C, pidx, nullptr, wzt, p[DM_RSSM_Z_B], embed_a ? nullptr : ea, Hd,
                               embed_a ? ai : nullptr, wat, nullptr, Hd, nullptr, p[DM_RSSM_IN_G], p[DM_RSSM_IN_B], 1e-3f,
                               za, Hd, st));
    } else {
      DM_TRY(linear(st, sk, skb, M, Hd, Z, cur + D, F, p[DM_RSSM_Z_W], p[DM_RSSM_Z_B], ea, Hd, x1, Hd));
      DM_TRY(norm_elu_fwd(M, Hd, x1, Hd, p[DM_RSSM_IN_G], p[DM_RSSM_IN_B], 1e-3f, za, Hd, stats, st));
    }
    if (gk.L > 1) {
// ... 68 lines not shown
```

### pydreamer_amd/hip.py

```python
import ctypes
import os
from ctypes import POINTER, Structure, c_char_p, c_float, c_int, c_int32, c_int64, c_size_t, c_void_p

import torch

_HERE = os.path.dirname(os.path.abspath(__file__))
LIB_PATH = os.environ.get('DM_LIB_PATH') or os.path.join(_HERE, 'libdreamer_hip.so')

DM_MAX_MLP_LAYERS = 8
DM_GEMM_ACCUM = 1
DM_GEMM_ELU = 2
DM_C2I_ELU = 1
DM_FLAG_IMAGE_U8 = 16
DM_FLAG_BF16 = 128
DM_GEMM_BF16 = 256

RSSM_PARAM_ORDER = [
    'z_mlp.weight', 'z_mlp.bias', 'a_mlp.weight', 'in_norm.weight', 'in_norm.bias',
    'gru.layers.0.weight_ih', 'gru.layers.0.weight_hh', 'gru.layers.0.bias_ih', 'gru.layers.0.bias_hh',
    'prior_mlp_h.weight', 'prior_mlp_h.bias', 'prior_norm.weight', 'prior_norm.bias', 'prior_mlp.weight', 'prior_mlp.bias',
    'post_mlp_h.weight', 'post_mlp_h.bias', 'post_mlp_e.weight', 'post_norm.weight', 'post_norm.bias',
    'post_mlp.weight', 'post_mlp.bias',
]
GRU_KINDS = {'gru': 0, 'gru_layernorm': 1, 'gru_layernorm_dv2': 2}
DM_FLAG_GRU_SHIFT = 5
_LN_SLOTS = {
    'gru': [None] * 6,
    'gru_layernorm': ['ln_reset.weight', 'ln_reset.bias', 'ln_update.weight', 'ln_update.bias', 'ln_newval.weight', 'ln_newval.bias'],
    'gru_layernorm_dv2': ['lnorm.weight', 'lnorm.bias', None, None, None, None],
}


DM_FLAG_GRU_LAYERS_SHIFT = 8
SCHED_FWD = {'fuse_ln': 1, 'fuse_sample': 2, 'frag': 4, 'wzt': 8, 'psync': 16}
SCHED_BWD = {'fuse_b': 1, 'fold': 2, 'fold_sm': 4, 'frag': 8}
SCHED_BWD_NCHUNK_SHIFT = 8
SCHED_ROLL = {'wzt': 1, 'wat': 2, 'actor_wpack': 4, 'actor_add0': 8, 'fuse_act': 16, 'tw_on': 32}
DM_MAX_GRU_LAYERS = 4


def rssm_param_names(gru_type='gru', gru_layers=1):
    names = list(RSSM_PARAM_ORDER)
    if gru_type != 'gru':
        ren = {'gru.layers.0.weight_ih': 'gru.layers.0.weight_ih.weight', 'gru.layers.0.weight_hh': 'gru.layers.0.weight_hh.weight',
               'gru.layers.0.bias_ih': None, 'gru.layers.0.bias_hh': None}
        names = [ren.get(n, n) for n in names]
    ln = lambda i: [n and f'gru.layers.{i}.{n}' for n in _LN_SLOTS[gru_type]]
    names = names + ln(0)
    cell = ('weight_ih', 'weight_hh', 'bias_ih', 'bias_hh') if gru_type == 'gru' else ('weight_ih.weight', 'weight_hh.weight', None, None)
    for i in range(1, DM_MAX_GRU_LAYERS):
        names += [f'gru.layers.{i}.{n}' if (n and i < gru_layers) else None for n in cell]
    for i in range(1, DM_MAX_GRU_LAYERS):
        names += ln(i) if i < gru_layers else [None] * 6
    return names


DM_RSSM_NPARAMS = len(RSSM_PARAM_ORDER) + 6 + (4 + 6) * (DM_MAX_GRU_LAYERS - 1)


class DreamerHipError(RuntimeError):
    pass


class dm_shape(Structure):
    _fields_ = [(n, c_int32) for n in ('T', 'B', 'I', 'H', 'D', 'Hd', 'S', 'C', 'E', 'A', 'mlp_hidden', 'mlp_layers',
                                       'cnn_depth', 'img', 'img_ch', 'flags')]


class dm_mlp_params(Structure):
    _fields_ = [('w', c_void_p * (DM_MAX_MLP_LAYERS + 1)), ('b', c_void_p * (DM_MAX_MLP_LAYERS + 1)),
                ('ln_g', c_void_p * DM_MAX_MLP_LAYERS), ('ln_b', c_void_p * DM_MAX_MLP_LAYERS),
                ('precision', c_int32), ('reserved_', c_int32)]


class dm_mlp_grads(Structure):
    _fields_ = [('w', c_void_p * (DM_MAX_MLP_LAYERS + 1)), ('b', c_void_p * (DM_MAX_MLP_LAYERS + 1)),
                ('ln_g', c_void_p * DM_MAX_MLP_LAYERS), ('ln_b', c_void_p * DM_MAX_MLP_LAYERS)]


class dm_conv_params(Structure):
    _fields_ = [('w', c_void_p * 5), ('b', c_void_p * 5)]


dm_conv_grads = dm_conv_params


class dm_rssm_params(Structure):
    _fields_ = [('p', c_void_p * DM_RSSM_NPARAMS)]


dm_rssm_grads = dm_rssm_params


class dm_reduce_item(Structure):
    _fields_ = [('x', c_void_p), ('n', c_int64), ('scale', c_float), ('mode', c_int32), ('center', c_void_p)]


class dm_replay_field(Structure):
    _fields_ = [('dst', c_void_p), ('row_bytes', c_int64), ('is_reset', c_int32), ('reserved_', c_int32)]


DM_REPLAY_MAX_FIELDS = 16


class dm_gru_params(Structure):
    _fields_ = [('w_ih', c_void_p), ('w_hh', c_void_p), ('b_ih', c_void_p), ('b_hh', c_void_p)]


dm_gru_grads = dm_gru_params


def gru_struct(w_ih, w_hh, b_ih, b_hh):
    s = dm_gru_params()
    s.w_ih, s.w_hh, s.b_ih, s.b_hh = w_ih.data_ptr(), w_hh.data_ptr(), b_ih.data_ptr(), b_hh.data_ptr()
    return s

_P = c_void_p
_SIGNATURES = {
    'dm_version': (c_int, []),
    'dm_last_error': (c_char_p, []),
    'dm_device_check': (c_int, []),
    'dm_workspace_bytes': (c_size_t, [POINTER(dm_shape)]),
    'dm_stream_create_cu_mask': (c_int, [_P, c_int, POINTER(c_void_p)]),
    'dm_stream_destroy': (c_int, [_P]),
    'dm_gemm_f32': (c_int, [c_int, c_int, c_int, c_int, c_int, _P, c_int, _P, c_int, _P, c_int, _P, _P, c_int, c_int,
                            _P, c_size_t, _P]),
    'dm_gemm_bf16h': (c_int, [c_int, c_int, c_int, c_int, c_int, _P, c_int, _P, c_int, _P, c_int, _P, _P, c_int, _P, c_size_t, _P]),
    'dm_ln_elu_fwd': (c_int, [c_int, c_int, _P, c_int, _P, _P, c_float, _P, c_int, _P, _P]),
    'dm_ln_elu_bwd': (c_int, [c_int, c_int, _P, c_int, _P, c_int, _P, _P, _P, c_int, _P, c_int, _P, _P, _P, c_size_t, _P]),
    'dm_colsum': (c_int, [c_int, c_int, _P, c_int, _P, _P, c_size_t, _P]),
    'dm_gru_gates_fwd': (c_int, [c_int, c_int, _P, _P, _P, c_int, _P, c_int, _P]),
    'dm_gru_gates_bwd': (c_int, [c_int, c_int, _P, _P, _P, c_int, _P, c_int, _P, _P, _P, c_int, _P]),
    'dm_sample_onehot': (c_int, [c_int, c_int, c_int, _P, c_int, _P, _P, _P, c_int, _P, _P]),
    'dm_kl_balance_fwd': (c_int, [c_int, c_int, c_int, _P, _P, _P, _P, _P, _P]),
    'dm_kl_balance_bwd': (c_int, [c_int, c_int, c_int, _P, _P, c_float, c_float, _P, _P, _P]),
    'dm_st_softmax_bwd': (c_int, [c_int, c_int, c_int, _P, c_int, _P, c_int, _P, c_int, c_int, _P]),
    'dm_mask_rows': (c_int, [c_int, c_int, _P, c_int, _P, _P, c_int, _P]),
    'dm_kl_sampled_fwd': (c_int, [c_int, c_int, c_int, _P, _P, _P, _P, _P]),
    'dm_kl_sampled_bwd': (c_int, [c_int, c_int, c_int, _P, _P, _P, c_float, _P, _P, _P, _P]),
    'dm_kl_sampled_gauss_fwd': (c_int, [c_int, c_int, _P, _P, _P, c_int, _P, _P]),
    'dm_kl_sampled_gauss_bwd': (c_int, [c_int, c_int, _P, _P, _P, c_int, c_float, _P, _P, _P, _P, c_int, _P]),
    'dm_reduce_i': (c_int, [c_int, c_int, c_int, _P, c_int, _P, _P, _P]),
    'dm_combine_rows': (c_int, [c_int, c_int64, POINTER(c_void_p), POINTER(c_float), _P, _P]),
    'dm_scale_rows': (c_int, [c_int64, c_int, _P, c_int, _P, c_float, _P]),
    'dm_im2col_s2': (c_int, [c_int, c_int, c_int, c_int, c_int, _P, c_int, _P, _P]),
    'dm_col2im_s2': (c_int, [c_int, c_int, c_int, c_int, c_int, _P, _P, c_int, _P, _P, _P]),
    'dm_mlp_acts_floats': (c_size_t, [c_int, c_int, c_int]),
    'dm_mlp_ws_floats': (c_size_t, [c_int, c_int, c_int]),
    'dm_mlp_head_fwd': (c_int, [c_int, c_int, c_int, c_int, c_int, _P, c_int, POINTER(dm_mlp_params), _P, _P, _P,
                                c_size_t, _P]),
    'dm_mlp_head_fwd_sparse': (c_int, [c_int, c_int, c_int, c_int, c_int, c_int, _P, c_int, POINTER(dm_mlp_params), _P, _P, _P, c_size_t, _P]),
    'dm_mlp_head_bwd': (c_int, [c_int, c_int, c_int, c_int, c_int, _P, c_int, POINTER(dm_mlp_params), _P, _P,
                                POINTER(dm_mlp_grads), _P, c_int, c_int, _P, c_size_t, _P]),
    'dm_head_loss': (c_int, [c_int, c_int, _P, _P, c_float, c_float, _P, _P, _P, _P]),
    'dm_head_loss_normal_nd': (c_int, [c_int, c_int, _P, _P, c_float, c_float, _P, _P, _P, _P]),
    'dm_cat_target_index': (c_int, [c_int, c_int, c_int, _P, _P, _P]),
    'dm_cat_image_loss': (c_int, [c_int, c_int, c_int, c_int, _P, c_int, _P, _P, _P, _P]),
    'dm_cat_image_pred': (c_int, [c_int, c_int, c_int, c_int, _P, c_int, _P, _P, _P, _P, _P, _P]),
    'dm_cat_concat_rows': (c_int, [c_int, c_int, c_int, c_int, _P, c_int, _P, _P, _P]),
    'dm_dense_image_rows': (c_int, [c_int, c_int, c_int, _P, _P, _P, _P, _P, c_int, _P]),
    'dm_elu_rows_fwd': (c_int, [c_int, c_int, _P, c_int, _P, c_int, _P]),
    'dm_elu_rows_bwd': (c_int, [c_int, c_int, _P, c_int, _P, c_int, _P, c_int, _P]),
    'dm_cat_image_loss_mix': (c_int, [c_int, c_int, c_int, c_int, _P, c_int, _P, c_float, _P, _P, _P]),
    'dm_goals_stats_ws_floats': (c_size_t, [c_int, c_int]),
    'dm_goals_stats': (c_int, [c_int, c_int, _P, _P, _P, _P, _P, c_size_t, _P]),
    'dm_preprocess_image_u8': (c_int, [c_int64, c_int, c_int, _P, _P, _P]),
    'dm_conv_encoder_acts_floats': (c_size_t, [POINTER(dm_shape)]),
    'dm_conv_encoder_fwd': (c_int, [POINTER(dm_shape), _P, POINTER(dm_conv_params), _P, _P, _P, c_size_t, _P]),
    'dm_conv_encoder_bwd': (c_int, [POINTER(dm_shape), _P, POINTER(dm_conv_params), _P, _P, POINTER(dm_conv_grads), _P,
                                    c_size_t, _P]),
    'dm_conv_encoder_fwd_planes': (c_int, [POINTER(dm_shape), _P, POINTER(dm_conv_params), _P, _P, _P, _P, c_int, _P, c_size_t, _P]),
    'dm_conv_encoder_bwd_planes': (c_int, [POINTER(dm_shape), _P, POINTER(dm_conv_params), _P, _P, _P, _P, c_int,
                                           POINTER(dm_conv_grads), _P, c_size_t, _P]),
    'dm_conv_decoder_acts_floats': (c_size_t, [POINTER(dm_shape)]),
    'dm_conv_decoder_pred_offset': (c_size_t, [POINTER(dm_shape)]),
    'dm_conv_decoder_mse_fwd': (c_int, [POINTER(dm_shape), _P, c_int, _P, POINTER(dm_conv_params), _P, _P, _P, _P,
                                        c_size_t, _P]),
    'dm_conv_decoder_mse_bwd': (c_int, [POINTER(dm_shape), _P, c_int, _P, POINTER(dm_conv_params), _P, c_float,
                                        POINTER(dm_conv_grads), _P, c_int, _P, c_size_t, _P]),
    'dm_conv_decoder_mse_bwd_rows': (c_int, [POINTER(dm_shape), _P, c_int, _P, POINTER(dm_conv_params), _P, c_float, _P,
                                             POINTER(dm_conv_grads), _P, c_int, _P, c_size_t, _P]),
    'dm_rssm_acts_floats': (c_size_t, [POINTER(dm_shape)]),
    'dm_rssm_sequence_fwd': (c_int, [POINTER(dm_shape), _P, _P, _P, _P, _P, _P, _P, POINTER(dm_rssm_params), _P, _P, _P,
                                     _P, _P, _P, c_size_t, _P]),
    'dm_rssm_sequence_bwd': (c_int, [POINTER(dm_shape), _P, _P, _P, POINTER(dm_rssm_params), _P, _P, _P, _P, _P, _P,
                                     POINTER(dm_rssm_grads), _P, _P, c_size_t, _P]),
    'dm_dream_rollout': (c_int, [POINTER(dm_shape), c_int, _P, POINTER(dm_rssm_params), POINTER(dm_mlp_params), _P, _P,
                                 _P, _P, _P, _P, _P, _P, c_size_t, _P]),
    'dm_gae_losses': (c_int, [c_int, c_int, c_float, c_float, _P, _P, _P, _P, _P, _P, _P, _P]),
    'dm_actor_loss': (c_int, [c_int, c_int, _P, _P, _P, _P, c_float, c_float, _P, _P, _P, _P]),
    'dm_critic_loss': (c_int, [c_int, _P, _P, _P, c_float, _P, _P, _P]),
    'dm_sample_continuous': (c_int, [c_int, c_int, c_int, _P, _P, _P, _P]),
    'dm_actor_loss_continuous': (c_int, [c_int, c_int, c_int, _P, _P, _P, _P, c_float, c_float, _P, _P, _P, _P]),
    'dm_multi_sum': (c_int, [c_int, POINTER(dm_reduce_item), _P, _P]),
    'dm_combine': (c_int, [c_int, _P, POINTER(c_float), _P, _P]),
    'dm_multi_tensor_norm_clip': (c_int, [_P, c_int64, c_float, _P, _P, c_size_t, _P]),
    'dm_scale_inplace': (c_int, [_P, c_int64, _P, _P]),
    'dm_adamw_step': (c_int, [_P, _P, _P, _P, c_int64, c_float, c_float, c_float, c_float, c_float, c_int, _P, _P]),
    'dm_copy_params': (c_int, [_P, _P, c_int64, _P]),
    'dm_axpby': (c_int, [c_int64, c_float, _P, c_float, _P, _P]),
    'dm_prof_begin': (c_int, [c_int]),
    'dm_prof_end': (c_int, [POINTER(ctypes.c_double), c_int]),
    'dm_prof_rows': (c_int, [POINTER(ctypes.c_double), c_int]),
    'dm_mlp_chain_min_rows': (c_int, [c_int]),
    'dm_rollout_fuse_act_enable': (c_int, [c_int]),
    'dm_bf16_twins_enable': (c_int, [c_int]),
    'dm_gemm_dma_enable': (c_int, [c_int]),
    'dm_dec_l4_bwd_direct_enable': (c_int, [c_int]),
    'dm_rssm_lds_enable': (c_int, [c_int]),
    'dm_bptt_fold_enable': (c_int, [c_int]),
    'dm_rssm_lds_status': (c_int, []),
    'dm_rssm_lds_status_ack': (c_int, []),
    'dm_rssm_lds_gave_up': (c_int, []),
    'dm_rssm_lds_prof': (c_int, [_P, c_int]),
    'dm_rssm_last_schedule': (c_int, [c_int]),
    'dm_wgrad_side_arm': (c_int, [c_int]),
    'dm_wgrad_side_touch': (c_int, []),
    'dm_wgrad_side_join': (c_int, [_P]),
    'dm_dream_rollout_marks': (c_int, [c_int, POINTER(c_int), POINTER(c_void_p)]),
    'dm_mlp_head_fwd_rows': (c_int, [c_int, c_int, c_int, c_int, c_int, c_int, c_int, c_int, _P, c_int, POINTER(dm_mlp_params), _P, _P, _P,
                                     c_size_t, _P]),
    'dm_replay_gather': (c_int, [c_int, c_int, c_int, POINTER(dm_replay_field), _P, _P, _P]),
    'dm_gru_sequence_acts_floats': (c_size_t, [c_int, c_int, c_int, c_int]),
    'dm_gru_sequence_ws_bytes': (c_size_t, [c_int, c_int, c_int, c_int]),
    'dm_gru_sequence_fwd': (c_int, [c_int, c_int, c_int, c_int, _P, c_int, _P, _P, POINTER(dm_gru_params), _P, _P, c_int,
                                    _P, c_size_t, _P]),
    'dm_gru_sequence_bwd': (c_int, [c_int, c_int, c_int, c_int, _P, c_int, POINTER(dm_gru_params), _P, _P, c_int, _P, c_int,
                                    POINTER(dm_gru_grads), _P, c_int, _P, c_size_t, _P]),
    'dm_gru_sequence_last_schedule': (c_int, []),
    'dm_gru_sequence_fuse_enable': (c_int, [c_int]),
}

_lib = None
DM_ABI_VERSION = 16


def lib():
    global _lib
    if _lib is None:
        if not os.path.exists(LIB_PATH):
            raise DreamerHipError(
                f'{LIB_PATH} not found: build it with `python -c "import __graft_entry__ as g; g.build()"` '
                f'(or `make -C pydreamer_amd/csrc`). There is no CPU fallback for the training path.')
        handle = ctypes.CDLL(LIB_PATH)
        for name, (restype, argtypes) in _SIGNATURES.items():
            fn = getattr(handle, name)
            fn.restype = restype
            fn.argtypes = argtypes
        if handle.dm_version() != DM_ABI_VERSION:
            raise DreamerHipError(f'{LIB_PATH} has ABI version {handle.dm_version()}, this binding is written for '
                                  f'{DM_ABI_VERSION}: rebuild it (`make -C pydreamer_amd/csrc`)')
        _lib = handle
    return _lib


def exported_symbols():
    return sorted(_SIGNATURES)


def call(name, *args):
    fn = getattr(lib(), name)
    rc = fn(*args)
    if rc != 0:
        msg = lib().dm_last_error().decode('utf-8', 'replace')
        raise DreamerHipError(f'{name} failed with code {rc}: {msg}')
    return rc


def last_schedule(which):
    word = int(lib().dm_rssm_last_schedule(which))
    if word < 0:
        raise DreamerHipError(f'dm_rssm_last_schedule({which}): no such entry point')
    bits = (SCHED_FWD, SCHED_BWD, SCHED_ROLL)[which]
    out = {k: bool(word & v) for k, v in bits.items()}
    if which == 1:
        out['nchunk'] = (word >> SCHED_BWD_NCHUNK_SHIFT) & 15
    return out


def ptr(t):
    if t is None:
        return None
    if not t.is_cuda:
# ... 68 lines not shown
```

Measured before the change: 30.29 grad-steps/s.

## Batch bias and layernorm param-grad column sums into grouped launches; coalesce KL kernels

Adds a grouped column-sum path that packs several bias and LayerNorm gamma/beta reductions into one partial kernel and one final kernel, each using a segment table. The MLP backward and RSSM parameter tails now use it instead of issuing separate colsum and ln-params launches. This cuts kernel launch count and the idle tail between many small reductions. The grouped path shares one workspace and flushes whenever the workspace or segment limit is reached. A separate LDS-staged, coalesced KL kernel path is also added behind its own enable flag.

```diff
diff --git a/include/dreamer_hip.h b/include/dreamer_hip.h
--- a/include/dreamer_hip.h
+++ b/include/dreamer_hip.h
@@ -72,6 +72,17 @@
                   const float* gamma, const float* dy, int lddy, float* dx, int lddx,
                   float* dgamma, float* dbeta, void* ws, size_t ws_bytes, void* stream);
 int dm_colsum(int rows, int n, const float* x, int ld, float* out, void* ws, size_t ws_bytes, void* stream);
+typedef struct dm_colsum_seg {
+  int32_t mode, rows, n, ldx, ldy, lddy;
+  const float* x;
+  const float* y;
+  const float* stats;
+  const float* dy;
+  float* out0;
+  float* out1;
+} dm_colsum_seg;
+int dm_colsum_multi(const dm_colsum_seg* segs, int count, void* ws, size_t ws_bytes, void* stream);
+int dm_colsum_group_enable(int on);
 
 int dm_gru_gates_fwd(int rows, int D, const float* gi, const float* gh, const float* h_in, int ldh,
                      float* h_out, int ldo, void* stream);
@@ -85,6 +96,7 @@
                       float* kl, float* ent_post, float* ent_prior, void* stream);
 int dm_kl_balance_bwd(int rows, int S, int C, const float* post, const float* prior,
                       float scale_post, float scale_prior, float* dpost, float* dprior, void* stream);
+int dm_kl_coalesced_enable(int on);
 int dm_st_softmax_bwd(int rows, int groups, int C, const float* logits, int ldl, const float* dz, int lddz,
                       float* dlogits, int lddl, int accum, void* stream);
 
diff --git a/pydreamer_amd/csrc/common.h b/pydreamer_amd/csrc/common.h
--- a/pydreamer_amd/csrc/common.h
+++ b/pydreamer_amd/csrc/common.h
@@ -146,6 +146,18 @@
 int dm_gemm_pair_launch(const DmGemm& g0, const DmGemm& g1, void* ws, size_t ws_bytes, hipStream_t stream);
 
 int dm_colsum_launch(int rows, int n, const float* x, int ld, float* out, void* ws, size_t ws_bytes, hipStream_t st);
+enum { DM_CS_PLAIN = 0,
+       DM_CS_LN = 1 };
+struct DmColsumSeg {
+  int mode = DM_CS_PLAIN;
+  int rows = 0, n = 0;
+  const float* x = nullptr; int ldx = 0;
+  const float* y = nullptr; int ldy = 0;
+  const float* stats = nullptr;
+  const float* dy = nullptr; int lddy = 0;
+  float* out0 = nullptr; float* out1 = nullptr;
+};
+int dm_colsum_multi_launch(const DmColsumSeg* segs, int count, void* ws, size_t ws_bytes, hipStream_t st);
 int dm_elu_fwd_launch(int rows, int n, const float* x, int ldx, float* y, int ldy, hipStream_t st);
 int dm_elu_bwd_launch(int rows, int n, const float* y, int ldy, const float* dy, int lddy, float* dx, int lddx,
                       hipStream_t st);
diff --git a/pydreamer_amd/csrc/elementwise.hip b/pydreamer_amd/csrc/elementwise.hip
--- a/pydreamer_amd/csrc/elementwise.hip
+++ b/pydreamer_amd/csrc/elementwise.hip
@@ -116,16 +116,12 @@
 }
 
 template <int MODE>
-__global__ void __launch_bounds__(256) colsum_partial_kernel(int rows, int n, int rows_per_chunk,
-                                                             const float* __restrict__ x, int ldx,
-                                                             const float* __restrict__ y, int ldy,
-                                                             const float* __restrict__ stats,
-                                                             const float* __restrict__ dy, int lddy,
-                                                             float* __restrict__ partial) {
-  __shared__ float red[2][4][64];
+__device__ __forceinline__ void colsum_partial_body(int bx, int chunk, float (*red)[4][64], int rows, int n, int rows_per_chunk,
+                                                    const float* __restrict__ x, int ldx, const float* __restrict__ y, int ldy,
+                                                    const float* __restrict__ stats, const float* __restrict__ dy, int lddy,
+                                                    float* __restrict__ partial) {
   const int cx = threadIdx.x & 63, ry = threadIdx.x >> 6;
-  const int col = blockIdx.x * 64 + cx;
-  const int chunk = blockIdx.y;
+  const int col = bx * 64 + cx;
   const int r0 = chunk * rows_per_chunk;
   const int r1 = min(rows, r0 + rows_per_chunk);
   float a0 = 0.f, a1 = 0.f;
@@ -163,11 +159,20 @@
     }
   }
 }
-
-__global__ void __launch_bounds__(256) colsum_flat_kernel(long long total, int n, int W, long long chunk_elems,
-                                                          const float* __restrict__ x, float* __restrict__ partial) {
-  __shared__ float sh[256];
-  const long long base = (long long)blockIdx.x * chunk_elems;
+template <int MODE>
+__global__ void __launch_bounds__(256) colsum_partial_kernel(int rows, int n, int rows_per_chunk,
+                                                             const float* __restrict__ x, int ldx,
+                                                             const float* __restrict__ y, int ldy,
+                                                             const float* __restrict__ stats,
+                                                             const float* __restrict__ dy, int lddy,
+                                                             float* __restrict__ partial) {
+  __shared__ float red[2][4][64];
+  colsum_partial_body<MODE>(blockIdx.x, blockIdx.y, red, rows, n, rows_per_chunk, x, ldx, y, ldy, stats, dy, lddy, partial);
+}
+
+__device__ __forceinline__ void colsum_flat_body(int chunk, float* sh, long long total, int n, int W, long long chunk_elems,
+                                                 const float* __restrict__ x, float* __restrict__ partial) {
+  const long long base = (long long)chunk * chunk_elems;
   const long long end = min(total, base + chunk_elems);
   float b0 = 0.f, b1 = 0.f, b2 = 0.f, b3 = 0.f;
   if ((int)threadIdx.x < W) {
@@ -185,15 +190,20 @@
   if ((int)threadIdx.x < n) {
     float s = 0.f;
     for (int t = threadIdx.x; t < W; t += n) s += sh[t];
-    partial[(size_t)blockIdx.x * n + threadIdx.x] = s;
-  }
-}
-
-__global__ void __launch_bounds__(256) colsum_final_kernel(int n, int chunks, int nq, const float* __restrict__ partial,
-                                                           float* __restrict__ out0, float* __restrict__ out1) {
-  __shared__ float red[8][32];
+    partial[(size_t)chunk * n + threadIdx.x] = s;
+  }
+}
+__global__ void __launch_bounds__(256) colsum_flat_kernel(long long total, int n, int W, long long chunk_elems,
+                                                          const float* __restrict__ x, float* __restrict__ partial) {
+  __shared__ float sh[256];
+  colsum_flat_body(blockIdx.x, sh, total, n, W, chunk_elems, x, partial);
+}
+
+__device__ __forceinline__ void colsum_final_body(int bx, float (*red)[32], int n, int chunks, int nq,
+                                                  const float* __restrict__ partial, float* __restrict__ out0,
+                                                  float* __restrict__ out1) {
   const int cx = threadIdx.x & 31, cy = threadIdx.x >> 5;
-  const int col = blockIdx.x * 32 + cx;
+  const int col = bx * 32 + cx;
   for (int q = 0; q < nq; ++q) {
     float s = 0.f;
     if (col < n) {
@@ -217,6 +227,11 @@
     __syncthreads();
   }
 }
+__global__ void __launch_bounds__(256) colsum_final_kernel(int n, int chunks, int nq, const float* __restrict__ partial,
+                                                           float* __restrict__ out0, float* __restrict__ out1) {
+  __shared__ float red[8][32];
+  colsum_final_body(blockIdx.x, red, n, chunks, nq, partial, out0, out1);
+}
 
 static int colsum_plan(int rows, size_t budget_floats, int n, int nq, int* rows_per_chunk) {
   int chunks = dm_cdiv(rows, 64);
@@ -228,6 +243,30 @@
   return dm_cdiv(rows, *rows_per_chunk);
 }
 
+struct ColsumCut {
+  bool flat;
+  int chunks, rpc, W;
+  long long total, chunk_elems;
+};
+static ColsumCut colsum_cut(int rows, int n, int ld, size_t budget) {
+  ColsumCut c = {};
+  if (n <= 64 && ld == n && (long long)rows * n >= (1 << 16)) {
+    c.flat = true;
+    c.total = (long long)rows * n;
+    c.W = 256 - 256 % n;
+    long long want = c.total / ((long long)c.W * 16);
+    if (want > 2048) want = 2048;
+    if (want < 1) want = 1;
+    if ((size_t)want * n > budget) want = (long long)(budget / n);
+    c.chunk_elems = (c.total + want - 1) / want;
+    c.chunk_elems = (c.chunk_elems + c.W - 1) / c.W * c.W;
+    c.chunks = (int)((c.total + c.chunk_elems - 1) / c.chunk_elems);
+  } else {
+    c.chunks = colsum_plan(rows, budget, n, 1, &c.rpc);
+  }
+  return c;
+}
+
 int dm_colsum_launch(int rows, int n, const float* x, int ld, float* out, void* ws, size_t ws_bytes, hipStream_t st) {
   if (n <= 0) return DM_OK;
   if (rows <= 0) {
@@ -235,30 +274,129 @@
     return DM_OK;
   }
   DM_REQUIRE(ws && ws_bytes >= (size_t)n * sizeof(float), DM_E_WORKSPACE, "colsum: workspace too small");
+  const ColsumCut c = colsum_cut(rows, n, ld, ws_bytes / sizeof(float));
+  if (c.flat)
+    hipLaunchKernelGGL(colsum_flat_kernel, dim3(c.chunks), dim3(256), 0, st, c.total, n, c.W, c.chunk_elems, x, (float*)ws);
+  else
+    hipLaunchKernelGGL((colsum_partial_kernel<0>), dim3(dm_cdiv(n, 64), c.chunks), dim3(256), 0, st, rows, n, c.rpc, x, ld,
+                       nullptr, 0, nullptr, nullptr, 0, (float*)ws);
+  DM_LAUNCH_CHECK();
+  hipLaunchKernelGGL(colsum_final_kernel, dim3(dm_cdiv(n, 32)), dim3(256), 0, st, n, c.chunks, 1, (const float*)ws, out,
+                     nullptr);
+  DM_LAUNCH_CHECK();
+  return DM_OK;
+}
+
+constexpr int CS_MAX_SEGS = 24;
+struct CsDev {
+  const float *x, *y, *stats, *dy;
+  float* partial;
+  float *out0, *out1;
+  long long total, chunk_elems;
+  int kind;
+  int rows, n, ldx, ldy, lddy, rpc, chunks, nq, W, nbx;
+  int pstart, fstart;
+};
+struct CsArgs { CsDev s[CS_MAX_SEGS]; };
+
+__global__ void __launch_bounds__(256) colsum_multi_partial_kernel(const CsArgs a, int count) {
+  __shared__ float sm[2 * 4 * 64];
+  int si = 0;
+  for (int i = 1; i < count; ++i) si = (int)blockIdx.x >= a.s[i].pstart ? i : si;
+  const CsDev& g = a.s[si];
+  const int local = blockIdx.x - g.pstart;
+  if (g.kind == 2) {
+    colsum_flat_body(local, sm, g.total, g.n, g.W, g.chunk_elems, g.x, g.partial);
+  } else if (g.kind == 1) {
+    colsum_partial_body<1>(local % g.nbx, local / g.nbx, reinterpret_cast<float(*)[4][64]>(sm), g.rows, g.n, g.rpc, g.x, g.ldx,
+                           g.y, g.ldy, g.stats, g.dy, g.lddy, g.partial);
+  } else {
+    colsum_partial_body<0>(local % g.nbx, local / g.nbx, reinterpret_cast<float(*)[4][64]>(sm), g.rows, g.n, g.rpc, g.x, g.ldx,
+                           nullptr, 0, nullptr, nullptr, 0, g.partial);
+  }
+}
+__global__ void __launch_bounds__(256) colsum_multi_final_kernel(const CsArgs a, int count) {
+  __shared__ float red[8][32];
+  int si = 0;
+  for (int i = 1; i < count; ++i) si = (int)blockIdx.x >= a.s[i].fstart ? i : si;
+  const CsDev& g = a.s[si];
+  colsum_final_body(blockIdx.x - g.fstart, red, g.n, g.chunks, g.nq, g.partial, g.out0, g.out1);
+}
+
+static int g_colsum_group = 1;
+extern "C" int dm_colsum_group_enable(int on) {
+  if (on >= 0) g_colsum_group = on ? 1 : 0;
+  return g_colsum_group;
+}
+
+static int colsum_multi_flush(CsArgs& a, int count, int pblocks, int fblocks, hipStream_t st) {
+  if (count == 0) return DM_OK;
+  hipLaunchKernelGGL(colsum_multi_partial_kernel, dim3(pblocks), dim3(256), 0, st, a, count);
+  DM_LAUNCH_CHECK();
+  hipLaunchKernelGGL(colsum_multi_final_kernel, dim3(fblocks), dim3(256), 0, st, a, count);
+  DM_LAUNCH_CHECK();
+  return DM_OK;
+}
+
+int dm_colsum_multi_launch(const DmColsumSeg* segs, int count, void* ws, size_t ws_bytes, hipStream_t st) {
   const size_t budget = ws_bytes / sizeof(float);
-  int chunks;
-  if (n <= 64 && ld == n && (long long)rows * n >= (1 << 16)) {
-    const long long total = (long long)rows * n;
-    const int W = 256 - 256 % n;
-    long long want = total / ((long long)W * 16);
-    if (want > 2048) want = 2048;
-    if (want < 1) want = 1;
-    if ((size_t)want * n > budget) want = (long long)(budget / n);
-    long long chunk_elems = (total + want - 1) / want;
-    chunk_elems = (chunk_elems + W - 1) / W * W;
-    chunks = (int)((total + chunk_elems - 1) / chunk_elems);
-    hipLaunchKernelGGL(colsum_flat_kernel, dim3(chunks), dim3(256), 0, st, total, n, W, chunk_elems, x, (float*)ws);
-  } else {
-    int rpc;
-    chunks = colsum_plan(rows, budget, n, 1, &rpc);
-    hipLaunchKernelGGL((colsum_partial_kernel<0>), dim3(dm_cdiv(n, 64), chunks), dim3(256), 0, st, rows, n, rpc, x, ld,
-                       nullptr, 0, nullptr, nullptr, 0, (float*)ws);
-  }
-  DM_LAUNCH_CHECK();
-  hipLaunchKernelGGL(colsum_final_kernel, dim3(dm_cdiv(n, 32)), dim3(256), 0, st, n, chunks, 1, (const float*)ws, out,
-                     nullptr);
-  DM_LAUNCH_CHECK();
-  return DM_OK;
+  if (!g_colsum_group) {
+    for (int i = 0; i < count; ++i) {
+      const DmColsumSeg& q = segs[i];
+      if (q.n <= 0) continue;
+      if (q.mode == DM_CS_LN && q.rows > 0) {
+        DM_TRY(dm_ln_elu_bwd_params_launch(q.rows, q.n, q.x, q.ldx, q.y, q.ldy, q.stats, q.dy, q.lddy, q.out0, q.out1, ws, ws_bytes, st));
+      } else if (q.mode == DM_CS_LN) {
+        (void)hipMemsetAsync(q.out0, 0, (size_t)q.n * sizeof(float), st);
+        (void)hipMemsetAsync(q.out1, 0, (size_t)q.n * sizeof(float), st);
+      } else {
+        DM_TRY(dm_colsum_launch(q.rows, q.n, q.x, q.ldx, q.out0, ws, ws_bytes, st));
+      }
+    }
+    return DM_OK;
+  }
+  CsArgs a;
+  int na = 0, pblocks = 0, fblocks = 0;
+  size_t used = 0;
+  for (int i = 0; i < count; ++i) {
+    const DmColsumSeg& q = segs[i];
+    if (q.n <= 0) continue;
+    if (q.rows <= 0) {
+      (void)hipMemsetAsync(q.out0, 0, (size_t)q.n * sizeof(float), st);
+      if (q.mode == DM_CS_LN) (void)hipMemsetAsync(q.out1, 0, (size_t)q.n * sizeof(float), st);
+      continue;
+    }
+    CsDev d = {};
+    d.n = q.n; d.out0 = q.out0; d.out1 = q.out1;
+    size_t need = 0;
+    if (q.mode == DM_CS_LN) {
+      DM_REQUIRE(ws && budget >= (size_t)2 * q.n, DM_E_WORKSPACE, "colsum_multi: workspace too small");
+      d.kind = 1; d.nq = 2; d.rows = q.rows;
+      d.x = q.x; d.ldx = q.ldx; d.y = q.y; d.ldy = q.ldy; d.stats = q.stats; d.dy = q.dy; d.lddy = q.lddy;
+      d.chunks = colsum_plan(q.rows, budget, q.n, 2, &d.rpc);
+      d.nbx = dm_cdiv(q.n, 64);
+      need = (size_t)d.chunks * 2 * q.n;
+    } else {
+      DM_REQUIRE(ws && budget >= (size_t)q.n, DM_E_WORKSPACE, "colsum_multi: workspace too small");
+      const ColsumCut c = colsum_cut(q.rows, q.n, q.ldx, budget);
+      d.kind = c.flat ? 2 : 0; d.nq = 1; d.rows = q.rows; d.x = q.x; d.ldx = q.ldx;
+      d.chunks = c.chunks; d.rpc = c.rpc; d.W = c.W; d.total = c.total; d.chunk_elems = c.chunk_elems;
+      d.nbx = dm_cdiv(q.n, 64);
+      need = (size_t)c.chunks * q.n;
+    }
+    if (na == CS_MAX_SEGS || used + need > budget) {
+      DM_TRY(colsum_multi_flush(a, na, pblocks, fblocks, st));
+      na = 0; pblocks = 0; fblocks = 0; used = 0;
+    }
+    d.partial = (float*)ws + used;
+    used += dm_align_up(need, 64);
+    d.pstart = pblocks;
+    d.fstart = fblocks;
+    pblocks += d.kind == 2 ? d.chunks : d.nbx * d.chunks;
+    fblocks += dm_cdiv(q.n, 32);
+    a.s[na++] = d;
+  }
+  return colsum_multi_flush(a, na, pblocks, fblocks, st);
 }
 
 int dm_ln_elu_fwd_launch(int rows, int n, const float* x, int ldx, const float* gamma, const float* beta, float eps,
@@ -352,6 +490,20 @@
   DM_TRY(dm_ln_elu_bwd_dx_launch(rows, n, x, ldx, y, ldy, stats, gamma, dy, lddy, dx, lddx, (hipStream_t)stream));
   return dm_ln_elu_bwd_params_launch(rows, n, x, ldx, y, ldy, stats, dy, lddy, dgamma, dbeta, ws, ws_bytes,
                                      (hipStream_t)stream);
+}
+extern "C" int dm_colsum_multi(const dm_colsum_seg* segs, int count, void* ws, size_t ws_bytes, void* stream) {
+  DM_REQUIRE(segs && count >= 0 && count <= 64, DM_E_SHAPE, "colsum_multi: bad segment list");
+  DmColsumSeg sg[64];
+  for (int i = 0; i < count; ++i) {
+    const dm_colsum_seg& q = segs[i];
+    DM_REQUIRE(q.mode == DM_CS_PLAIN || q.mode == DM_CS_LN, DM_E_SHAPE, "colsum_multi: segment %d has mode %d", i, q.mode);
+    DM_REQUIRE(q.n <= 0 || (q.x && q.out0 && (q.mode == DM_CS_PLAIN || (q.y && q.stats && q.dy && q.out1))), DM_E_NULL,
+               "colsum_multi: segment %d has a null pointer", i);
+    sg[i].mode = q.mode; sg[i].rows = q.rows; sg[i].n = q.n;
+    sg[i].x = q.x; sg[i].ldx = q.ldx; sg[i].y = q.y; sg[i].ldy = q.ldy; sg[i].stats = q.stats; sg[i].dy = q.dy; sg[i].lddy = q.lddy;
+    sg[i].out0 = q.out0; sg[i].out1 = q.out1;
+  }
+  return dm_colsum_multi_launch(sg, count, ws, ws_bytes, (hipStream_t)stream);
 }
 
 extern "C" int dm_colsum(int rows, int n, const float* x, int ld, float* out, void* ws, size_t ws_bytes, void* stream) {
@@ -1331,6 +1483,121 @@
   }
 }
 
+constexpr int KL_STAGE_MAXC = 32;
+constexpr int KL_FWD_SLAB = 32;
+constexpr int KL_BWD_TILE = 128;
+__host__ __device__ constexpr int kl_pitch(int C) { return C | 1; }
+
+__device__ __forceinline__ void kl_stage_in(const float* __restrict__ g, int cnt, int C, int P, float* l, int t, int nth, bool vec) {
+  if (vec) {
+    for (int e = 4 * t; e < cnt; e += 4 * nth) {
+      const float4 v = *reinterpret_cast<const float4*>(g + e);
+      const float f[4] = {v.x, v.y, v.z, v.w};
+#pragma unroll
+      for (int j = 0; j < 4; ++j) l[((e + j) / C) * P + (e + j) % C] = f[j];
+    }
+  } else {
+    for (int e = t; e < cnt; e += nth) l[(e / C) * P + e % C] = g[e];
+  }
+}
+__device__ __forceinline__ void kl_stage_out(float* __restrict__ g, int cnt, int C, int P, const float* l, int t, int nth, bool vec) {
+  if (vec) {
+    for (int e = 4 * t; e < cnt; e += 4 * nth) {
+      float f[4];
+#pragma unroll
+      for (int j = 0; j < 4; ++j) f[j] = l[((e + j) / C) * P + (e + j) % C];
+      *reinterpret_cast<float4*>(g + e) = make_float4(f[0], f[1], f[2], f[3]);
+    }
+  } else {
+    for (int e = t; e < cnt; e += nth) g[e] = l[(e / C) * P + e % C];
+  }
+}
+
+__global__ void __launch_bounds__(256) kl_fwd_staged_kernel(int rows, int S, int C, int vec, const float* __restrict__ post,
+                                                            const float* __restrict__ prior, float* __restrict__ kl,
+                                                            float* __restrict__ ent_post, float* __restrict__ ent_prior) {
+  __shared__ float stage[4][2][KL_FWD_SLAB * kl_pitch(KL_STAGE_MAXC)];
+  const int wave = threadIdx.x >> 6, lane = threadIdx.x & 63;
+  const int row = blockIdx.x * 4 + wave;
+  const bool live = row < rows;
+  const int P = kl_pitch(C);
+  float* la_ = stage[wave][0];
+  float* lb_ = stage[wave][1];
+  float akl = 0.f, aep = 0.f, aeq = 0.f;
+  for (int s0 = 0; s0 < S; s0 += KL_FWD_SLAB) {
+    const int ng = min(KL_FWD_SLAB, S - s0);
+    if (live) {
+      kl_stage_in(post + ((size_t)row * S + s0) * C, ng * C, C, P, la_, lane, 64, vec);
+      kl_stage_in(prior + ((size_t)row * S + s0) * C, ng * C, C, P, lb_, lane, 64, vec);
+    }
+    __syncthreads();
+    const int half = (s0 / KL_FWD_SLAB) & 1;
+    const int gl = lane & 31;
+    if (live && (lane >> 5) == half && gl < ng) {
+      const float* a = la_ + gl * P;
+      const float* b = lb_ + gl * P;
+      const float la = dm_group_lse(a, C), lb = dm_group_lse(b, C);
+      float gk = 0.f, ep = 0.f, eq = 0.f;
+      for (int k = 0; k < C; ++k) {
+        const float lp = a[k] - la, lq = b[k] - lb;
+        const float p = expf(lp), q = expf(lq);
+        gk += p * (lp - lq);
+        ep -= p * lp;
+        eq -= q * lq;
+      }
+      akl += gk; aep += ep; aeq += eq;
+    }
+    __syncthreads();
+  }
+  akl = dm_wave_sum(akl); aep = dm_wave_sum(aep); aeq = dm_wave_sum(aeq);
+  if (live && lane == 0) {
+    kl[row] = akl;
+    if (ent_post) ent_post[row] = aep;
+    if (ent_prior) ent_prior[row] = aeq;
+  }
+}
+
+__global__ void __launch_bounds__(KL_BWD_TILE) kl_bwd_staged_kernel(long long total, int C, int vec, const float* __restrict__ post,
+                                                                    const float* __restrict__ prior, float sp, float sq,
+                                                                    float* __restrict__ dpost, float* __restrict__ dprior) {
+  __shared__ float stage[2][KL_BWD_TILE * kl_pitch(KL_STAGE_MAXC)];
+  const int P = kl_pitch(C);
+  const int t = threadIdx.x;
+  for (long long g0 = (long long)blockIdx.x * KL_BWD_TILE; g0 < total; g0 += (long long)gridDim.x * KL_BWD_TILE) {
+    const int ng = (int)min((long long)KL_BWD_TILE, total - g0);
+    kl_stage_in(post + (size_t)g0 * C, ng * C, C, P, stage[0], t, KL_BWD_TILE, vec);
+    kl_stage_in(prior + (size_t)g0 * C, ng * C, C, P, stage[1], t, KL_BWD_TILE, vec);
+    __syncthreads();
+    if (t < ng) {
+      float* a = stage[0] + t * P;
+      float* b = stage[1] + t * P;
+      const float la = dm_group_lse(a, C), lb = dm_group_lse(b, C);
+      float gk = 0.f;
+      for (int k = 0; k < C; ++k) {
+        const float lp = a[k] - la, lq = b[k] - lb;
+        gk += expf(lp) * (lp - lq);
+      }
+      for (int k = 0; k < C; ++k) {
+        const float lp = a[k] - la, lq = b[k] - lb;
+        const float p = expf(lp), q = expf(lq);
+        a[k] = sp * p * ((lp - lq) - gk);
+        b[k] = sq * (q - p);
+      }
+    }
+    __syncthreads();
+    kl_stage_out(dpost + (size_t)g0 * C, ng * C, C, P, stage[0], t, KL_BWD_TILE, vec);
+    kl_stage_out(dprior + (size_t)g0 * C, ng * C, C, P, stage[1], t, KL_BWD_TILE, vec);
+    __syncthreads();
+  }
+}
+
+static int g_kl_coalesced = 1;
+extern "C" int dm_kl_coalesced_enable(int on) {
+  if (on >= 0) g_kl_coalesced = on ? 1 : 0;
+  return g_kl_coalesced;
+}
+static bool kl_al16(const void* p) { return ((uintptr_t)p & 15) == 0; }
+
 __global__ void __launch_bounds__(256) kl_sampled_fwd_kernel(int rows, int S, int C, const float* __restrict__ post,
                                                              const float* __restrict__ prior, const int32_t* __restrict__ idx,
                                                              float* __restrict__ out) {
@@ -1561,7 +1828,12 @@
     DM_LAUNCH_CHECK();
     return DM_OK;
   }
-  hipLaunchKernelGGL(kl_fwd_kernel, dim3(dm_cdiv(rows, 4)), dim3(256), 0, st, rows, S, C, post, prior, kl, ep, eq);
+  if (g_kl_coalesced && C <= KL_STAGE_MAXC) {
+    const int vec = ((size_t)S * C) % 4 == 0 && kl_al16(post) && kl_al16(prior);
+    hipLaunchKernelGGL(kl_fwd_staged_kernel, dim3(dm_cdiv(rows, 4)), dim3(256), 0, st, rows, S, C, vec, post, prior, kl, ep, eq);
+  } else {
+    hipLaunchKernelGGL(kl_fwd_kernel, dim3(dm_cdiv(rows, 4)), dim3(256), 0, st, rows, S, C, post, prior, kl, ep, eq);
+  }
   DM_LAUNCH_CHECK();
   return DM_OK;
 }
@@ -1574,8 +1846,16 @@
     DM_LAUNCH_CHECK();
     return DM_OK;
   }
-  hipLaunchKernelGGL(kl_bwd_kernel, dim3(ew_blocks((size_t)rows * S)), dim3(256), 0, st, rows, S, C, post, prior, sp, sq,
-                     dpost, dprior);
+  if (g_kl_coalesced && C <= KL_STAGE_MAXC) {
+    const long long total = (long long)rows * S;
+    const int vec = ((size_t)total * C) % 4 == 0 && kl_al16(post) && kl_al16(prior) && kl_al16(dpost) && kl_al16(dprior);
+    const long long tiles = (total + KL_BWD_TILE - 1) / KL_BWD_TILE;
+    hipLaunchKernelGGL(kl_bwd_staged_kernel, dim3((unsigned)(tiles < 65536 ? tiles : 65536)), dim3(KL_BWD_TILE), 0, st, total, C,
+                       vec, post, prior, sp, sq, dpost, dprior);
+  } else {
+    hipLaunchKernelGGL(kl_bwd_kernel, dim3(ew_blocks((size_t)rows * S)), dim3(256), 0, st, rows, S, C, post, prior, sp, sq,
+                       dpost, dprior);
+  }
   DM_LAUNCH_CHECK();
   return DM_OK;
 }
diff --git a/pydreamer_amd/csrc/mlp.hip b/pydreamer_amd/csrc/mlp.hip
--- a/pydreamer_amd/csrc/mlp.hip
+++ b/pydreamer_amd/csrc/mlp.hip
@@ -290,7 +290,7 @@
     q.B = a.y[layers - 1]; q.ldb = hidden;
     q.C = g->w[layers]; q.ldc = hidden;
     DM_TRY(dm_gemm_launch(q, splitk, skb, st));
-    DM_TRY(dm_colsum_launch(rows, out_dim, dout, out_dim, g->b[layers], splitk, skb, st));
+    if (!normed) DM_TRY(dm_colsum_launch(rows, out_dim, dout, out_dim, g->b[layers], splitk, skb, st));
     DmGemm d;
     d.a_layout = 0; d.b_layout = 1;
     d.M = rows; d.N = hidden; d.K = out_dim;
@@ -306,8 +306,19 @@
     if (normed) {
       DM_TRY(dm_ln_elu_bwd_dx_launch(rows, hidden, a.xpre[l], hidden, a.y[l], hidden, a.stats[l], p->ln_g[l], dy, hidden,
                                      dxp, hidden, st));
-      DM_TRY(dm_ln_elu_bwd_params_launch(rows, hidden, a.xpre[l], hidden, a.y[l], hidden, a.stats[l], dy, hidden,
-                                         g->ln_g[l], g->ln_b[l], splitk, skb, st));
+      DmColsumSeg sg[3];
+      int nsg = 0;
+      sg[nsg].mode = DM_CS_LN; sg[nsg].rows = rows; sg[nsg].n = hidden;
+      sg[nsg].x = a.xpre[l]; sg[nsg].ldx = hidden; sg[nsg].y = a.y[l]; sg[nsg].ldy = hidden; sg[nsg].stats = a.stats[l];
+      sg[nsg].dy = dy; sg[nsg].lddy = hidden; sg[nsg].out0 = g->ln_g[l]; sg[nsg].out1 = g->ln_b[l];
+      ++nsg;
+      sg[nsg].rows = rows; sg[nsg].n = hidden; sg[nsg].x = dxp; sg[nsg].ldx = hidden; sg[nsg].out0 = g->b[l];
+      ++nsg;
+      if (l == layers - 1) {
+        sg[nsg].rows = rows; sg[nsg].n = out_dim; sg[nsg].x = dout; sg[nsg].ldx = out_dim; sg[nsg].out0 = g->b[layers];
+        ++nsg;
+      }
+      DM_TRY(dm_colsum_multi_launch(sg, nsg, splitk, skb, st));
     } else {
       DM_TRY(dm_elu_bwd_launch(rows, hidden, a.y[l], hidden, dy, hidden, dxp, hidden, st));
     }
@@ -318,7 +329,7 @@
     q.B = in; q.ldb = ldin;
     q.C = g->w[l]; q.ldc = kin;
     DM_TRY(dm_gemm_launch(q, splitk, skb, st));
-    DM_TRY(dm_colsum_launch(rows, hidden, dxp, hidden, g->b[l], splitk, skb, st));
+    if (!normed) DM_TRY(dm_colsum_launch(rows, hidden, dxp, hidden, g->b[l], splitk, skb, st));
     if (l > 0 || dx) {
       DmGemm d;
       d.a_layout = 0; d.b_layout = 1;
diff --git a/pydreamer_amd/csrc/rssm.hip b/pydreamer_amd/csrc/rssm.hip
--- a/pydreamer_amd/csrc/rssm.hip
+++ b/pydreamer_amd/csrc/rssm.hip
@@ -96,11 +96,18 @@
   if (gamma) return dm_ln_elu_bwd_dx_launch(rows, n, x, ldx, y, ldy, stats, gamma, dy, lddy, dx, lddx, st);
   return dm_elu_bwd_launch(rows, n, y, ldy, dy, lddy, dx, lddx, st);
 }
-static int norm_elu_bwd_params(int rows, int n, const float* x, int ldx, const float* y, int ldy, const float* stats,
-                               const float* dy, int lddy, float* dgamma, float* dbeta, void* ws, size_t ws_bytes,
-                               hipStream_t st) {
-  if (!dgamma && !dbeta) return DM_OK;
-  return dm_ln_elu_bwd_params_launch(rows, n, x, ldx, y, ldy, stats, dy, lddy, dgamma, dbeta, ws, ws_bytes, st);
+static DmColsumSeg colsum_seg(int rows, int n, const float* x, int ld, float* out) {
+  DmColsumSeg q;
+  q.rows = rows; q.n = n; q.x = x; q.ldx = ld; q.out0 = out;
+  return q;
+}
+static DmColsumSeg ln_params_seg(int rows, int n, const float* x, int ldx, const float* y, int ldy, const float* stats,
+                                 const float* dy, int lddy, float* dgamma, float* dbeta) {
+  DmColsumSeg q;
+  q.mode = DM_CS_LN;
+  q.rows = rows; q.n = n; q.x = x; q.ldx = ldx; q.y = y; q.ldy = ldy; q.stats = stats; q.dy = dy; q.lddy = lddy;
+  q.out0 = dgamma; q.out1 = dbeta;
+  return q;
 }
 
 static DmGemm linear_q(int rows, int nout, int kin, const float* x, int ldx, const float* W, const float* bias,
@@ -574,11 +581,12 @@
     return DM_OK;
   }
 
-  int cell_param_grads(int i) const {
+  int cell_param_grads(int i, DmColsumSeg* sg, int* nsg) const {
     const int ls = gk.ls;
     if (kind == 0) {
-      DM_TRY(dm_colsum_launch(N, 3 * ls, dgi + 3 * ls * i, 3 * D, gk.g_bih[i], sk_w, skb, sw));
-      return dm_colsum_launch(N, 3 * ls, dgh + 3 * ls * i, 3 * D, gk.g_bhh[i], sk_w, skb, sw);
+      sg[(*nsg)++] = colsum_seg(N, 3 * ls, dgi + 3 * ls * i, 3 * D, gk.g_bih[i]);
+      sg[(*nsg)++] = colsum_seg(N, 3 * ls, dgh + 3 * ls * i, 3 * D, gk.g_bhh[i]);
+      return DM_OK;
     }
     DM_TRY(dm_gru_norm_param_grads_launch(kind, N, ls, a.gs + 3 * ls * i, a.gst + 6 * i, dgl + 3 * ls * i, lnpg, lnpb, sw, 3 * D,
                                           6 * gk.L));
@@ -593,18 +601,23 @@
   int param_tail() const {
     const int L = gk.L;
     const bool stacked = L > 1;
+    DmColsumSeg sg[5 + 2 * 4];
+    int nsg = 0;
     if (stacked) DM_TRY(dm_wgrad_side_fork(st, sw));
-    DM_TRY(dm_colsum_launch(N, ZP, dpost, ZP, g[DM_RSSM_POST_OB], sk_w, skb, sw));
-    DM_TRY(norm_elu_bwd_params(N, Hd, a.x2, Hd, a.pin, Hd, a.st2, dpin, Hd, g[DM_RSSM_POST_G], g[DM_RSSM_POST_B], sk_w, skb, sw));
-    DM_TRY(dm_colsum_launch(N, Hd, dx2s, Hd, g[DM_RSSM_POST_H_B], sk_w, skb, sw));
+    sg[nsg++] = colsum_seg(N, ZP, dpost, ZP, g[DM_RSSM_POST_OB]);
+    if (g[DM_RSSM_POST_G] || g[DM_RSSM_POST_B])
+      sg[nsg++] = ln_params_seg(N, Hd, a.x2, Hd, a.pin, Hd, a.st2, dpin, Hd, g[DM_RSSM_POST_G], g[DM_RSSM_POST_B]);
+    sg[nsg++] = colsum_seg(N, Hd, dx2s, Hd, g[DM_RSSM_POST_H_B]);
     if (stacked) DM_TRY(wgrads(0, 3, 0, N, 0));
     for (int i = 0; i < L; ++i) {
       if (stacked) DM_TRY(wgrads(3 + 2 * i, 2, 0, N, 0));
-      DM_TRY(cell_param_grads(i));
-    }
-    DM_TRY(norm_elu_bwd_params(N, Hd, a.x1, Hd, a.za, Hd, a.st1, dza, Hd, g[DM_RSSM_IN_G], g[DM_RSSM_IN_B], sk_w, skb, sw));
-    DM_TRY(dm_colsum_launch(N, Hd, dx1s, Hd, g[DM_RSSM_Z_B], sk_w, skb, sw));
+      DM_TRY(cell_param_grads(i, sg, &nsg));
+    }
+    if (g[DM_RSSM_IN_G] || g[DM_RSSM_IN_B])
+      sg[nsg++] = ln_params_seg(N, Hd, a.x1, Hd, a.za, Hd, a.st1, dza, Hd, g[DM_RSSM_IN_G], g[DM_RSSM_IN_B]);
+    sg[nsg++] = colsum_seg(N, Hd, dx1s, Hd, g[DM_RSSM_Z_B]);
     if (stacked) DM_TRY(wgrads(3 + 2 * L, 2, 0, N, 0));
+    DM_TRY(dm_colsum_multi_launch(sg, nsg, sk_w, skb, sw));
     return dm_wgrad_side_mark(sw, st);
   }
 };
@@ -639,10 +652,16 @@
   DM_TRY(dgrad(st, sk, skb, N, Hd, D, c.dx3, Hd, p[DM_RSSM_PRIOR_H_W], dfeat, F, 1, nullptr));
   DM_TRY(dm_wgrad_side_fork(st, sw));
   DM_TRY(wgrad(sw, sk_w, skb, N, ZP, Hd, dprior, ZP, a.prin, Hd, g[DM_RSSM_PRIOR_W]));
-  DM_TRY(dm_colsum_launch(N, ZP, dprior, ZP, g[DM_RSSM_PRIOR_OB], sk_w, skb, sw));
-  DM_TRY(norm_elu_bwd_params(N, Hd, a.x3, Hd, a.prin, Hd, a.st3, c.dprin, Hd, g[DM_RSSM_PRIOR_G], g[DM_RSSM_PRIOR_B], sk_w, skb, sw));
   DM_TRY(wgrad(sw, sk_w, skb, N, Hd, D, c.dx3, Hd, feat, F, g[DM_RSSM_PRIOR_H_W]));
-  DM_TRY(dm_colsum_launch(N, Hd, c.dx3, Hd, g[DM_RSSM_PRIOR_H_B], sk_w, skb, sw));
+  {
+    DmColsumSeg sg[3];
+    int nsg = 0;
+    sg[nsg++] = colsum_seg(N, ZP, dprior, ZP, g[DM_RSSM_PRIOR_OB]);
+    if (g[DM_RSSM_PRIOR_G] || g[DM_RSSM_PRIOR_B])
+      sg[nsg++] = ln_params_seg(N, Hd, a.x3, Hd, a.prin, Hd, a.st3, c.dprin, Hd, g[DM_RSSM_PRIOR_G], g[DM_RSSM_PRIOR_B]);
+    sg[nsg++] = colsum_seg(N, Hd, c.dx3, Hd, g[DM_RSSM_PRIOR_H_B]);
+    DM_TRY(dm_colsum_multi_launch(sg, nsg, sk_w, skb, sw));
+  }
 
   DM_TRY(transpose(st, p[DM_RSSM_POST_W], c.wt_post, ZP, Hd));
   DM_TRY(transpose(st, p[DM_RSSM_POST_H_W], c.wt_post_h, Hd, D));
diff --git a/pydreamer_amd/hip.py b/pydreamer_amd/hip.py
--- a/pydreamer_amd/hip.py
+++ b/pydreamer_amd/hip.py
@@ -96,6 +96,11 @@
     _fields_ = [('x', c_void_p), ('n', c_int64), ('scale', c_float), ('mode', c_int32), ('center', c_void_p)]
 
 
+class dm_colsum_seg(Structure):
+    _fields_ = [(n, c_int32) for n in ('mode', 'rows', 'n', 'ldx', 'ldy', 'lddy')] + \
+               [(n, c_void_p) for n in ('x', 'y', 'stats', 'dy', 'out0', 'out1')]
+
+
 class dm_replay_field(Structure):
     _fields_ = [('dst', c_void_p), ('row_bytes', c_int64), ('is_reset', c_int32), ('reserved_', c_int32)]
 
@@ -129,6 +134,9 @@
     'dm_ln_elu_fwd': (c_int, [c_int, c_int, _P, c_int, _P, _P, c_float, _P, c_int, _P, _P]),
     'dm_ln_elu_bwd': (c_int, [c_int, c_int, _P, c_int, _P, c_int, _P, _P, _P, c_int, _P, c_int, _P, _P, _P, c_size_t, _P]),
     'dm_colsum': (c_int, [c_int, c_int, _P, c_int, _P, _P, c_size_t, _P]),
+    'dm_colsum_multi': (c_int, [_P, c_int, _P, c_size_t, _P]),
+    'dm_colsum_group_enable': (c_int, [c_int]),
+    'dm_kl_coalesced_enable': (c_int, [c_int]),
     'dm_gru_gates_fwd': (c_int, [c_int, c_int, _P, _P, _P, c_int, _P, c_int, _P]),
     'dm_gru_gates_bwd': (c_int, [c_int, c_int, _P, _P, _P, c_int, _P, c_int, _P, _P, _P, c_int, _P]),
     'dm_sample_onehot': (c_int, [c_int, c_int, c_int, _P, c_int, _P, _P, _P, c_int, _P, _P]),
```

Result: no change. 30.42 grad-steps/s, median of 6 (+0.4%).
